# jerry102102102/RL_brain_trainer

Measured on AMD Instinct MI355X. Metric: env-steps/sec (whole node), Stage-5 Approach->Finisher PPO loops (rollout + update); value = the Approach loop, finisher.value = the Finisher loop, higher is better.
Workload: dtype f32

## Files before the change

include/kp1_ppo.h:

```cpp
#ifndef KP1_PPO_H
#define KP1_PPO_H

#include <stdint.h>

#include "kp1.h"

#ifdef __cplusplus
extern "C" {
#endif

int kp1_gae_scan(int32_t device, const float* rewards, const float* values, const uint8_t* dones, const float* last_values,
                 float gamma, float gae_lambda, float* advantages, float* returns, int32_t T, int32_t N, void* stream);

int kp1_gae_scan_replicas(int32_t device, const float* rewards, const float* values, const uint8_t* dones, const float* last_values,
                          const float* gamma_lambda, int32_t n_per_replica, float* advantages, float* returns, int32_t T, int32_t N, void* stream);

int kp1_bootstrap_truncated(int32_t device, float* rewards, const float* terminal_values, const uint8_t* dones, float gamma,
                            int64_t count, void* stream);

int kp1_adv_minibatch_sums(int32_t device, const float* advantages, const int64_t* idx, int64_t total, int64_t minibatch, double* out_sums,
                           void* stream);
int kp1_random_permutation(int32_t device, int64_t n, const uint32_t* keys, int64_t* out, void* stream);

int kp1_adv_minibatch_stats(int32_t device, const double* sums, int64_t n_minibatches, float* out_stats, void* stream);

#define KP1_CURRICULUM_MAX_WINDOW 1024
#define KP1_CURRICULUM_MAX_HISTORY 64
typedef struct kp1_curriculum_event {
  int64_t total_timesteps;
  int32_t from_stage, to_stage;
  double trigger_success_rate;
} kp1_curriculum_event;
typedef struct kp1_curriculum_state {
  int32_t stage_index;
  int32_t stage_episode_count;
  int32_t ring_len, ring_head;
  int32_t window_episodes, min_episodes_per_stage, max_stage_index, n_events;
  double success_rate_threshold;
  int64_t num_timesteps;
  int32_t ring[KP1_CURRICULUM_MAX_WINDOW];
  kp1_curriculum_event events[KP1_CURRICULUM_MAX_HISTORY];
} kp1_curriculum_state;

int kp1_curriculum_create(int32_t device, double success_rate_threshold, int32_t window_episodes, int32_t min_episodes_per_stage,
                          int32_t max_stage_index, int32_t initial_stage_index, kp1_curriculum_state** out_dev);
int kp1_curriculum_destroy(int32_t device, kp1_curriculum_state* st_dev);
int kp1_curriculum_observe(int32_t device, kp1_curriculum_state* st_dev, const uint8_t* dones, int32_t n, int32_t steps_per_call, void* stream);
int kp1_curriculum_observe_chunk(int32_t device, kp1_curriculum_state* st_dev, const uint8_t* dones, int32_t n_local, int32_t chunk_steps,
                                 int32_t world, void* stream);
int kp1_curriculum_read(int32_t device, const kp1_curriculum_state* st_dev, kp1_curriculum_state* out_host, void* stream);
int kp1_bind_stage_ptr(kp1_env* env, const int32_t* stage_dev);

#define KP1_CURRICULUM_MAX_REPLICAS 16
int kp1_curriculum_create_population(int32_t device, int32_t n_replicas, double success_rate_threshold, int32_t window_episodes,
                                     int32_t min_episodes_per_stage, int32_t max_stage_index, const int32_t* initial_stages,
                                     kp1_curriculum_state** out_dev);
int kp1_curriculum_observe_population(int32_t device, kp1_curriculum_state* states_dev, const uint8_t* dones, int32_t n_per_replica,
                                      int32_t n_replicas, int32_t steps_per_call, void* stream);
int kp1_curriculum_read_replica(int32_t device, const kp1_curriculum_state* states_dev, int32_t n_replicas, int32_t k,
                                kp1_curriculum_state* out_host, void* stream);
int kp1_bind_population_stages(kp1_env* env, const kp1_curriculum_state* states_dev, int32_t n_replicas);

#define KP1_DOCK_CURRICULUM_MAX_STAGES 16
#define KP1_DOCK_CURRICULUM_MAX_WINDOW 1024
#define KP1_DOCK_CURRICULUM_MAX_HISTORY 32
typedef struct kp1_dock_curriculum_stage {
  double action_delta_scale, dock_residual_action_limit, dock_delta_q_change_limit_scale;
  double close_bucket_probability, close_bucket_min_pos_error_m, close_bucket_max_pos_error_m, close_bucket_max_ori_error_rad,
         handoff_state_probability;
  double close_init_q_noise[KP1_NJ], init_q_noise[KP1_NJ];
  double success_rate_threshold;
  int32_t min_episodes;
  int32_t window_episodes;
  int32_t handoff_offset, handoff_count;
} kp1_dock_curriculum_stage;
typedef struct kp1_dock_curriculum_event {
  int64_t total_timesteps;
  int32_t from_stage, to_stage, stage_episode_count, reserved0;
  double trigger_success_rate;
} kp1_dock_curriculum_event;
typedef struct kp1_dock_curriculum_state {
  int32_t stage_index, stage_episode_count, ring_len, ring_head, window_episodes, n_stages, n_events, reserved0;
  int64_t num_timesteps;
  kp1_dock_curriculum_stage stages[KP1_DOCK_CURRICULUM_MAX_STAGES];
  kp1_dock_curriculum_event events[KP1_DOCK_CURRICULUM_MAX_HISTORY];
  uint8_t ring[KP1_DOCK_CURRICULUM_MAX_WINDOW];
} kp1_dock_curriculum_state;
int kp1_dock_curriculum_create(kp1_env* env, const kp1_dock_curriculum_stage* stages_host, int32_t n_stages, int32_t window_episodes,
                               kp1_dock_curriculum_state** out_dev);
int kp1_dock_curriculum_destroy(kp1_env* env, kp1_dock_curriculum_state* st_dev);
int kp1_dock_curriculum_observe(kp1_env* env, kp1_dock_curriculum_state* st_dev, const uint8_t* dones, int32_t n_local, int32_t chunk_steps, int32_t world,
                                void* stream);
int kp1_dock_curriculum_read(kp1_env* env, const kp1_dock_curriculum_state* st_dev, kp1_dock_curriculum_state* out_host, void* stream);
int kp1_dock_curriculum_create_population(kp1_env* env, const kp1_dock_curriculum_stage* stages_host, int32_t n_stages, int32_t window_episodes,
                                          int32_t n_replicas, kp1_dock_curriculum_state** out_dev);
int kp1_dock_curriculum_observe_population(kp1_env* env, kp1_dock_curriculum_state* states_dev, const uint8_t* dones, int32_t n_per_replica,
                                           int32_t n_replicas, void* stream);
int kp1_dock_curriculum_read_replica(kp1_env* env, const kp1_dock_curriculum_state* states_dev, int32_t n_replicas, int32_t k,
                                     kp1_dock_curriculum_state* out_host, void* stream);

#define KP1_MLP_IN 56
#define KP1_MLP_IN_PAD 64
#define KP1_MLP_IN_ROUTE 80
#define KP1_MLP_IN_ROUTE_PAD 128
#define KP1_MLP_ACT 7

typedef struct kp1_mlp kp1_mlp;

int kp1_mlp_create(int32_t device, int32_t hidden, int32_t max_batch, kp1_mlp** out);
int kp1_mlp_create_ex(int32_t device, int32_t hidden, int32_t obs_dim, int32_t max_batch, kp1_mlp** out);
#define KP1_MLP_MAX_REPLICAS 16
int kp1_mlp_create_population(int32_t device, int32_t hidden, int32_t obs_dim, int32_t max_batch, int32_t replicas, kp1_mlp** out);
int32_t kp1_mlp_replicas(const kp1_mlp* m);
typedef struct kp1_replica_hparams {
  float learning_rate, adam_eps, max_grad_norm, clip_range, ent_coef, vf_coef;
} kp1_replica_hparams;
int kp1_mlp_set_replica_hparams(kp1_mlp* m, const kp1_replica_hparams* host, int32_t n, void* stream);
int kp1_mlp_destroy(kp1_mlp* m);
int64_t kp1_mlp_num_params(int32_t hidden);
int64_t kp1_mlp_num_params_ex(int32_t hidden, int32_t obs_dim);
int kp1_mlp_pack_weights(kp1_mlp* m, const float* params, void* stream);

int kp1_mlp_forward(kp1_mlp* m, const float* obs, int32_t obs_stride, int32_t n, const float* noise, float* mean, float* value,
                    float* action, float* clipped_action, float* log_prob, void* stream);

int kp1_mlp_forward_env_step(kp1_mlp* m, kp1_env* env, const float* obs, int32_t obs_stride, const float* noise, float* value, float* action,
                             float* log_prob, float* next_obs, float* reward, uint8_t* done, float* terminal_obs, void* stream);

int kp1_eval_step(kp1_mlp* m, kp1_env* env, float* obs, float* reward, uint8_t* done, const kp1_eval_buffers* buffers, int32_t step,
                  const double* ready_thresholds , int32_t confirm_steps, void* stream);

int kp1_mlp_loss_grad(kp1_mlp* m, const float* obs, int32_t obs_stride, const int64_t* idx, int32_t n, const float* actions,
                      const float* old_log_prob, const float* advantages, const float* returns, float adv_mean, float adv_inv_std,
                      const float* adv_stats_dev, float clip_range, float ent_coef, float vf_coef, float inv_count, float* grad_out,
                      float* stats_out, int32_t grad_is_zero, void* stream);

#define KP1_MLP_OPT_FUSED 1
#define KP1_MLP_OPT_ACTOR_EXTRA_STEPS 2
#define KP1_MLP_OPT_STEP_COUNT 3
#define KP1_MLP_OPT_PROFILE 4
#define KP1_MLP_OPT_BF16X3_WGRAD 5
#define KP1_MLP_PROFILE_SLOTS 4
#define KP1_MLP_PROFILE_TILE 0
#define KP1_MLP_PROFILE_WGRAD 1
#define KP1_MLP_PROFILE_FINALIZE 2
#define KP1_MLP_PROFILE_ADAM 3
int kp1_mlp_set_option(kp1_mlp* m, int32_t option, int32_t value);
int kp1_mlp_profile_read(kp1_mlp* m, float* out_us , int32_t* out_launches );

int kp1_mlp_adam_step(kp1_mlp* m, float* params, float* grad, float* exp_avg, float* exp_avg_sq, float lr, float eps,
                      float max_grad_norm, int32_t step, int32_t flags, void* stream);

int kp1_mlp_anchor_loss_grad(kp1_mlp* m, const float* obs, int32_t obs_stride, const int64_t* idx, int32_t n, const float* teacher_actions,
                             float loss_weight, float* grad_out, float* loss_out, void* stream);

int kp1_mlp_anchor_adam_step(kp1_mlp* m, float* params, float* grad, float* exp_avg, float* exp_avg_sq, float lr, float eps,
                             float max_grad_norm, int32_t step, void* stream);

int kp1_mlp_placement_check(int32_t device, int32_t n_rows, int32_t* out, void* stream);
int kp1_mlp_time_kernels(kp1_mlp* m, const float* obs, int32_t obs_stride, int32_t n, int32_t iters, float* out_ms, double* out_flops,
                         void* stream);

int kp1_set_obs_stride(kp1_env* env, int32_t stride);

#ifdef __cplusplus
}
#endif
#endif
```

rl_brain_trainer_amd/csrc/kp1_mlp.hip:

```cpp
#include <hip/hip_runtime.h>
#include <hip/hip_ext.h>

#include <cmath>
#include <cstddef>
#include <cstdlib>
#include <cstring>
#include <vector>

#include "../../include/kp1_ppo.h"
#include "kp1_device.hpp"
#include "kp1_host.hpp"

using kp1::fail;
using namespace kp1;

typedef float f32x16 __attribute__((ext_vector_type(16)));
typedef float f32x4 __attribute__((ext_vector_type(4)));

namespace {

constexpr int ACT = KP1_MLP_ACT, HEADS = 8;
constexpr float LOG_SQRT_2PI = 0.9189385332046727f;

enum { EPI_BIAS_TANH = 0, EPI_DTANH = 1 };
// ... 1097 lines not shown
#pragma unroll
    for (int j = 0; j < WLOADS; ++j) *reinterpret_cast<f32x4*>(w3s + 4 * (threadIdx.x + 256 * j)) = wv[j];
#pragma unroll
    for (int j = 0; j < LOADS; ++j) {
      const int f = threadIdx.x + 256 * j, r = f / Q, c4 = f % Q;
      *reinterpret_cast<f32x4*>(h2s + r * hpitch + 4 * c4) = hv[j];
    }
  }
  __syncthreads();
  const int row_l = threadIdx.x >> 3, out = threadIdx.x & 7;
  const int row = blockIdx.x * HEAD_ROWS + row_l;
  const bool ok = row < a.n && out < ACT;
  float d = 0.f, l = 0.f;
  if (ok) {
    const int64_t src = a.idx ? a.idx[row] : (int64_t)row;
    const float mean = head_dot(h2s + row_l * hpitch, w3s + out * HP, HP) + a.b3[out];
    const float diff = mean - a.teacher[src * ACT + out];
    d = a.dcoef * diff;
    l = a.lcoef * diff * diff;
  }
  dout[row_l * 8 + out] = d;
  float dsum = d;
  dsum += __shfl_xor(dsum, 8);
  dsum += __shfl_xor(dsum, 16);
  dsum += __shfl_xor(dsum, 32);
  float lsum = l;
#pragma unroll
  for (int off = 1; off < 64; off <<= 1) lsum += __shfl_xor(lsum, off);
  const int wave_ = threadIdx.x >> 6;
  if ((threadIdx.x & 63) < 8) red[wave_ * 12 + out] = dsum;
  if ((threadIdx.x & 63) == 0) red[wave_ * 12 + 8] = lsum;
  __syncthreads();
  float* part = a.hpart + (int64_t)blockIdx.x * a.hpart_stride;
  if (threadIdx.x < 8) {
    const int slot = threadIdx.x < ACT ? threadIdx.x : 8;
    part[10 * HP + (threadIdx.x < ACT ? threadIdx.x : 15)] = ((red[slot] + red[12 + slot]) + red[24 + slot]) + red[36 + slot];
  }
  const int rows_here = min(HEAD_ROWS, a.n - blockIdx.x * HEAD_ROWS);
  for (int hh = threadIdx.x; hh < 2 * HP; hh += 256) {
    const int h = hh % HP;
    if (hh >= HP) {
      for (int r = 0; r < rows_here; ++r) a.dz2[a.strideH + (int64_t)(blockIdx.x * HEAD_ROWS + r) * HP + h] = 0.f;
      continue;
    }
    float wcol[ACT], gw[ACT];
#pragma unroll
    for (int o = 0; o < ACT; ++o) {
      wcol[o] = w3s[o * HP + h];
      gw[o] = 0.f;
    }
    float gb2 = 0.f;
    for (int r = 0; r < rows_here; ++r) {
      const float hp = h2s[r * hpitch + h];
      float dp = 0.f;
#pragma unroll
      for (int o = 0; o < ACT; ++o) {
        const float dd = dout[r * 8 + o];
        dp = fmaf(dd, wcol[o], dp);
        gw[o] = fmaf(dd, hp, gw[o]);
      }
      const float dz = dp * (1.f - hp * hp);
      a.dz2[(int64_t)(blockIdx.x * HEAD_ROWS + r) * HP + h] = dz;
      gb2 += dz;
    }
#pragma unroll
    for (int o = 0; o < ACT; ++o) part[o * HP + h] = gw[o];
    part[8 * HP + h] = gb2;
  }
}

__device__ __forceinline__ bool is_actor_element(const ParamLayout& L, int64_t i) {
  return (i >= L.p_w1 && i < L.v_w1) || (i >= L.a_w && i < L.c_w);
}

struct AnchorFinalizeArgs {
  FinalizeArgs f;
  float* loss_out;
};

template <bool POP = false>
__global__ void __launch_bounds__(256) anchor_finalize_kernel(const AnchorFinalizeArgs a_) {
  const FinalizeArgs a = POP ? finalize_args_replica(a_.f, blockIdx.y) : a_.f;
  const ParamLayout& L = a.L;
  __shared__ double sq[4];
  const int64_t i = (int64_t)(blockIdx.x * 256u + threadIdx.x);
  float gval = 0.f;
  if (i < L.total) {
    if (is_actor_element(L, i)) {
      const PartialSrc s = finalize_source(a, i);
      for (int c = 0; c < s.n; ++c) gval += s.p[(int64_t)c * s.stride];
    }
    a.grad[i] = gval;
  }
  if (blockIdx.x == 0 && threadIdx.x == 0) {
    float t = 0.f;
    for (int c = 0; c < a.h_n; ++c) t += a.hpart[(int64_t)c * a.h_stride + 10 * L.Hp + 15];
    a_.loss_out[POP ? blockIdx.y : 0u] = t;
  }
  double w = (double)gval * (double)gval;
  for (int off = 32; off > 0; off >>= 1) w += __shfl_xor(w, off);
  if ((threadIdx.x & 63) == 0) sq[threadIdx.x >> 6] = w;
  __syncthreads();
  if (threadIdx.x == 0) a.sumsq[blockIdx.x] = ((sq[0] + sq[1]) + sq[2]) + sq[3];
}

template <bool POP = false>
__global__ void __launch_bounds__(ADAM_BLOCK) anchor_adam_kernel(float* __restrict__ p, const float* __restrict__ g, float* __restrict__ m, float* __restrict__ v,
                                                          const double* __restrict__ partials, int n_partials, float lr, float eps, float max_norm,
                                                          const ParamLayout L, const Packed k_, const int* __restrict__ step_dev, int host_step,
                                                          unsigned r_partials, const float* __restrict__ hparams) {
  __shared__ float sh[3];
  const Packed k = POP ? packed_replica(k_, L, blockIdx.y) : k_;
  if constexpr (POP) {
    const unsigned o = blockIdx.y * (unsigned)L.total;
    p += o; g += o; m += o; v += o;
    partials += blockIdx.y * r_partials;
    if (hparams) {
      const float* e = hparams + blockIdx.y * (unsigned)HP_FIELDS;
      lr = e[HP_LR];
      eps = e[HP_EPS];
    }
  }
  const int64_t i = (int64_t)blockIdx.x * ADAM_BLOCK + threadIdx.x;
  const bool actor = i < L.total && is_actor_element(L, i);
  const int64_t il = actor ? i : L.p_w1;
  const float g_in = g[il], m_in = m[il], v_in = v[il], p_in = p[il];
  double s = 0.0;
  if (threadIdx.x < 64) {
    for (int q = threadIdx.x; q < n_partials; q += 64) s += partials[q];
    for (int off = 32; off > 0; off >>= 1) s += __shfl_xor(s, off);
  }
  if (threadIdx.x == 0) {
    const float norm = (float)sqrt(s);
    const int st = (host_step > 0 ? host_step : step_dev[0]) + step_dev[1] + 1;
    sh[0] = max_norm > 0.f ? fminf(max_norm / (norm + 1e-6f), 1.f) : 1.f;
    sh[1] = (float)((double)lr / (1.0 - pow(0.9, (double)st)));
    sh[2] = (float)sqrt(1.0 - pow(0.999, (double)st));
  }
  __syncthreads();
  if (actor) {
    const float gi = g_in * sh[0];
    const float mn = 0.9f * m_in + 0.1f * gi;
    const float vn = 0.999f * v_in + 0.001f * gi * gi;
    const float denom = sqrtf(vn) / sh[2] + eps;
    const float pn = p_in - sh[1] * (mn / denom);
    m[i] = mn; v[i] = vn; p[i] = pn;
    pack_one(i, pn, L, k);
  }
}

__global__ void anchor_count_kernel(int* __restrict__ actor_extra) { *actor_extra += 1; }

#include "kp1_env_step.inc"
#include "kp1_eval_step.inc"
#include "kp1_mlp_tile.inc"
#include "kp1_mlp_fused.inc"

}

struct kp1_mlp {
  int device = 0, H = 0, Hp = 0, max_batch = 0;
  int K = 1;
  ParamLayout L;
  Packed k{};
  float* h1 = nullptr;
  float* h2 = nullptr;
  float* dz2 = nullptr;
  float* dz1 = nullptr;
  float* xf = nullptr;
  int bf16x3 = 0;
  unsigned short* sp_h1 = nullptr; unsigned short* sp_dz2 = nullptr; unsigned short* sp_dz1 = nullptr; unsigned short* sp_xf = nullptr;
  double* partials = nullptr;
  double* anchor_partials = nullptr;
  float* slab = nullptr;
  float* slab1 = nullptr;
  float* bslab = nullptr;
  float* hpart = nullptr;
  int n_finalize_blocks = 0;
  int* step_dev = nullptr;
  float* hparams_dev = nullptr;
  bool hparams_on = false;
  int last_s2_n = 0, last_s1_n = 0;
  int fused = 1;
  const float* last_params = nullptr;
  bool slab_stale = false;
  std::vector<void*> allocs;
  int profile = 0;
  struct ProfPair { hipEvent_t a, b; };
  std::vector<ProfPair> prof[KP1_MLP_PROFILE_SLOTS];
  int prof_used[KP1_MLP_PROFILE_SLOTS] = {0, 0, 0, 0};
};

namespace {
struct ProfSlotInFlight { hipEvent_t a = nullptr, b = nullptr; bool attached = false; };
thread_local ProfSlotInFlight tl_prof;

struct ProfScope {
  kp1_mlp* m; int slot; hipStream_t stream; bool on;
  ProfScope(kp1_mlp* m_, int slot_, hipStream_t s_) : m(m_), slot(slot_), stream(s_), on(m_->profile != 0) {
    if (!on) return;
    auto& v = m->prof[slot];
    if (m->prof_used[slot] >= (int)v.size()) {
      kp1_mlp::ProfPair p{};
      if (hipEventCreate(&p.a) != hipSuccess || hipEventCreate(&p.b) != hipSuccess) { on = false; return; }
      v.push_back(p);
    }
    tl_prof.a = v[m->prof_used[slot]].a;
    tl_prof.b = v[m->prof_used[slot]].b;
    tl_prof.attached = false;
  }
  ~ProfScope() {
    if (!on) return;
    if (!tl_prof.attached) {
      (void)hipEventRecord(tl_prof.a, stream);
      (void)hipEventRecord(tl_prof.b, stream);
    }
    tl_prof = ProfSlotInFlight{};
    m->prof_used[slot] += 1;
  }
};

#define KP1_LAUNCH(kernel, grid, block, bytes, stream, ...)                                                        \
  do {                                                                                                             \
    if (tl_prof.a != nullptr && !tl_prof.attached) {                                                               \
      tl_prof.attached = true;                                                                                     \
      hipExtLaunchKernelGGL(kernel, grid, block, bytes, stream, tl_prof.a, tl_prof.b, 0, __VA_ARGS__);             \
    } else {                                                                                                       \
      hipLaunchKernelGGL(kernel, grid, block, bytes, stream, __VA_ARGS__);                                         \
    }                                                                                                              \
  } while (0)
}

namespace {

constexpr int N_PARTIALS = 128;
constexpr int ANCHOR_PARTIALS = 256;
constexpr int PARTIALS_STRIDE = 2 * N_PARTIALS + 2048;
constexpr int TN_SPLIT2 = 8, TN_SPLIT1 = 16;

int tn_chunk_rows(int n, int tiles) {
  int chunks = (256 + tiles - 1) / tiles;
  if (chunks > 64) chunks = 64;
  if (chunks < 1) chunks = 1;
  int rows = (n + chunks - 1) / chunks;
  rows = (rows + 63) / 64 * 64;
  return rows < 64 ? 64 : rows;
}

int mlp_check_device(const kp1_mlp* m) {
  HIP_TRY(hipSetDevice(m->device));
  return KP1_OK;
}

constexpr size_t TN_LDS_BYTES = sizeof(float) * 2 * 2 * 64 * (128 + 4);

template <int BN, int EPI, int K, bool POP = false>
int launch_nt_inst(const GemmNT& g, hipStream_t stream) {
  constexpr int NTH = BN == 256 ? 512 : 256;
  constexpr int BM = 64;
  constexpr int BKS = 32;
  size_t bytes = sizeof(float) * (BM * (size_t)(K + 4) + 2 * (size_t)BN * (BKS + 4));
  const size_t epi = sizeof(float) * (BM * (size_t)(BN + 4) + (size_t)(NTH / (BN / 4)) * BN);
  if (epi > bytes) bytes = epi;
  HIP_TRY(hipFuncSetAttribute((const void*)gemm_nt_kernel<BN, EPI, K, NTH, BM, BKS, POP>, hipFuncAttributeMaxDynamicSharedMemorySize, (int)bytes));
  hipLaunchKernelGGL((gemm_nt_kernel<BN, EPI, K, NTH, BM, BKS, POP>), dim3((g.M + BM - 1) / BM, g.N / BN, POP ? 2 * g.reps : 2), dim3(NTH), bytes, stream, g);
  return KP1_OK;
}

int nt_row_tiles(int n, int Hp) {
  (void)Hp;
  return (n + 63) / 64;
}

template <int EPI>
int launch_nt(const GemmNT& g, hipStream_t stream) {
  if (g.N % 128 != 0) return fail(KP1_ERR_INVALID, "gemm_nt needs N % 128 == 0");
  if (g.reps > 1) {
    if (g.N != 128) return fail(KP1_ERR_UNSUPPORTED, "population gemm_nt is instantiated for N = 128");
    if (g.K == 64) return launch_nt_inst<128, EPI, 64, true>(g, stream);
    if (g.K == 128) return launch_nt_inst<128, EPI, 128, true>(g, stream);
    return fail(KP1_ERR_UNSUPPORTED, "population gemm_nt is instantiated for K in {64, 128}");
  }
  const int row_tiles = (g.M + 63) / 64;
  const bool wide = (g.N % 256 == 0) && row_tiles * 2 >= 200;
  if (g.K == 64) return wide ? launch_nt_inst<256, EPI, 64>(g, stream) : launch_nt_inst<128, EPI, 64>(g, stream);
  if (g.K == 128) return wide ? launch_nt_inst<256, EPI, 128>(g, stream) : launch_nt_inst<128, EPI, 128>(g, stream);
  if (g.K == 256) return wide ? launch_nt_inst<256, EPI, 256>(g, stream) : launch_nt_inst<128, EPI, 256>(g, stream);
  return fail(KP1_ERR_UNSUPPORTED, "gemm_nt is instantiated for K in {64, 128, 256}");
}

int launch_tn(kp1_mlp* m, GemmTN t, int n_o_tiles, int slab_cols, float* slab, int* n_chunks_out, hipStream_t stream);

int launch_fused(const FusedArgs& fa_in, hipStream_t stream) {
  FusedArgs fa = fa_in;
  static const int stagger_us = [] { const char* e = std::getenv("KP1_FU_STAGGER_US"); return e ? std::atoi(e) : 11; }();
  static const int n_cus = [] {
    int dev = 0, n = 0;
    if (hipGetDevice(&dev) != hipSuccess || hipDeviceGetAttribute(&n, hipDeviceAttributeMultiprocessorCount, dev) != hipSuccess) n = 256;
    return n;
  }();
  const dim3 grid((fa.n + FU_BM - 1) / FU_BM, 1, 2);
  fa.n_cus = n_cus;
  fa.stagger_ticks = (int)(grid.x * grid.z) > n_cus ? stagger_us * 100 : 0;
  const size_t bytes = sizeof(float) * FU_LDS_FLOATS;
  if (fa.sp_h1 != nullptr) {
    if (fa.inp == 64) {
// ... 205 lines not shown
  }
  *out = m;
  return KP1_OK;
}
}

extern "C" {

int kp1_mlp_destroy(kp1_mlp* m) {
  if (!m) return KP1_OK;
  (void)hipSetDevice(m->device);
  (void)hipDeviceSynchronize();
  for (void* p : m->allocs) (void)hipFree(p);
  for (void* p : {(void*)m->sp_h1, (void*)m->sp_dz2, (void*)m->sp_dz1, (void*)m->sp_xf}) (void)hipFree(p);
  for (auto& v : m->prof)
    for (auto& pr : v) {
      (void)hipEventDestroy(pr.a);
      (void)hipEventDestroy(pr.b);
    }
  delete m;
  return KP1_OK;
}

int kp1_mlp_set_option(kp1_mlp* m, int32_t option, int32_t value) {
  if (!m) return fail(KP1_ERR_INVALID, "NULL argument");
  if (option == KP1_MLP_OPT_FUSED) {
    m->fused = value ? 1 : 0;
    if (!m->fused && m->slab_stale && m->last_params) {
      HIP_TRY(hipSetDevice(m->device));
      HIP_TRY(hipDeviceSynchronize());
      Packed k = m->k;
      k.formats = PACK_SLAB | PACK_FRAG;
      hipLaunchKernelGGL(pack_kernel<false>, dim3((unsigned)((m->L.total + 255) / 256)), dim3(256), 0, (hipStream_t)0, m->last_params, m->L, k);
      HIP_TRY(kp1::launch_status());
      HIP_TRY(hipDeviceSynchronize());
      m->slab_stale = false;
    }
    return KP1_OK;
  }
  if (option == KP1_MLP_OPT_BF16X3_WGRAD) {
    if (value && m->K > 1) return fail(KP1_ERR_UNSUPPORTED, "the bf16x3 weight-gradient experiment is not available on population handles");
    if (value && !(m->fused && m->Hp == FU_HP)) return fail(KP1_ERR_UNSUPPORTED, "the bf16x3 weight-gradient experiment needs the 2x256 tile kernels");
    if (value && !m->sp_h1) {
      HIP_TRY(hipSetDevice(m->device));
      const size_t act = (size_t)3 * 2 * m->max_batch * m->Hp * sizeof(unsigned short), xb = (size_t)3 * m->max_batch * m->L.INP * sizeof(unsigned short);
      for (unsigned short** p : {&m->sp_h1, &m->sp_dz2, &m->sp_dz1}) {
        HIP_TRY(hipMalloc((void**)p, act));
        HIP_TRY(hipMemset(*p, 0, act));
      }
      HIP_TRY(hipMalloc((void**)&m->sp_xf, xb));
      HIP_TRY(hipMemset(m->sp_xf, 0, xb));
    }
    m->bf16x3 = value ? 1 : 0;
    return KP1_OK;
  }
  if (option == KP1_MLP_OPT_PROFILE) {
    m->profile = value ? 1 : 0;
    for (int k = 0; k < KP1_MLP_PROFILE_SLOTS; ++k) m->prof_used[k] = 0;
    return KP1_OK;
  }
  if (option == KP1_MLP_OPT_STEP_COUNT) {
    if (value < 0) return fail(KP1_ERR_INVALID, "step count must be >= 0");
    HIP_TRY(hipSetDevice(m->device));
    HIP_TRY(hipMemcpy(m->step_dev, &value, sizeof(int), hipMemcpyHostToDevice));
    return KP1_OK;
  }
  if (option == KP1_MLP_OPT_ACTOR_EXTRA_STEPS) {
    if (value < 0) return fail(KP1_ERR_INVALID, "actor extra steps must be >= 0");
    HIP_TRY(hipSetDevice(m->device));
    HIP_TRY(hipMemcpy(m->step_dev + 1, &value, sizeof(int), hipMemcpyHostToDevice));
    return KP1_OK;
  }
  return fail(KP1_ERR_INVALID, "unknown kp1_mlp option");
}

int kp1_mlp_set_replica_hparams(kp1_mlp* m, const kp1_replica_hparams* host, int32_t n, void* stream) {
  static_assert(sizeof(kp1_replica_hparams) == sizeof(float) * HP_FIELDS, "kp1_replica_hparams is HP_FIELDS floats");
  static_assert(offsetof(kp1_replica_hparams, learning_rate) == sizeof(float) * HP_LR && offsetof(kp1_replica_hparams, adam_eps) == sizeof(float) * HP_EPS &&
                offsetof(kp1_replica_hparams, max_grad_norm) == sizeof(float) * HP_MAX_NORM && offsetof(kp1_replica_hparams, clip_range) == sizeof(float) * HP_CLIP &&
                offsetof(kp1_replica_hparams, ent_coef) == sizeof(float) * HP_ENT && offsetof(kp1_replica_hparams, vf_coef) == sizeof(float) * HP_VF,
                "kp1_replica_hparams field order");
  if (!m) return fail(KP1_ERR_INVALID, "NULL argument");
  if (n == 0) {
    m->hparams_on = false;
    return KP1_OK;
  }
  if (m->K == 1) return fail(KP1_ERR_UNSUPPORTED, "a K = 1 handle takes its hyper-parameters as scalar arguments, not a per-replica table");
  if (n != m->K || !host) return fail(KP1_ERR_INVALID, "kp1_mlp_set_replica_hparams needs one entry per replica (n = K)");
  for (int r = 0; r < n; ++r) {
    const kp1_replica_hparams& h = host[r];
    for (float v : {h.learning_rate, h.adam_eps, h.max_grad_norm, h.clip_range, h.ent_coef, h.vf_coef})
      if (!std::isfinite(v)) return fail(KP1_ERR_INVALID, "replica hyper-parameters must be finite");
  }
  int rc = mlp_check_device(m);
  if (rc != KP1_OK) return rc;
  HIP_TRY(hipMemcpyAsync(m->hparams_dev, host, sizeof(kp1_replica_hparams) * (size_t)n, hipMemcpyHostToDevice, (hipStream_t)stream));
  HIP_TRY(hipStreamSynchronize((hipStream_t)stream));
  m->hparams_on = true;
  return KP1_OK;
}

int kp1_mlp_pack_weights(kp1_mlp* m, const float* params, void* stream) {
  if (!m || !params) return fail(KP1_ERR_INVALID, "NULL argument");
  int rc = mlp_check_device(m);
  if (rc != KP1_OK) return rc;
  Packed k = m->k;
  k.formats = PACK_SLAB | PACK_FRAG;
  if (m->K > 1)
    hipLaunchKernelGGL(pack_kernel<true>, dim3((unsigned)((m->L.total + 255) / 256), m->K), dim3(256), 0, (hipStream_t)stream, params, m->L, k);
  else
    hipLaunchKernelGGL(pack_kernel<false>, dim3((unsigned)((m->L.total + 255) / 256)), dim3(256), 0, (hipStream_t)stream, params, m->L, k);
  HIP_TRY(kp1::launch_status());
  m->last_params = params;
  m->slab_stale = false;
  return KP1_OK;
}

int kp1_mlp_forward(kp1_mlp* m, const float* obs, int32_t obs_stride, int32_t n, const float* noise, float* mean, float* value, float* action,
                    float* clipped_action, float* log_prob, void* stream) {
  if (!m || !obs) return fail(KP1_ERR_INVALID, "NULL argument");
  if (n <= 0 || n > m->max_batch) return fail(KP1_ERR_INVALID, "n exceeds the workspace max_batch");
  const int IN = m->L.IN, INP = m->L.INP;
  if (obs_stride != IN && obs_stride != INP) return fail(KP1_ERR_INVALID, "obs_stride must be the observation width or its padded width (56 / 64, or 80 / 128)");
  int rc = mlp_check_device(m);
  if (rc != KP1_OK) return rc;
  if (m->fused && m->Hp == FU_HP) {
    FusedArgs fa{};
    fa.obs = obs; fa.obs_stride = obs_stride; fa.Kreal = obs_stride >= INP ? INP : IN; fa.inp = INP; fa.idx = nullptr; fa.n = n;
    fa.k = m->k;
    fa.noise = noise; fa.mean = mean; fa.value = value; fa.action = action; fa.clipped = clipped_action; fa.log_prob = log_prob;
    rc = launch_fused_infer(fa, (hipStream_t)stream);
    if (rc != KP1_OK) return rc;
    HIP_TRY(kp1::launch_status());
    return KP1_OK;
  }
  rc = launch_forward_layers(m, obs, obs_stride, nullptr, n, (hipStream_t)stream);
  if (rc != KP1_OK) return rc;
  HeadArgs a{};
  a.h2 = m->h2; a.strideH = (int64_t)m->max_batch * m->Hp; a.Hp = m->Hp; a.n = n; a.H = m->H;
  a.w3 = m->k.w3; a.b3 = m->k.b3; a.log_std = m->k.log_std;
  a.noise = noise; a.mean = mean; a.value = value; a.action = action; a.clipped = clipped_action; a.log_prob = log_prob;
  if (m->K > 1) {
    a.r_act = (unsigned)(2 * a.strideH);
    hipLaunchKernelGGL(head_infer_kernel<true>, dim3((n + HEAD_ROWS - 1) / HEAD_ROWS, m->K), dim3(256), sizeof(float) * HEADS * m->Hp, (hipStream_t)stream, a);
  } else {
    hipLaunchKernelGGL(head_infer_kernel<false>, dim3((n + HEAD_ROWS - 1) / HEAD_ROWS), dim3(256), sizeof(float) * HEADS * m->Hp, (hipStream_t)stream, a);
  }
  HIP_TRY(kp1::launch_status());
  return KP1_OK;
}

int kp1_mlp_forward_env_step(kp1_mlp* m, kp1_env* env, const float* obs, int32_t obs_stride, const float* noise, float* value, float* action,
                             float* log_prob, float* next_obs, float* reward, uint8_t* done, float* terminal_obs, void* stream) {
  if (!m || !env || !obs || !action || !next_obs || !reward || !done) return fail(KP1_ERR_INVALID, "NULL argument to kp1_mlp_forward_env_step");
  if (m->K > 1) return fail(KP1_ERR_UNSUPPORTED, "kp1_mlp_forward_env_step is not available on population handles");
  if (!(m->fused && m->Hp == FU_HP) || m->L.INP != 64)
    return fail(KP1_ERR_UNSUPPORTED, "kp1_mlp_forward_env_step needs the 2x256 tile kernels and the 56-float observation (padded to 64)");
  if (obs_stride != m->L.IN && obs_stride != m->L.INP) return fail(KP1_ERR_INVALID, "obs_stride must be 56 or 64");
  int rc = mlp_check_device(m);
  if (rc != KP1_OK) return rc;
  FusedArgs fa{};
  int mode = 0, device = 0;
  int64_t n_envs = 0;
  rc = kp1::env_step_args_f32(env, &fa.env, sizeof fa.env, nullptr, next_obs, reward, done, terminal_obs, 1, &mode, &n_envs, &device);
  if (rc != KP1_OK) return rc;
  if (device != m->device) return fail(KP1_ERR_INVALID, "the env handle and the MLP workspace live on different devices");
  if (n_envs > m->max_batch) return fail(KP1_ERR_INVALID, "more envs than the workspace max_batch");
  fa.obs = obs; fa.obs_stride = obs_stride; fa.Kreal = obs_stride >= m->L.INP ? m->L.INP : m->L.IN; fa.inp = m->L.INP; fa.idx = nullptr; fa.n = (int)n_envs;
  fa.k = m->k;
  fa.noise = noise; fa.value = value; fa.action = action; fa.log_prob = log_prob;
  rc = launch_fused_infer_env(fa, mode, (hipStream_t)stream);
  if (rc != KP1_OK) return rc;
  HIP_TRY(kp1::launch_status());
  return KP1_OK;
}

int kp1_eval_step(kp1_mlp* m, kp1_env* env, float* obs, float* reward, uint8_t* done, const kp1_eval_buffers* b, int32_t step,
                  const double* ready_thresholds, int32_t confirm_steps, void* stream) {
  if (!m || !env || !obs || !reward || !done || !b) return fail(KP1_ERR_INVALID, "NULL argument to kp1_eval_step");
  if (!b->metrics || !b->counters || !b->flags || !b->state || !b->n_alive) return fail(KP1_ERR_INVALID, "kp1_eval_step: NULL buffer");
  if (b->hand_metrics && (!b->hand_step || !b->hand_success || !b->hand_state)) return fail(KP1_ERR_INVALID, "kp1_eval_step: incomplete handoff buffers");
  if (step < 1) return fail(KP1_ERR_INVALID, "kp1_eval_step accounts env steps 1, 2, ...: step 0 (the initialisation after a reset) is kp1_eval_accumulate's");
  if (m->Hp != ES_HP) return fail(KP1_ERR_UNSUPPORTED, "kp1_eval_step covers the layer-wise widths (hidden 64 / 128); a 2x256 policy is evaluated through kp1_mlp_forward");
  if (m->L.INP != ES_INP) return fail(KP1_ERR_UNSUPPORTED, "kp1_eval_step needs the 56-float observation (padded to 64)");
  EvalStepArgs a{};
  int mode = 0, device = 0;
  int64_t n_envs = 0;
  int rc = kp1::env_step_args_f32(env, &a.env, sizeof a.env, nullptr, obs, reward, done, nullptr, 0, &mode, &n_envs, &device);
  if (rc != KP1_OK) return rc;
  if (a.env.stage_ptr) return fail(KP1_ERR_UNSUPPORTED, "kp1_eval_step: the env handle is bound to a curriculum tracker (an evaluation handle has none)");
  if (device != m->device) return fail(KP1_ERR_INVALID, "the env handle and the MLP workspace live on different devices");
  if (mode != KP1_MODE_APPROACH && mode != KP1_MODE_DOCK) return fail(KP1_ERR_UNSUPPORTED, "kp1_eval_step steps the approach or the dock mode");
  if (n_envs <= 0 || n_envs % m->K != 0) return fail(KP1_ERR_INVALID, "kp1_eval_step: the env count must be a multiple of the handle's replica count");
  rc = mlp_check_device(m);
  if (rc != KP1_OK) return rc;
  const int Hp = m->Hp, INP = m->L.INP;
  a.b = *b;
  a.w1 = m->k.w1p; a.b1 = m->k.b1; a.w2 = m->k.w2; a.b2 = m->k.b2; a.w3 = m->k.w3; a.b3 = m->k.b3;
  a.r_w1 = (unsigned)(2 * Hp * INP); a.r_w2 = (unsigned)(2 * Hp * Hp); a.r_b = (unsigned)(2 * Hp); a.r_w3 = (unsigned)(HEADS * Hp); a.r_b3 = (unsigned)HEADS;
  a.n = (int)(n_envs / m->K);
  a.Kreal = a.env.obs_stride >= INP ? INP : m->L.IN;
  a.step = step; a.confirm = confirm_steps;
  a.track_ready = ready_thresholds != nullptr;
  if (ready_thresholds) { a.thr_pos = ready_thresholds[0]; a.thr_ori = ready_thresholds[1]; a.thr_act = ready_thresholds[2]; a.thr_dq = ready_thresholds[3]; }
  hipStream_t st = (hipStream_t)stream;
  HIP_TRY(hipMemsetAsync(b->n_alive, 0, sizeof(int32_t), st));
  const dim3 grid((unsigned)((a.n + ES_BM - 1) / ES_BM), (unsigned)m->K);
  const bool pop = m->K > 1, dock = mode == KP1_MODE_DOCK;
  if (pop && dock) hipLaunchKernelGGL((eval_step_kernel<KP1_MODE_DOCK, true>), grid, dim3(ES_NTH), 0, st, a);
  else if (pop) hipLaunchKernelGGL((eval_step_kernel<KP1_MODE_APPROACH, true>), grid, dim3(ES_NTH), 0, st, a);
  else if (dock) hipLaunchKernelGGL((eval_step_kernel<KP1_MODE_DOCK, false>), grid, dim3(ES_NTH), 0, st, a);
  else hipLaunchKernelGGL((eval_step_kernel<KP1_MODE_APPROACH, false>), grid, dim3(ES_NTH), 0, st, a);
  HIP_TRY(kp1::launch_status());
  return KP1_OK;
}

int kp1_mlp_loss_grad(kp1_mlp* m, const float* obs, int32_t obs_stride, const int64_t* idx, int32_t n, const float* actions,
                      const float* old_log_prob, const float* advantages, const float* returns, float adv_mean, float adv_inv_std,
                      const float* adv_stats_dev, float clip_range, float ent_coef, float vf_coef, float inv_count, float* grad_out,
                      float* stats_out, int32_t grad_is_zero, void* stream_) {
  if (!m || !obs || !actions || !old_log_prob || !advantages || !returns || !grad_out) return fail(KP1_ERR_INVALID, "NULL argument");
  if (n <= 0 || n > m->max_batch) return fail(KP1_ERR_INVALID, "n exceeds the workspace max_batch");
  const int IN = m->L.IN, INP = m->L.INP;
  if (obs_stride != IN && obs_stride != INP) return fail(KP1_ERR_INVALID, "obs_stride must be the observation width or its padded width (56 / 64, or 80 / 128)");
  int rc = mlp_check_device(m);
  if (rc != KP1_OK) return rc;
  hipStream_t stream = (hipStream_t)stream_;
  const int Hp = m->Hp, H = m->H;
  const int64_t act_stride = (int64_t)m->max_batch * Hp;
  const ParamLayout& L = m->L;
  (void)grad_is_zero;
  const bool fused = m->fused && Hp == FU_HP;
  const bool pop = m->K > 1;
  if (pop && !idx) return fail(KP1_ERR_INVALID, "population handles gather their rows through idx [K][n]");
  const int64_t hpart_rep = (int64_t)(m->max_batch / 32) * (10 * Hp + 32);
  int adv_mode = 0;
  if (adv_stats_dev) adv_mode = 2;
  else if (adv_inv_std > 0.f) adv_mode = 3;
  else if (adv_inv_std == 0.f) adv_mode = 1;
  if (adv_mode == 1) {
    if (pop)
      hipLaunchKernelGGL(adv_partials_kernel<true>, dim3(N_PARTIALS, m->K), dim3(256), 0, stream, advantages, idx, n, m->partials, (unsigned)PARTIALS_STRIDE);
    else
      hipLaunchKernelGGL(adv_partials_kernel<false>, dim3(N_PARTIALS), dim3(256), 0, stream, advantages, idx, n, m->partials, 0u);
  }
  const int hpart_stride = 10 * Hp + 32;
  if (fused) {
    FusedArgs fa{};
    fa.obs = obs; fa.obs_stride = obs_stride; fa.Kreal = obs_stride >= INP ? INP : IN; fa.inp = INP; fa.idx = idx; fa.n = n;
    fa.k = m->k;
    fa.actions = actions; fa.old_logp = old_log_prob; fa.adv = advantages; fa.ret = returns;
    fa.adv_partials = m->partials; fa.n_adv_partials = N_PARTIALS; fa.adv_stats = adv_stats_dev; fa.adv_mean = adv_mean; fa.adv_inv_std = adv_inv_std;
    fa.adv_mode = adv_mode;
    fa.clip_range = clip_range; fa.vf_coef = vf_coef; fa.inv_count = inv_count;
    fa.h1 = m->h1; fa.dz2 = m->dz2; fa.dz1 = m->dz1; fa.act_stride = act_stride; fa.xf = m->xf;
    fa.bslab = m->bslab; fa.hpart = m->hpart; fa.hpart_stride = hpart_stride;
    if (m->bf16x3) {
      fa.sp_h1 = m->sp_h1; fa.sp_dz2 = m->sp_dz2; fa.sp_dz1 = m->sp_dz1; fa.sp_xf = m->sp_xf;
      fa.sp_plane = (int64_t)2 * m->max_batch * Hp; fa.sp_plane_x = (int64_t)m->max_batch * INP;
    }
    {
      ProfScope ps(m, KP1_MLP_PROFILE_TILE, stream);
      rc = launch_fused(fa, stream);
    }
    if (rc != KP1_OK) return rc;
  } else {
    rc = launch_forward_layers(m, obs, obs_stride, idx, n, stream);
    if (rc != KP1_OK) return rc;
    HeadArgs a{};
    a.h2 = m->h2; a.strideH = act_stride; a.Hp = Hp; a.n = n; a.H = H;
    a.w3 = m->k.w3; a.b3 = m->k.b3; a.log_std = m->k.log_std;
    a.idx = idx; a.actions = actions; a.old_logp = old_log_prob; a.adv = advantages; a.ret = returns;
    a.adv_partials = m->partials; a.n_adv_partials = N_PARTIALS; a.adv_stats = adv_stats_dev; a.adv_mean = adv_mean; a.adv_inv_std = adv_inv_std;
    a.adv_mode = adv_mode;
    a.clip_range = clip_range; a.ent_coef = ent_coef; a.vf_coef = vf_coef; a.inv_count = inv_count;
    a.dz2 = m->dz2;
    a.hpart = m->hpart; a.hpart_stride = hpart_stride;
    a.r_act = (unsigned)(2 * act_stride); a.r_hpart = (unsigned)hpart_rep; a.r_partials = (unsigned)PARTIALS_STRIDE;
    a.hparams = pop && m->hparams_on ? m->hparams_dev : nullptr;
    {
      const dim3 hgrid((n + HEAD_ROWS - 1) / HEAD_ROWS, m->K);
      const size_t hbytes = sizeof(float) * (HEADS * Hp + HEAD_ROWS * 8 + 84 + 2 * HEAD_ROWS * (Hp + 4));
      if (pop) {
        HIP_TRY(hipFuncSetAttribute((const void*)head_train_kernel<128, true>, hipFuncAttributeMaxDynamicSharedMemorySize, (int)hbytes));
        hipLaunchKernelGGL((head_train_kernel<128, true>), hgrid, dim3(256), hbytes, stream, a);
      } else if (Hp == 256) {
        HIP_TRY(hipFuncSetAttribute((const void*)head_train_kernel<256>, hipFuncAttributeMaxDynamicSharedMemorySize, (int)hbytes));
        hipLaunchKernelGGL(head_train_kernel<256>, hgrid, dim3(256), hbytes, stream, a);
      } else {
        HIP_TRY(hipFuncSetAttribute((const void*)head_train_kernel<128>, hipFuncAttributeMaxDynamicSharedMemorySize, (int)hbytes));
        hipLaunchKernelGGL(head_train_kernel<128>, hgrid, dim3(256), hbytes, stream, a);
      }
    }
    GemmNT g{};
    g.A = m->dz2; g.lda = Hp; g.strideA = act_stride; g.gather = nullptr;
    g.W = m->k.w2t; g.strideW = (int64_t)Hp * Hp;
    g.bias = nullptr; g.strideBias = 0;
    g.C = m->dz1; g.ldc = Hp; g.strideC = act_stride;
    g.aux = m->h1; g.strideAux = act_stride;
    g.colsum = m->bslab; g.strideColsum = Hp;
    g.M = n; g.N = Hp; g.K = Hp; g.Kreal = Hp;
    g.reps = m->K;
    g.r_A = g.r_C = g.r_aux = (unsigned)(2 * act_stride); g.r_W = (unsigned)(2 * Hp * Hp);
    g.r_colsum = (unsigned)((m->max_batch / 32) * 2 * Hp);
    rc = launch_nt<EPI_DTANH>(g, stream);
    if (rc != KP1_OK) return rc;
  }

  int s2_n = 0, s1_n = 0;
  if (fused) {
    TnFragArgs t{};
    t.inp = INP;
    t.dz2 = m->dz2; t.h1 = m->h1; t.dz1 = m->dz1; t.act_stride = act_stride; t.xf = m->xf;
    t.slab2 = m->slab; t.s2_net = (int64_t)Hp * Hp; t.s2_chunk = 2 * t.s2_net;
    t.slab1 = m->slab1; t.s1_net = (int64_t)Hp * INP; t.s1_chunk = 2 * t.s1_net;
    t.groups = (n + FU_BM - 1) / FU_BM * (FU_BM / 8);
    auto up8 = [](int v) { return (v + 7) / 8 * 8; };
    t.cg2 = up8((t.groups + TN_SPLIT2 - 1) / TN_SPLIT2);
    t.cg1 = up8((t.groups + TN_SPLIT1 - 1) / TN_SPLIT1);
    t.n_chunks2 = (t.groups + t.cg2 - 1) / t.cg2;
    t.n_chunks1 = (t.groups + t.cg1 - 1) / t.cg1;
    if (m->bf16x3) {
      TnBf16Args b{};
// ... 398 lines not shown
```

rl_brain_trainer_amd/csrc/kp1_mlp_tile.inc:

```

struct FusedArgs {
  const float* obs; int64_t obs_stride; int Kreal;
  int inp;
  const int64_t* idx; int n;
  Packed k;
  const float* actions; const float* old_logp; const float* adv; const float* ret;
  const double* adv_partials; int n_adv_partials; const float* adv_stats; float adv_mean, adv_inv_std; int adv_mode;
  float clip_range, vf_coef, inv_count;
  float* h1; float* dz2; float* dz1; int64_t act_stride;
  float* xf;
  float* bslab;
  float* hpart; int hpart_stride;
  const float* noise; float* mean; float* value; float* action; float* clipped; float* log_prob;
  int net_base;
  int stagger_ticks, n_cus;
  StepArgs<float> env;
  unsigned short* sp_h1; unsigned short* sp_dz2; unsigned short* sp_dz1; unsigned short* sp_xf; int64_t sp_plane, sp_plane_x;
};

typedef __bf16 bf16x8 __attribute__((ext_vector_type(8)));
struct Split3 { bf16x8 hi, mid, lo; };
__device__ __forceinline__ Split3 split3(const float* v) {
  Split3 o;
#pragma unroll
  for (int j = 0; j < 8; ++j) {
    const __bf16 h = (__bf16)v[j];
    const float r1 = v[j] - (float)h;
    const __bf16 m = (__bf16)r1;
    const float r2 = r1 - (float)m;
    o.hi[j] = h;
    o.mid[j] = m;
    o.lo[j] = (__bf16)r2;
  }
  return o;
}
__device__ __forceinline__ void store_split3(unsigned short* __restrict__ base, int64_t plane, int64_t fi, int ncb, int cb, int lane, const Split3& s) {
  const int64_t at = ((fi * ncb + cb) * 64 + lane) * 8;
  *reinterpret_cast<bf16x8*>(base + at) = s.hi;
  *reinterpret_cast<bf16x8*>(base + plane + at) = s.mid;
  *reinterpret_cast<bf16x8*>(base + 2 * plane + at) = s.lo;
}

__host__ __device__ inline int64_t frag8_at(int64_t b, int64_t col, int64_t C) {
  return ((b >> 3) * (C >> 5) + (col >> 5)) * 256 + ((col & 31) + 32 * ((b & 7) >> 2)) * 4 + (b & 3);
}

__device__ __forceinline__ f32x4 fu_wload(const char* __restrict__ base, unsigned off) {
  const __amdgpu_buffer_rsrc_t r = __builtin_amdgcn_make_buffer_rsrc(const_cast<char*>(base), 0, 0x7fffffff, 0x00020000);
  return __builtin_bit_cast(f32x4, __builtin_amdgcn_raw_buffer_load_b128(r, (int)off, 0, AUX_SC1));
}
constexpr int FU_HP = 256, FU_BKS = 32, FU_AP = FU_HP + 4;
constexpr int FU_STAGE = FU_HP * FU_BKS;
constexpr int FU_BM = 32, FU_NW = 4, FU_CB = 2, FU_NTH = 64 * FU_NW;
constexpr int FU_SCRATCH = 4 * FU_BM * 8 + FU_BM * 8 + FU_NW * 24 + 64;
constexpr int FU_LDS_FLOATS = 2 * FU_BM * FU_AP + HEADS * FU_HP + FU_SCRATCH;
static_assert(FU_LDS_FLOATS * 4 * 2 <= 160 * 1024, "the two training tiles of one CU must fit its LDS");

template <bool TRAIN, int K1S, int ENV = 0, bool SPLIT = false>
__global__ void __launch_bounds__(FU_NTH, ENV ? 1 : 2) mlp_tile_kernel(const FusedArgs a) {
  static_assert(!(TRAIN && ENV), "the env step rides on the inference tile only");
  static_assert(TRAIN || !SPLIT, "split planes are written by the training tile");
  constexpr int NW = FU_NW, CB = FU_CB, BM = FU_BM, NTH = FU_NTH, CW = 32 * CB;
  constexpr int INP = K1S * FU_BKS, FU_XP = INP + 4, GS_L2 = K1S, GS_BW = K1S + 8, GS_END = K1S + 16;
  constexpr int KG = FU_BKS / 8, NB = CB * KG;
  constexpr int L1_REAL_GROUPS = K1S == 2 ? (KP1_MLP_IN + 7) / 8 : (KP1_MLP_IN_ROUTE + 7) / 8;
  extern __shared__ float lds[];
  float* bufA = lds;
  float* bufB = bufA + BM * FU_AP;
  float* w3s = bufB + BM * FU_AP;
  float* dotred = w3s + HEADS * FU_HP;
  float* dout = dotred + 4 * BM * 8;
  float* wsum = dout + BM * 8;
  float* misc = wsum + NW * 24;

  const int z = (int)blockIdx.z + a.net_base;
  const int m0 = blockIdx.x * BM, slot = blockIdx.x;
  const int tid = threadIdx.x, lane = tid & 63, wave = __builtin_amdgcn_readfirstlane(tid >> 6);
  const unsigned lane_off = (unsigned)lane * 16u;
  const char* __restrict__ W1F = reinterpret_cast<const char*>(a.k.w1f + (int64_t)z * K1S * FU_STAGE + wave * NB * 64 * 4);
  const char* __restrict__ W2F = reinterpret_cast<const char*>(a.k.w2f + (int64_t)z * 8 * FU_STAGE + wave * NB * 64 * 4);
  const char* __restrict__ W2TF = reinterpret_cast<const char*>(a.k.w2tf + (int64_t)z * 8 * FU_STAGE + wave * NB * 64 * 4);

  f32x4 bf[3][NB];
#define FU_BLOAD(gs)                                                                                    \
  if ((gs) < GS_END) {                                                                                  \
    const char* p_ = (gs) < GS_L2 ? W1F + (gs) * (FU_STAGE * 4) : ((gs) < GS_BW ? W2F + ((gs) - GS_L2) * (FU_STAGE * 4) : W2TF + ((gs) - GS_BW) * (FU_STAGE * 4)); \
    _Pragma("unroll") for (int q = 0; q < NB; ++q) bf[(gs) % 3][q] = fu_wload(p_, q * 1024 + lane_off); \
  }
  f32x16 acc[CB];
#define FU_INIT_ACC(bias)                                                                               \
  _Pragma("unroll") for (int c = 0; c < CB; ++c)                                                        \
    _Pragma("unroll") for (int e = 0; e < 16; ++e) acc[c][e] = (bias)[c];
#ifdef KP1_TR_HEADS
#define KP1_TR_G2(slot)
#define KP1_TR_HD(slot) KP1_TR(slot)
#else
#define KP1_TR_G2(slot) KP1_TR(slot)
#define KP1_TR_HD(slot)
#endif
#ifdef KP1_FU_NOMFMA
#define FU_MFMA(acc_, a_, b_) acc_[0] += (a_) * (b_);
#else
#define FU_MFMA(acc_, a_, b_) acc_ = __builtin_amdgcn_mfma_f32_32x32x2f32(a_, b_, acc_, 0, 0, 0);
#endif
#ifdef KP1_FU_NOTANH
#define FU_TANH(x) (x)
#else
#define FU_TANH(x) kp_tanh(x)
#endif
#define FU_GEMM(abuf, ap, KT, GS0)                                                                      \
  {                                                                                                     \
    const float* as = (abuf) + (lane & 31) * (ap) + 4 * (lane >> 5);                                     \
    _Pragma("unroll") for (int s = 0; s < (KT); ++s) {                                                  \
      FU_BLOAD((GS0) + s + 2)                                                                           \
      __builtin_amdgcn_sched_barrier(0);                                                                \
      f32x4 av[KG];                                                                                     \
      _Pragma("unroll") for (int kg = 0; kg < KG; ++kg)                                                 \
        av[kg] = *reinterpret_cast<const f32x4*>(as + s * FU_BKS + kg * 8);                              \
      _Pragma("unroll") for (int kg = 0; kg < KG; ++kg)                                                 \
        if (!((GS0) == 0 && s * KG + kg >= L1_REAL_GROUPS))    \
        _Pragma("unroll") for (int i = 0; i < 4; ++i)                                                   \
          _Pragma("unroll") for (int c = 0; c < CB; ++c)                                                \
            FU_MFMA(acc[c], av[kg][i], bf[((GS0) + s) % 3][c * KG + kg][i])                              \
      __builtin_amdgcn_sched_barrier(0);                                                                \
      if ((GS0) == GS_L2) { KP1_TR_G2(7 + s) }                                                          \
    }                                                                                                   \
  }
#define FU_ROW(e) (((e) & 3) + 8 * ((e) >> 2) + 4 * (lane >> 5))
#define FU_COL(c) (wave * CW + (c) * 32 + (lane & 31))
#ifdef KP1_FU_NOSTORE
#define FU_STORE_ACC(dst)
#else
#define FU_STORE_ACC(dst)                                                                               \
  _Pragma("unroll") for (int c = 0; c < CB; ++c)                                                        \
    _Pragma("unroll") for (int g = 0; g < 4; ++g) {                                                     \
      const f32x4 v_ = {acc[c][4 * g], acc[c][4 * g + 1], acc[c][4 * g + 2], acc[c][4 * g + 3]};        \
      *reinterpret_cast<f32x4*>((dst) + ((int64_t)((m0 >> 3) + g) * (FU_HP / 32) + wave * CB + c) * 256 + lane * 4) = v_; \
    }
#endif
#define FU_STORE_ACC_SPLIT(dst, plane)                                                                  \
  if constexpr (SPLIT) {                                                                               \
    _Pragma("unroll") for (int c = 0; c < CB; ++c)                                                      \
      _Pragma("unroll") for (int f = 0; f < 2; ++f) {                                                   \
        float v8_[8];                                                                                   \
        _Pragma("unroll") for (int j = 0; j < 8; ++j) v8_[j] = acc[c][8 * f + j];                       \
        store_split3((dst) + (int64_t)z * ((plane) / 2), (plane), (int64_t)(m0 >> 4) + f, FU_HP / 32, wave * CB + c, lane, split3(v8_)); \
      }                                                                                                 \
  }
#define FU_STORE_FRAG_SPLIT(tile, pitch, dst, plane, zoff, C)                                           \
  if constexpr (SPLIT) {                                                                               \
    _Pragma("unroll") for (int q = wave; q < (BM / 16) * ((C) / 32); q += NW) {                         \
      const int f_ = q / ((C) / 32), cb_ = q % ((C) / 32);                                              \
      const float* t_ = (tile) + (16 * f_ + 4 * (lane >> 5)) * (pitch) + 32 * cb_ + (lane & 31);        \
      float v8_[8];                                                                                     \
      _Pragma("unroll") for (int j = 0; j < 8; ++j) v8_[j] = t_[(8 * (j >> 2) + (j & 3)) * (pitch)];    \
      store_split3((dst) + (zoff), (plane), (int64_t)(m0 >> 4) + f_, (C) / 32, cb_, lane, split3(v8_));  \
    }                                                                                                   \
  }
#ifdef KP1_FU_NOSTORE
#define FU_STORE_FRAG(tile, pitch, dst, C)
#else
#define FU_STORE_FRAG(tile, pitch, dst, C)                                                              \
  _Pragma("unroll") for (int q = wave; q < (BM / 8) * ((C) / 32); q += NW) {                            \
    const int g_ = q / ((C) / 32), cb_ = q % ((C) / 32);                                                \
    const float* t_ = (tile) + (8 * g_ + 4 * (lane >> 5)) * (pitch) + 32 * cb_ + (lane & 31);           \
    f32x4 v_;                                                                                           \
    _Pragma("unroll") for (int i = 0; i < 4; ++i) v_[i] = t_[i * (pitch)];                              \
    *reinterpret_cast<f32x4*>((dst) + ((int64_t)((m0 >> 3) + g_) * ((C) / 32) + cb_) * 256 + lane * 4) = v_; \
  }
#endif

  KP1_TR(0)
  if (TRAIN) { KP1_CLK(0, 0) }
  if (TRAIN && a.stagger_ticks > 0) {
    const int linear = blockIdx.x + gridDim.x * blockIdx.z;
    if (linear >= a.n_cus && linear < 2 * a.n_cus) {
      const unsigned long long t0_ = wall_clock64();
      while (wall_clock64() - t0_ < (unsigned long long)a.stagger_ticks) __builtin_amdgcn_s_sleep(16);
    }
  }
  FU_BLOAD(0)
  FU_BLOAD(1)
  __builtin_amdgcn_sched_barrier(0);
  {
    constexpr int XQ = INP / 4, X_LOADS = BM * XQ / NTH;
    constexpr int W3_LOADS = HEADS * FU_HP / 4 / NTH;
    static_assert(X_LOADS >= 1 && X_LOADS * NTH == BM * XQ && W3_LOADS >= 1 && W3_LOADS * NTH == HEADS * FU_HP / 4, "prologue loads must tile the workgroup");
    int64_t xrow[X_LOADS];
    f32x4 xv[X_LOADS], w3v[W3_LOADS];
#pragma unroll
    for (int j = 0; j < X_LOADS; ++j) {
      const int m = min(m0 + (tid + NTH * j) / XQ, a.n - 1);
      xrow[j] = a.idx ? a.idx[m] : (int64_t)m;
    }
#pragma unroll
    for (int j = 0; j < X_LOADS; ++j) {
      const int k = 4 * ((tid + NTH * j) % XQ);
      xv[j] = *reinterpret_cast<const f32x4*>(a.obs + xrow[j] * a.obs_stride + (k < a.Kreal ? k : 0));
    }
#pragma unroll
    for (int j = 0; j < W3_LOADS; ++j) w3v[j] = *reinterpret_cast<const f32x4*>(a.k.w3 + 4 * (tid + NTH * j));
#pragma unroll
    for (int j = 0; j < X_LOADS; ++j) {
      const int f = tid + NTH * j, row = f / XQ, k = 4 * (f % XQ);
      const float keep = (m0 + row < a.n && k < a.Kreal) ? 1.f : 0.f;
      *reinterpret_cast<f32x4*>(bufB + row * FU_XP + k) = xv[j] * keep;
    }
#pragma unroll
    for (int j = 0; j < W3_LOADS; ++j) *reinterpret_cast<f32x4*>(w3s + 4 * (tid + NTH * j)) = w3v[j];
  }
  if (TRAIN && z == 0 && wave == 0) {
    float mean = 0.f, inv_std = 1.f;
    if (a.adv_mode == 1) {
      double ps = 0.0, pss = 0.0;
      for (int k = lane; k < a.n_adv_partials; k += 64) {
        ps += a.adv_partials[2 * k];
        pss += a.adv_partials[2 * k + 1];
      }
      for (int off = 32; off > 0; off >>= 1) {
        ps += __shfl_xor(ps, off);
        pss += __shfl_xor(pss, off);
      }
      const double mu = ps / a.n;
      const double var = a.n > 1 ? fmax((pss - a.n * mu * mu) / (a.n - 1), 0.0) : 0.0;
      mean = (float)mu;
      inv_std = (float)(1.0 / (sqrt(var) + 1e-8));
    } else if (a.adv_mode == 2) {
      mean = a.adv_stats[0];
      inv_std = a.adv_stats[1];
    } else if (a.adv_mode == 3) {
      mean = a.adv_mean;
      inv_std = a.adv_inv_std;
    }
    if (lane == 0) {
      misc[0] = mean;
      misc[1] = inv_std;
    }
  }
  float bias1[CB], bias2[CB];
#pragma unroll
  for (int c = 0; c < CB; ++c) {
    bias1[c] = a.k.b1[z * FU_HP + FU_COL(c)];
    bias2[c] = a.k.b2[z * FU_HP + FU_COL(c)];
  }
  const int l_row = tid >> 3, l_out = tid & 7;
  const bool l_ok = m0 + l_row < a.n;
  const int64_t l_src = a.idx ? a.idx[min(m0 + l_row, a.n - 1)] : (int64_t)min(m0 + l_row, a.n - 1);
  __syncthreads();
  KP1_TR(1)
  constexpr bool fp32_out = !SPLIT;
  if (TRAIN && z == 0 && fp32_out) { FU_STORE_FRAG(bufB, FU_XP, a.xf, INP) }
  if (TRAIN && z == 0) { FU_STORE_FRAG_SPLIT(bufB, FU_XP, a.sp_xf, a.sp_plane_x, (int64_t)0, INP) }

  FU_INIT_ACC(bias1)
  FU_GEMM(bufB, FU_XP, K1S, 0)
#pragma unroll
  for (int c = 0; c < CB; ++c)
#pragma unroll
    for (int e = 0; e < 16; ++e) {
      acc[c][e] = FU_TANH(acc[c][e]);
      bufA[FU_ROW(e) * FU_AP + FU_COL(c)] = acc[c][e];
    }
  if (TRAIN && fp32_out) { FU_STORE_ACC(a.h1 + z * a.act_stride) }
  if (TRAIN) { FU_STORE_ACC_SPLIT(a.sp_h1, a.sp_plane) }
  __syncthreads();
  KP1_TR(2)
  float l_act = 0.f, l_old = 0.f, l_adv = 0.f, l_ret = 0.f, l_b3 = a.k.b3[l_out], l_ls = a.k.log_std[l_out < ACT ? l_out : 0];
  if (TRAIN) {
    if (z == 0) {
      if (l_out < ACT) l_act = a.actions[l_src * ACT + l_out];
      l_old = a.old_logp[l_src];
      l_adv = a.adv[l_src];
    } else {
      l_ret = a.ret[l_src];
    }
  } else if (z == 0 && a.noise && l_ok && l_out < ACT) {
    l_act = a.noise[l_src * ACT + l_out];
  }

  FU_INIT_ACC(bias2)
  FU_GEMM(bufA, FU_AP, 8, GS_L2)
#pragma unroll
  for (int c = 0; c < CB; ++c)
#pragma unroll
    for (int e = 0; e < 16; ++e) bufB[FU_ROW(e) * FU_AP + FU_COL(c)] = FU_TANH(acc[c][e]);
  __syncthreads();
  KP1_TR(3)

  {
    const int row = lane & 31, kq = wave, part = kq * 2 + (lane >> 5);
    const float* hrow = bufB + row * FU_AP + part * 32;
    f32x4 hv[8];
#pragma unroll
    for (int q = 0; q < 8; ++q) hv[q] = *reinterpret_cast<const f32x4*>(hrow + 4 * q);
    auto dot = [&](int o) {
      const float* w = w3s + o * FU_HP + part * 32;
      float s = 0.f;
#pragma unroll
      for (int q = 0; q < 8; ++q) {
        const f32x4 wv = *reinterpret_cast<const f32x4*>(w + 4 * q);
        s = fmaf(hv[q].x, wv.x, s);
        s = fmaf(hv[q].y, wv.y, s);
        s = fmaf(hv[q].z, wv.z, s);
        s = fmaf(hv[q].w, wv.w, s);
      }
      s += __shfl_xor(s, 32);
      if (lane < 32) dotred[(kq * BM + row) * 8 + o] = s;
    };
    if (z == 0) {
#pragma unroll
      for (int o = 0; o < ACT; ++o) dot(o);
    } else {
      dot(7);
    }
  }
  __syncthreads();
  KP1_TR_HD(7)
  if (!TRAIN) {
    const bool mine = z == 0 ? l_out < ACT : l_out == 7;
    float v = 0.f;
    if (mine) {
#pragma unroll
      for (int p = 0; p < 4; ++p) v += dotred[(p * BM + l_row) * 8 + l_out];
      v += l_b3;
    }
    float lp = 0.f;
    if (z == 0) {
      float act = v;
      if (l_ok && l_out < ACT) {
        if (a.mean) a.mean[l_src * ACT + l_out] = v;
        if (a.noise) {
          act = fmaf(expf(l_ls), l_act, v);
          lp = -0.5f * l_act * l_act - l_ls - LOG_SQRT_2PI;
        }
        if (a.action) a.action[l_src * ACT + l_out] = act;
        if (a.clipped) a.clipped[l_src * ACT + l_out] = fminf(fmaxf(act, -1.f), 1.f);
      }
      lp += __shfl_xor(lp, 1);
      lp += __shfl_xor(lp, 2);
      lp += __shfl_xor(lp, 4);
      if (l_ok && l_out == 0 && a.log_prob) a.log_prob[l_src] = lp;
      if constexpr (ENV != 0) {
        dout[l_row * 8 + l_out] = (l_ok && l_out < ACT) ? act : 0.f;
        __syncthreads();
        if (wave == 0) {
          const bool live = lane < BM && m0 + lane < a.n;
          float o[KP1_OBS_DIM];
          if (live) step_env_lane<float, ENV == 1 ? KP1_MODE_APPROACH : KP1_MODE_DOCK, false>(a.env, (int64_t)(m0 + lane), dout + lane * 8, o);
          store_obs_tile(a.env.obs, (int64_t)m0, min(BM, a.n - m0), o, live, a.env.obs_stride, bufA);
        }
      }
    } else if (l_ok && l_out == 7 && a.value) {
      a.value[l_src] = v;
    }
    return;
  }
  {
    const int row_l = l_row, out = l_out;
    const bool ok = l_ok;
    const bool mine = z == 0 ? out < ACT : out == 7;
    float v = 0.f;
    if (mine) {
#pragma unroll
      for (int p = 0; p < 4; ++p) v += dotred[(p * BM + row_l) * 8 + out];
      v += l_b3;
    }
    float zs = 0.f, inv_sd = 1.f, lp = 0.f;
    if (z == 0 && ok && out < ACT) {
      inv_sd = expf(-l_ls);
      zs = (l_act - v) * inv_sd;
      lp = -0.5f * zs * zs - l_ls - LOG_SQRT_2PI;
    }
    lp += __shfl_xor(lp, 1);
    lp += __shfl_xor(lp, 2);
    lp += __shfl_xor(lp, 4);
    float g_logp = 0.f, d = 0.f, pl = 0.f, vl = 0.f, kl = 0.f;
    if (ok && z == 0) {
      const float A = (l_adv - misc[0]) * misc[1];
      const float lr_ = lp - l_old;
      const float ratio = expf(lr_);
      const float rc = fminf(fmaxf(ratio, 1.f - a.clip_range), 1.f + a.clip_range);
      const float s1 = ratio * A, s2 = rc * A;
      const bool inside = ratio >= 1.f - a.clip_range && ratio <= 1.f + a.clip_range;
      g_logp = (inside || s1 < s2) ? -A * ratio * a.inv_count : 0.f;
      if (out < ACT) {
        d = g_logp * zs * inv_sd;
      } else {
        pl = -fminf(s1, s2);
        kl = (ratio - 1.f) - lr_;
      }
    } else if (ok && out == 7) {
      d = a.vf_coef * 2.f * (v - l_ret) * a.inv_count;
      vl = (l_ret - v) * (l_ret - v);
    }
    dout[row_l * 8 + out] = (ok && mine) ? d : 0.f;
    float gls = (z == 0 && ok && out < ACT) ? g_logp * (zs * zs - 1.f) : 0.f;
    float dsum = (ok && mine) ? d : 0.f;
    float l0 = pl, l1 = vl, l2 = kl;
#pragma unroll
    for (int off = 8; off < 64; off <<= 1) {
      gls += __shfl_xor(gls, off);
      dsum += __shfl_xor(dsum, off);
      l0 += __shfl_xor(l0, off);
      l1 += __shfl_xor(l1, off);
      l2 += __shfl_xor(l2, off);
    }
    if (lane < 8) {
      wsum[wave * 24 + out] = dsum;
      wsum[wave * 24 + 8 + out] = gls;
      if (out == 7) {
        wsum[wave * 24 + 16] = l0;
        wsum[wave * 24 + 17] = l1;
        wsum[wave * 24 + 18] = l2;
      }
    }
  }
  KP1_TR_HD(8)
  __syncthreads();
  KP1_TR_HD(9)
  if (tid < 18) {
    const int k = tid;
    const int w = k < 8 ? k : (k < 15 ? 8 + (k - 8) : 16 + (k - 15));
    const float v = ((wsum[w] + wsum[24 + w]) + wsum[48 + w]) + wsum[72 + w];
    const bool pi_slot = (k < 7) || (k >= 8 && k < 15) || k == 15 || k == 17;
    if (pi_slot == (z == 0)) a.hpart[(int64_t)slot * a.hpart_stride + 10 * FU_HP + k] = v;
  }
  {
    constexpr int DZ_COLS = FU_HP / NW, DZ_CG = DZ_COLS / 4, DZ_RG = 64 / DZ_CG, DZ_ROWS = 32 / DZ_RG;
    const int cg = lane % DZ_CG, rg = lane / DZ_CG, col = wave * DZ_COLS + 4 * cg;
    float* part = a.hpart + (int64_t)slot * a.hpart_stride;
    f32x4 gw[ACT], gb2 = {0.f, 0.f, 0.f, 0.f}, w3c[ACT];
#pragma unroll
    for (int o = 0; o < ACT; ++o) {
      gw[o] = f32x4{0.f, 0.f, 0.f, 0.f};
      w3c[o] = f32x4{0.f, 0.f, 0.f, 0.f};
    }
    if (z == 0) {
#pragma unroll
      for (int o = 0; o < ACT; ++o) w3c[o] = *reinterpret_cast<const f32x4*>(w3s + o * FU_HP + col);
    } else {
      w3c[0] = *reinterpret_cast<const f32x4*>(w3s + 7 * FU_HP + col);
    }
#pragma unroll
    for (int j = 0; j < DZ_ROWS; ++j) {
      const int row = rg * DZ_ROWS + j;
      const f32x4 h = *reinterpret_cast<const f32x4*>(bufB + row * FU_AP + col);
      f32x4 dp = {0.f, 0.f, 0.f, 0.f};
      if (z == 0) {
#pragma unroll
        for (int o = 0; o < ACT; ++o) {
          const float dd = dout[row * 8 + o];
          dp += dd * w3c[o];
          gw[o] += dd * h;
        }
      } else {
        const float dd = dout[row * 8 + 7];
        dp = dd * w3c[0];
        gw[0] += dd * h;
      }
      const f32x4 dz = dp * (1.f - h * h);
      gb2 += dz;
      *reinterpret_cast<f32x4*>(bufB + row * FU_AP + col) = dz;
    }
    auto fold = [&](f32x4 v) {
#pragma unroll
      for (int i = 0; i < 4; ++i) {
#pragma unroll
        for (int off = DZ_CG; off < 64; off <<= 1) v[i] += __shfl_xor(v[i], off);
      }
      return v;
    };
    gb2 = fold(gb2);
    if (z == 0) {
#pragma unroll
      for (int o = 0; o < ACT; ++o) {
        const f32x4 t = fold(gw[o]);
        if (rg == 0) *reinterpret_cast<f32x4*>(part + o * FU_HP + col) = t;
      }
      if (rg == 0) *reinterpret_cast<f32x4*>(part + 8 * FU_HP + col) = gb2;
    } else {
      const f32x4 t = fold(gw[0]);
      if (rg == 0) {
        *reinterpret_cast<f32x4*>(part + 7 * FU_HP + col) = t;
        *reinterpret_cast<f32x4*>(part + 9 * FU_HP + col) = gb2;
      }
    }
  }
  KP1_TR_HD(10)
  __syncthreads();
  KP1_TR(4)
  if (fp32_out) { FU_STORE_FRAG(bufB, FU_AP, a.dz2 + z * a.act_stride, FU_HP) }
  if (TRAIN) { FU_STORE_FRAG_SPLIT(bufB, FU_AP, a.sp_dz2, a.sp_plane, (int64_t)z * (a.sp_plane / 2), FU_HP) }

  {
    float zero[CB];
#pragma unroll
    for (int c = 0; c < CB; ++c) zero[c] = 0.f;
    FU_INIT_ACC(zero)
  }
  FU_GEMM(bufB, FU_AP, 8, GS_BW)
  {
    float* __restrict__ bs = a.bslab + ((int64_t)slot * 2 + z) * FU_HP;
#pragma unroll
// ... 31 lines not shown
```

rl_brain_trainer_amd/csrc/kp1_ppo.hip:

```cpp
#include <hip/hip_runtime.h>

#include <cstring>
#include <vector>

#include "../../include/kp1_ppo.h"
#include "kp1_host.hpp"

using kp1::fail;

namespace {

__global__ void __launch_bounds__(256) gae_scan_kernel(const float* __restrict__ rewards, const float* __restrict__ values,
                                                       const uint8_t* __restrict__ dones, const float* __restrict__ last_values,
                                                       float gamma, float lam, float* __restrict__ adv, float* __restrict__ ret, int T, int N) {
  const int i = blockIdx.x * blockDim.x + threadIdx.x;
  if (i >= N) return;
  float next_value = last_values[i];
  float last_gae = 0.0f;
  for (int t = T - 1; t >= 0; --t) {
    const int64_t k = (int64_t)t * N + i;
    const float nonterm = (dones[k] & (KP1_DONE_TERMINATED | KP1_DONE_TRUNCATED)) ? 0.0f : 1.0f;
    const float v = values[k];
    const float delta = rewards[k] + gamma * next_value * nonterm - v;
    last_gae = delta + gamma * lam * nonterm * last_gae;
    adv[k] = last_gae;
    ret[k] = last_gae + v;
    next_value = v;
  }
}

__global__ void __launch_bounds__(256) gae_scan_replicas_kernel(const float* __restrict__ rewards, const float* __restrict__ values,
                                                                const uint8_t* __restrict__ dones, const float* __restrict__ last_values,
                                                                const float* __restrict__ gamma_lambda, int n_per_replica, float* __restrict__ adv,
                                                                float* __restrict__ ret, int T, int N) {
  const int i = blockIdx.x * blockDim.x + threadIdx.x;
  if (i >= N) return;
  const int r = i / n_per_replica;
  const float gamma = gamma_lambda[2 * r], lam = gamma_lambda[2 * r + 1];
  float next_value = last_values[i];
  float last_gae = 0.0f;
  for (int t = T - 1; t >= 0; --t) {
    const int64_t k = (int64_t)t * N + i;
    const float nonterm = (dones[k] & (KP1_DONE_TERMINATED | KP1_DONE_TRUNCATED)) ? 0.0f : 1.0f;
    const float v = values[k];
    const float delta = rewards[k] + gamma * next_value * nonterm - v;
    last_gae = delta + gamma * lam * nonterm * last_gae;
    adv[k] = last_gae;
    ret[k] = last_gae + v;
    next_value = v;
  }
}

__global__ void __launch_bounds__(256) bootstrap_kernel(float* __restrict__ rewards, const float* __restrict__ tv,
                                                        const uint8_t* __restrict__ dones, float gamma, int64_t count) {
  const int64_t k = (int64_t)blockIdx.x * blockDim.x + threadIdx.x;
  if (k >= count) return;
  const uint8_t d = dones[k];
  if ((d & KP1_DONE_TRUNCATED) && !(d & KP1_DONE_TERMINATED)) rewards[k] += gamma * tv[k];
}

struct TrackerCtx {
  int stage, count, len, head, window, min_episodes, max_stage, n_events, sum;
  double threshold;
  long long timesteps;
  bool ring_dirty;
};

__device__ __forceinline__ void tracker_load(const kp1_curriculum_state* __restrict__ st, int* __restrict__ ring, TrackerCtx& c) {
  const int lane = threadIdx.x;
  c.stage = st->stage_index; c.count = st->stage_episode_count; c.len = st->ring_len; c.head = st->ring_head;
  c.window = st->window_episodes; c.min_episodes = st->min_episodes_per_stage; c.max_stage = st->max_stage_index; c.n_events = st->n_events;
  c.threshold = st->success_rate_threshold; c.timesteps = st->num_timesteps;
  c.ring_dirty = false;
  int part = 0;
  for (int k = lane; k < c.window; k += 64) {
    const int v = st->ring[k];
    ring[k] = v;
    const int age = k >= c.head ? k - c.head : k - c.head + c.window;
    if (age < c.len) part += v;
  }
  for (int off = 32; off > 0; off >>= 1) part += __shfl_xor(part, off);
  c.sum = part;
  __syncthreads();
}

__device__ __forceinline__ void tracker_store(kp1_curriculum_state* __restrict__ st, const int* __restrict__ ring, const TrackerCtx& c) {
  const int lane = threadIdx.x;
  __syncthreads();
  if (c.ring_dirty)
    for (int k = lane; k < c.window; k += 64) st->ring[k] = ring[k];
  if (lane == 0) {
    st->stage_index = c.stage; st->stage_episode_count = c.count; st->ring_len = c.len; st->ring_head = c.head;
    st->n_events = c.n_events; st->num_timesteps = c.timesteps;
  }
}

constexpr int TRK_BLOCK = 64 * 64, TRK_PARALLEL_MIN = 192;
struct TrackerScratch { uint8_t* sbit; uint16_t* pfx; };

__device__ __forceinline__ void tracker_append_run(int* __restrict__ ring, TrackerCtx& c, const uint8_t* __restrict__ sbit, int pos, int R) {
  const int lane = threadIdx.x, W = c.window;
  const int j0 = R > W ? R - W : 0;
  __syncthreads();
  for (int j = j0 + lane; j < R; j += 64) ring[(c.head + c.len + j) % W] = sbit[pos + j];
  __syncthreads();
  const int over = c.len + R - W;
  c.head = over > 0 ? (c.head + over) % W : c.head;
  c.len = c.len + R < W ? c.len + R : W;
  c.count += R;
  int part = 0;
  for (int k = lane; k < W; k += 64) {
    const int age = k >= c.head ? k - c.head : k - c.head + W;
    if (age < c.len) part += ring[k];
  }
  for (int off = 32; off > 0; off >>= 1) part += __shfl_xor(part, off);
  c.sum = part;
}

__device__ __forceinline__ void tracker_block_parallel(kp1_curriculum_state* __restrict__ st, int* __restrict__ ring, TrackerCtx& c, const TrackerScratch& ws,
                                                       unsigned long long dmask, unsigned long long smask, int E) {
  const int lane = threadIdx.x, W = c.window;
  int mine = __popcll(dmask), off = mine;
  for (int d = 1; d < 64; d <<= 1) {
    const int up = __shfl_up(off, d);
    if (lane >= d) off += up;
  }
  off -= mine;
  __syncthreads();
  for (unsigned long long m = dmask; m; m &= m - 1) {
    const int b = __ffsll((long long)m) - 1;
    ws.sbit[off++] = (uint8_t)((smask >> b) & 1ull);
  }
  __syncthreads();
  int pos = 0;
  while (pos < E) {
    const int R = E - pos;
    if (c.stage >= c.max_stage) {
      tracker_append_run(ring, c, ws.sbit, pos, R);
      break;
    }
    const int L = c.len, T = L + R;
    const int seg = (T + 63) / 64, j_lo = lane * seg < T ? lane * seg : T, j_hi = j_lo + seg < T ? j_lo + seg : T;
    auto y = [&](int j) -> int { return j < L ? ring[(c.head + j) % W] : (int)ws.sbit[pos + (j - L)]; };
    int tot = 0;
    for (int j = j_lo; j < j_hi; ++j) tot += y(j);
    int run = tot;
    for (int d = 1; d < 64; d <<= 1) {
      const int up = __shfl_up(run, d);
      if (lane >= d) run += up;
    }
    run -= tot;
    __syncthreads();
    if (lane == 0) ws.pfx[0] = 0;
    for (int j = j_lo; j < j_hi; ++j) {
      run += y(j);
      ws.pfx[j + 1] = (uint16_t)run;
    }
    __syncthreads();
    int best = R;
    for (int r = lane; r < R; r += 64) {
      const int filled = L + r + 1;
      if (filled < W || c.count + r + 1 < c.min_episodes) continue;
      const int wsum = (int)ws.pfx[filled] - (int)ws.pfx[filled - W];
      if ((double)wsum / (double)W >= c.threshold) {
        best = r;
        break;
      }
    }
    for (int d = 32; d > 0; d >>= 1) {
      const int o = __shfl_xor(best, d);
      best = o < best ? o : best;
    }
    if (best >= R) {
      tracker_append_run(ring, c, ws.sbit, pos, R);
      break;
    }
    const int filled = L + best + 1;
    const double rate = (double)((int)ws.pfx[filled] - (int)ws.pfx[filled - W]) / (double)W;
    if (lane == 0 && c.n_events < KP1_CURRICULUM_MAX_HISTORY) {
      kp1_curriculum_event& ev = st->events[c.n_events];
      ev.total_timesteps = c.timesteps;
      ev.from_stage = c.stage;
      ev.to_stage = c.stage + 1;
      ev.trigger_success_rate = rate;
    }
    c.n_events += 1;
    c.stage += 1;
    c.count = 0;
    c.len = 0;
    c.head = 0;
    c.sum = 0;
    pos += best + 1;
  }
}

__device__ __forceinline__ void curriculum_scan(kp1_curriculum_state* __restrict__ st, int* __restrict__ ring, TrackerCtx& c, const TrackerScratch& ws,
                                                const uint8_t* __restrict__ dones, int n, int steps_per_call) {
  const int lane = threadIdx.x;
  c.timesteps += steps_per_call;
  for (int base = 0; base < n; base += 64 * 64) {
    const int first = base + lane * 64;
    unsigned long long dmask = 0ull, smask = 0ull;
    if (first + 64 <= n && (reinterpret_cast<uintptr_t>(dones + first) & 15) == 0) {
      const uint4* p = reinterpret_cast<const uint4*>(dones + first);
      uint4 w[4];
#pragma unroll
      for (int q = 0; q < 4; ++q) w[q] = p[q];
#pragma unroll
      for (int q = 0; q < 4; ++q) {
        const unsigned int words[4] = {w[q].x, w[q].y, w[q].z, w[q].w};
#pragma unroll
        for (int k = 0; k < 4; ++k)
#pragma unroll
          for (int b = 0; b < 4; ++b) {
            const unsigned int d = (words[k] >> (8 * b)) & 0xffu;
            const int bit = q * 16 + k * 4 + b;
            if (d & (KP1_DONE_TERMINATED | KP1_DONE_TRUNCATED)) {
              dmask |= 1ull << bit;
              if (d & KP1_DONE_SUCCESS) smask |= 1ull << bit;
            }
          }
      }
    } else {
      for (int b = 0; b < 64 && first + b < n; ++b) {
        const uint8_t d = dones[first + b];
        if (d & (KP1_DONE_TERMINATED | KP1_DONE_TRUNCATED)) {
          dmask |= 1ull << b;
          if (d & KP1_DONE_SUCCESS) smask |= 1ull << b;
        }
      }
    }
    unsigned long long busy = __ballot(dmask != 0ull);
    if (busy == 0ull) continue;
    c.ring_dirty = true;
    {
      int ended = __popcll(dmask);
      for (int off = 32; off > 0; off >>= 1) ended += __shfl_xor(ended, off);
      if (ended >= TRK_PARALLEL_MIN) {
        tracker_block_parallel(st, ring, c, ws, dmask, smask, ended);
        continue;
      }
    }
    int stage = c.stage, count = c.count, len = c.len, head = c.head, sum = c.sum, n_events = c.n_events;
    const int window = c.window;
    while (busy) {
      const int src = __ffsll((long long)busy) - 1;
      busy &= busy - 1;
      unsigned long long m = __shfl(dmask, src);
      const unsigned long long sm = __shfl(smask, src);
      if (lane != 0) continue;
      while (m) {
        const int b = __ffsll((long long)m) - 1;
        m &= m - 1;
        const int success = (int)((sm >> b) & 1ull);
        count += 1;
        if (len < window) {
          ring[head + len < window ? head + len : head + len - window] = success;
          len += 1;
          sum += success;
        } else {
          sum += success - ring[head];
          ring[head] = success;
          head = head + 1 < window ? head + 1 : 0;
        }
        if (stage >= c.max_stage) continue;
        if (count < c.min_episodes) continue;
        if (len < window) continue;
        const double rate = (double)sum / (double)len;
        if (rate >= c.threshold) {
          if (n_events < KP1_CURRICULUM_MAX_HISTORY) {
            kp1_curriculum_event& ev = st->events[n_events];
            ev.total_timesteps = c.timesteps;
            ev.from_stage = stage;
            ev.to_stage = stage + 1;
            ev.trigger_success_rate = rate;
          }
          n_events += 1;
          stage += 1;
          count = 0;
          len = 0;
          head = 0;
          sum = 0;
        }
      }
    }
    c.stage = __shfl(stage, 0); c.count = __shfl(count, 0); c.len = __shfl(len, 0); c.head = __shfl(head, 0);
    c.sum = __shfl(sum, 0); c.n_events = __shfl(n_events, 0);
  }
}

__global__ void __launch_bounds__(64) curriculum_kernel(kp1_curriculum_state* __restrict__ st, const uint8_t* __restrict__ dones, int n,
                                                        int steps_per_call) {
  __shared__ int ring[KP1_CURRICULUM_MAX_WINDOW];
  __shared__ uint8_t sbit[TRK_BLOCK];
  __shared__ uint16_t pfx[TRK_BLOCK + KP1_CURRICULUM_MAX_WINDOW + 1];
  const TrackerScratch ws = {sbit, pfx};
  {
    const int lane = threadIdx.x;
    bool any = false;
    for (int base = 0; base < n; base += 64 * 64) {
      const int first = base + lane * 64;
      if (first + 64 <= n && (reinterpret_cast<uintptr_t>(dones + first) & 15) == 0) {
        const uint4* p = reinterpret_cast<const uint4*>(dones + first);
        unsigned int acc = 0u;
#pragma unroll
        for (int q = 0; q < 4; ++q) {
          const uint4 w = p[q];
          acc |= w.x | w.y | w.z | w.w;
        }
        any |= (acc & (0x01010101u * (unsigned)(KP1_DONE_TERMINATED | KP1_DONE_TRUNCATED))) != 0u;
      } else {
        for (int b = 0; b < 64 && first + b < n; ++b) any |= (dones[first + b] & (KP1_DONE_TERMINATED | KP1_DONE_TRUNCATED)) != 0;
      }
    }
    if (__ballot(any) == 0ull) {
      if (lane == 0) atomicAdd(reinterpret_cast<unsigned long long*>(&st->num_timesteps), (unsigned long long)(long long)steps_per_call);
      return;
    }
  }
  TrackerCtx c;
  tracker_load(st, ring, c);
  curriculum_scan(st, ring, c, ws, dones, n, steps_per_call);
  tracker_store(st, ring, c);
}

__global__ void __launch_bounds__(64) curriculum_chunk_kernel(kp1_curriculum_state* __restrict__ st, const uint8_t* __restrict__ dones, int n_local,
                                                              int chunk_steps, int world, int steps_per_env_step) {
  __shared__ int ring[KP1_CURRICULUM_MAX_WINDOW];
  __shared__ uint8_t sbit[TRK_BLOCK];
  __shared__ uint16_t pfx[TRK_BLOCK + KP1_CURRICULUM_MAX_WINDOW + 1];
  const TrackerScratch ws = {sbit, pfx};
  TrackerCtx c;
  tracker_load(st, ring, c);
  for (int t = 0; t < chunk_steps; ++t)
    for (int r = 0; r < world; ++r)
      curriculum_scan(st, ring, c, ws, dones + ((int64_t)r * chunk_steps + t) * n_local, n_local, r == 0 ? steps_per_env_step : 0);
  tracker_store(st, ring, c);
}

__global__ void __launch_bounds__(64) curriculum_population_kernel(kp1_curriculum_state* __restrict__ states, const uint8_t* __restrict__ dones_all,
                                                                   int n, int steps_per_call) {
  __shared__ int ring[KP1_CURRICULUM_MAX_WINDOW];
  __shared__ uint8_t sbit[TRK_BLOCK];
  __shared__ uint16_t pfx[TRK_BLOCK + KP1_CURRICULUM_MAX_WINDOW + 1];
  const TrackerScratch ws = {sbit, pfx};
  kp1_curriculum_state* __restrict__ st = states + blockIdx.x;
  const uint8_t* __restrict__ dones = dones_all + (int64_t)blockIdx.x * n;
  {
    const int lane = threadIdx.x;
    bool any = false;
    for (int base = 0; base < n; base += 64 * 64) {
      const int first = base + lane * 64;
      if (first + 64 <= n && (reinterpret_cast<uintptr_t>(dones + first) & 15) == 0) {
        const uint4* p = reinterpret_cast<const uint4*>(dones + first);
        unsigned int acc = 0u;
#pragma unroll
        for (int q = 0; q < 4; ++q) {
          const uint4 w = p[q];
          acc |= w.x | w.y | w.z | w.w;
        }
        any |= (acc & (0x01010101u * (unsigned)(KP1_DONE_TERMINATED | KP1_DONE_TRUNCATED))) != 0u;
      } else {
        for (int b = 0; b < 64 && first + b < n; ++b) any |= (dones[first + b] & (KP1_DONE_TERMINATED | KP1_DONE_TRUNCATED)) != 0;
      }
    }
    if (__ballot(any) == 0ull) {
      if (lane == 0) atomicAdd(reinterpret_cast<unsigned long long*>(&st->num_timesteps), (unsigned long long)(long long)steps_per_call);
      return;
    }
  }
  TrackerCtx c;
  tracker_load(st, ring, c);
  curriculum_scan(st, ring, c, ws, dones, n, steps_per_call);
  tracker_store(st, ring, c);
}

int check_device(int device) {
  int count = 0;
  if (hipGetDeviceCount(&count) != hipSuccess || count <= 0) return fail(KP1_ERR_NO_DEVICE, "no HIP device: this library has no CPU path");
  if (device < 0 || device >= count) return fail(KP1_ERR_INVALID, "device index out of range");
  HIP_TRY(hipSetDevice(device));
  return KP1_OK;
}

}

extern "C" {

int kp1_gae_scan(int32_t device, const float* rewards, const float* values, const uint8_t* dones, const float* last_values, float gamma,
                 float gae_lambda, float* advantages, float* returns, int32_t T, int32_t N, void* stream) {
  if (!rewards || !values || !dones || !last_values || !advantages || !returns || T <= 0 || N <= 0) return fail(KP1_ERR_INVALID, "bad argument to kp1_gae_scan");
  int rc = check_device(device);
  if (rc != KP1_OK) return rc;
  const int block = N <= 16384 ? 64 : 256;
  hipLaunchKernelGGL(gae_scan_kernel, dim3((N + block - 1) / block), dim3(block), 0, (hipStream_t)stream, rewards, values, dones, last_values,
                     gamma, gae_lambda, advantages, returns, T, N);
  HIP_TRY(kp1::launch_status());
  return KP1_OK;
}

int kp1_gae_scan_replicas(int32_t device, const float* rewards, const float* values, const uint8_t* dones, const float* last_values,
                          const float* gamma_lambda, int32_t n_per_replica, float* advantages, float* returns, int32_t T, int32_t N, void* stream) {
  if (!rewards || !values || !dones || !last_values || !gamma_lambda || !advantages || !returns || T <= 0 || N <= 0)
    return fail(KP1_ERR_INVALID, "bad argument to kp1_gae_scan_replicas");
  if (n_per_replica <= 0 || N % n_per_replica != 0) return fail(KP1_ERR_INVALID, "kp1_gae_scan_replicas: N must be a multiple of n_per_replica");
  int rc = check_device(device);
  if (rc != KP1_OK) return rc;
  const int block = N <= 16384 ? 64 : 256;
  hipLaunchKernelGGL(gae_scan_replicas_kernel, dim3((N + block - 1) / block), dim3(block), 0, (hipStream_t)stream, rewards, values, dones,
                     last_values, gamma_lambda, n_per_replica, advantages, returns, T, N);
  HIP_TRY(kp1::launch_status());
  return KP1_OK;
}

}

namespace {
__global__ void __launch_bounds__(256) adv_minibatch_sums_kernel(const float* __restrict__ adv, const int64_t* __restrict__ idx, int64_t total, int64_t mb,
                                                                 double* __restrict__ out) {
  __shared__ double s1[256], s2[256];
  const int64_t begin = (int64_t)blockIdx.x * mb, end = begin + mb < total ? begin + mb : total;
  double a = 0.0, b = 0.0;
  for (int64_t i = begin + threadIdx.x; i < end; i += 256) {
    const double v = (double)adv[idx ? idx[i] : i];
    a += v;
    b += v * v;
  }
  s1[threadIdx.x] = a;
  s2[threadIdx.x] = b;
  __syncthreads();
  for (int k = 128; k > 0; k >>= 1) {
    if (threadIdx.x < k) {
      s1[threadIdx.x] += s1[threadIdx.x + k];
      s2[threadIdx.x] += s2[threadIdx.x + k];
    }
    __syncthreads();
  }
  if (threadIdx.x == 0) {
    out[3 * blockIdx.x] = s1[0];
    out[3 * blockIdx.x + 1] = s2[0];
    out[3 * blockIdx.x + 2] = (double)(end - begin);
  }
}
struct PermKeys { uint32_t mul[4], add[4]; };
__global__ void __launch_bounds__(256) permutation_kernel(int64_t* __restrict__ out, int64_t n, int bits, const PermKeys k) {
  const int64_t i = (int64_t)blockIdx.x * 256 + threadIdx.x;
  if (i >= n) return;
  const uint32_t mask = bits >= 32 ? 0xffffffffu : ((1u << bits) - 1u);
  const int sh = bits > 1 ? bits / 2 : 1;
  uint32_t x = (uint32_t)i;
  do {
#pragma unroll
    for (int r = 0; r < 4; ++r) {
      x = (x * k.mul[r] + k.add[r]) & mask;
      x ^= x >> sh;
    }
  } while ((int64_t)x >= n);
  out[i] = (int64_t)x;
}

__global__ void __launch_bounds__(64) adv_minibatch_stats_kernel(const double* __restrict__ sums, int64_t n_mb, float* __restrict__ out) {
#pragma clang fp contract(off)
  const int64_t b = (int64_t)blockIdx.x * 64 + threadIdx.x;
  if (b >= n_mb) return;
  const double s0 = sums[3 * b], s1 = sums[3 * b + 1], cnt = sums[3 * b + 2];
  const double mean = s0 / cnt;
  const double dof = cnt - 1.0 < 1.0 ? 1.0 : cnt - 1.0;
  double var = (s1 - cnt * mean * mean) / dof;
  var = var < 0.0 ? 0.0 : var;
  out[2 * b] = (float)mean;
  out[2 * b + 1] = (float)(1.0 / (sqrt(var) + 1e-8));
}
}

extern "C" {

int kp1_random_permutation(int32_t device, int64_t n, const uint32_t* keys, int64_t* out, void* stream) {
  if (!keys || !out || n <= 0 || n > ((int64_t)1 << 31)) return fail(KP1_ERR_INVALID, "bad argument to kp1_random_permutation");
  int rc = check_device(device);
  if (rc != KP1_OK) return rc;
  int bits = 1;
  while (((int64_t)1 << bits) < n) ++bits;
  PermKeys k;
  for (int r = 0; r < 4; ++r) {
    k.mul[r] = keys[r] | 1u;
    k.add[r] = keys[4 + r];
  }
  hipLaunchKernelGGL(permutation_kernel, dim3((unsigned)((n + 255) / 256)), dim3(256), 0, (hipStream_t)stream, out, n, bits, k);
  HIP_TRY(kp1::launch_status());
  return KP1_OK;
}

int kp1_adv_minibatch_stats(int32_t device, const double* sums, int64_t n_minibatches, float* out_stats, void* stream) {
  if (!sums || !out_stats || n_minibatches <= 0) return fail(KP1_ERR_INVALID, "bad argument to kp1_adv_minibatch_stats");
  int rc = check_device(device);
  if (rc != KP1_OK) return rc;
  hipLaunchKernelGGL(adv_minibatch_stats_kernel, dim3((unsigned)((n_minibatches + 63) / 64)), dim3(64), 0, (hipStream_t)stream, sums, n_minibatches,
                     out_stats);
  HIP_TRY(kp1::launch_status());
  return KP1_OK;
}

int kp1_adv_minibatch_sums(int32_t device, const float* advantages, const int64_t* idx, int64_t total, int64_t minibatch, double* out_sums,
                           void* stream) {
  if (!advantages || !out_sums || total <= 0 || minibatch <= 0) return fail(KP1_ERR_INVALID, "bad argument to kp1_adv_minibatch_sums");
  int rc = check_device(device);
  if (rc != KP1_OK) return rc;
  const int64_t n_mb = (total + minibatch - 1) / minibatch;
  hipLaunchKernelGGL(adv_minibatch_sums_kernel, dim3((unsigned)n_mb), dim3(256), 0, (hipStream_t)stream, advantages, idx, total, minibatch, out_sums);
  HIP_TRY(kp1::launch_status());
  return KP1_OK;
}

int kp1_bootstrap_truncated(int32_t device, float* rewards, const float* terminal_values, const uint8_t* dones, float gamma, int64_t count,
                            void* stream) {
  if (!rewards || !terminal_values || !dones || count <= 0) return fail(KP1_ERR_INVALID, "bad argument to kp1_bootstrap_truncated");
  int rc = check_device(device);
  if (rc != KP1_OK) return rc;
  hipLaunchKernelGGL(bootstrap_kernel, dim3((unsigned)((count + 255) / 256)), dim3(256), 0, (hipStream_t)stream, rewards, terminal_values, dones,
                     gamma, count);
  HIP_TRY(kp1::launch_status());
  return KP1_OK;
}

int kp1_curriculum_create(int32_t device, double success_rate_threshold, int32_t window_episodes, int32_t min_episodes_per_stage,
                          int32_t max_stage_index, int32_t initial_stage_index, kp1_curriculum_state** out_dev) {
  return kp1_curriculum_create_population(device, 1, success_rate_threshold, window_episodes, min_episodes_per_stage, max_stage_index,
                                          &initial_stage_index, out_dev);
}
int kp1_curriculum_create_population(int32_t device, int32_t n_replicas, double success_rate_threshold, int32_t window_episodes,
                                     int32_t min_episodes_per_stage, int32_t max_stage_index, const int32_t* initial_stages,
                                     kp1_curriculum_state** out_dev) {
  if (!out_dev || !initial_stages) return fail(KP1_ERR_INVALID, "NULL argument");
  if (n_replicas < 1 || n_replicas > KP1_CURRICULUM_MAX_REPLICAS) return fail(KP1_ERR_INVALID, "n_replicas must be in [1, KP1_CURRICULUM_MAX_REPLICAS]");
  int rc = check_device(device);
  if (rc != KP1_OK) return rc;
  std::vector<kp1_curriculum_state> h((size_t)n_replicas);
  for (int k = 0; k < n_replicas; ++k) {
    kp1_curriculum_state& s = h[(size_t)k];
    std::memset(&s, 0, sizeof s);
    s.success_rate_threshold = success_rate_threshold;
    s.window_episodes = window_episodes < 1 ? 1 : window_episodes;
    if (s.window_episodes > KP1_CURRICULUM_MAX_WINDOW) return fail(KP1_ERR_INVALID, "window_episodes exceeds KP1_CURRICULUM_MAX_WINDOW");
    s.min_episodes_per_stage = min_episodes_per_stage < 1 ? 1 : min_episodes_per_stage;
    s.max_stage_index = max_stage_index < 0 ? 0 : max_stage_index;
    int init = initial_stages[k] < s.max_stage_index ? initial_stages[k] : s.max_stage_index;
    s.stage_index = init < 0 ? 0 : init;
  }
  kp1_curriculum_state* d = nullptr;
  HIP_TRY(hipMalloc((void**)&d, sizeof(kp1_curriculum_state) * h.size()));
  HIP_TRY(hipMemcpy(d, h.data(), sizeof(kp1_curriculum_state) * h.size(), hipMemcpyHostToDevice));
  *out_dev = d;
  return KP1_OK;
}
int kp1_curriculum_destroy(int32_t device, kp1_curriculum_state* st_dev) {
  int rc = check_device(device);
  if (rc != KP1_OK) return rc;
  HIP_TRY(hipFree(st_dev));
  return KP1_OK;
}
int kp1_curriculum_observe(int32_t device, kp1_curriculum_state* st_dev, const uint8_t* dones, int32_t n, int32_t steps_per_call, void* stream) {
  if (!st_dev || !dones || n <= 0) return fail(KP1_ERR_INVALID, "bad argument to kp1_curriculum_observe");
  int rc = check_device(device);
  if (rc != KP1_OK) return rc;
  hipLaunchKernelGGL(curriculum_kernel, dim3(1), dim3(64), 0, (hipStream_t)stream, st_dev, dones, n, steps_per_call);
  HIP_TRY(kp1::launch_status());
  return KP1_OK;
}
int kp1_curriculum_observe_chunk(int32_t device, kp1_curriculum_state* st_dev, const uint8_t* dones, int32_t n_local, int32_t chunk_steps,
                                 int32_t world, void* stream) {
  if (!st_dev || !dones || n_local <= 0 || chunk_steps <= 0 || world <= 0) return fail(KP1_ERR_INVALID, "bad argument to kp1_curriculum_observe_chunk");
  int rc = check_device(device);
  if (rc != KP1_OK) return rc;
  hipLaunchKernelGGL(curriculum_chunk_kernel, dim3(1), dim3(64), 0, (hipStream_t)stream, st_dev, dones, n_local, chunk_steps, world, n_local * world);
  HIP_TRY(kp1::launch_status());
  return KP1_OK;
}
int kp1_curriculum_observe_population(int32_t device, kp1_curriculum_state* states_dev, const uint8_t* dones, int32_t n_per_replica,
                                      int32_t n_replicas, int32_t steps_per_call, void* stream) {
  if (!states_dev || !dones || n_per_replica <= 0 || n_replicas < 1 || n_replicas > KP1_CURRICULUM_MAX_REPLICAS)
    return fail(KP1_ERR_INVALID, "bad argument to kp1_curriculum_observe_population");
  int rc = check_device(device);
  if (rc != KP1_OK) return rc;
  hipLaunchKernelGGL(curriculum_population_kernel, dim3((unsigned)n_replicas), dim3(64), 0, (hipStream_t)stream, states_dev, dones, n_per_replica,
                     steps_per_call);
  HIP_TRY(kp1::launch_status());
  return KP1_OK;
}
int kp1_curriculum_read_replica(int32_t device, const kp1_curriculum_state* states_dev, int32_t n_replicas, int32_t k, kp1_curriculum_state* out_host,
                                void* stream) {
  if (!states_dev || !out_host) return fail(KP1_ERR_INVALID, "NULL argument");
  if (k < 0 || k >= n_replicas) return fail(KP1_ERR_INVALID, "replica index out of range");
  return kp1_curriculum_read(device, states_dev + k, out_host, stream);
}
int kp1_curriculum_read(int32_t device, const kp1_curriculum_state* st_dev, kp1_curriculum_state* out_host, void* stream) {
  if (!st_dev || !out_host) return fail(KP1_ERR_INVALID, "NULL argument");
  int rc = check_device(device);
  if (rc != KP1_OK) return rc;
  HIP_TRY(hipMemcpyAsync(out_host, st_dev, sizeof *out_host, hipMemcpyDeviceToHost, (hipStream_t)stream));
  HIP_TRY(hipStreamSynchronize((hipStream_t)stream));
  return KP1_OK;
}

}
```

rl_brain_trainer_amd/mlp.py:

```python
from __future__ import annotations

import ctypes as C

import torch

from . import native

OBS_DIM, OBS_PAD, ACT_DIM = 56, 64, 7


def _p(t: torch.Tensor | None):
    return C.c_void_p(t.data_ptr()) if t is not None else None


class MlpKernels:
    def __init__(self, hidden: int, device: torch.device, max_batch: int = 8192, obs_dim: int = OBS_DIM, replicas: int = 1) -> None:
        self.L = native.load()
        L = self.L
        vp, i32, f32 = C.c_void_p, C.c_int32, C.c_float
        L.kp1_mlp_create_ex.argtypes = [i32, i32, i32, i32, C.POINTER(vp)]
        L.kp1_mlp_create_population.argtypes = [i32, i32, i32, i32, i32, C.POINTER(vp)]
        L.kp1_mlp_replicas.argtypes = [vp]
        L.kp1_mlp_replicas.restype = i32
        L.kp1_mlp_destroy.argtypes = [vp]
        L.kp1_mlp_num_params_ex.argtypes = [i32, i32]
        L.kp1_mlp_num_params_ex.restype = C.c_int64
        L.kp1_mlp_pack_weights.argtypes = [vp, vp, vp]
        L.kp1_mlp_forward.argtypes = [vp, vp, i32, i32, vp, vp, vp, vp, vp, vp, vp]
        L.kp1_mlp_forward_env_step.argtypes = [vp, vp, vp, i32, vp, vp, vp, vp, vp, vp, vp, vp, vp]
        L.kp1_mlp_loss_grad.argtypes = [vp, vp, i32, vp, i32, vp, vp, vp, vp, f32, f32, vp, f32, f32, f32, f32, vp, vp, i32, vp]
        L.kp1_mlp_adam_step.argtypes = [vp, vp, vp, vp, vp, f32, f32, f32, i32, i32, vp]
        L.kp1_mlp_time_kernels.argtypes = [vp, vp, i32, i32, i32, vp, vp, vp]
        L.kp1_mlp_placement_check.argtypes = [i32, i32, vp, vp]
        L.kp1_mlp_set_option.argtypes = [vp, i32, i32]
        L.kp1_mlp_profile_read.argtypes = [vp, vp, vp]
        L.kp1_mlp_set_replica_hparams.argtypes = [vp, vp, i32, vp]
        self.hidden = hidden
        self.device = device
        self.max_batch = int(max_batch)
        self._h = vp()
        self.obs_dim = int(obs_dim)
        self.obs_pad = 64 if self.obs_dim <= 64 else 128
        if replicas == 1:
            native.check(L.kp1_mlp_create_ex(device.index or 0, hidden, self.obs_dim, self.max_batch, C.byref(self._h)))
        else:
            native.check(L.kp1_mlp_create_population(device.index or 0, hidden, self.obs_dim, self.max_batch, int(replicas), C.byref(self._h)))
        self.replicas = int(L.kp1_mlp_replicas(self._h))
        self.num_params = int(L.kp1_mlp_num_params_ex(hidden, self.obs_dim))

    def close(self) -> None:
        if self._h.value:
            self.L.kp1_mlp_destroy(self._h)
            self._h = C.c_void_p()

    OPT_FUSED = 1

    def set_fused(self, on: bool) -> None:
        native.check(self.L.kp1_mlp_set_option(self._h, self.OPT_FUSED, int(bool(on))))

    OPT_ACTOR_EXTRA_STEPS = 2

    def set_actor_extra_steps(self, steps: int) -> None:
        native.check(self.L.kp1_mlp_set_option(self._h, self.OPT_ACTOR_EXTRA_STEPS, int(steps)))

    OPT_STEP_COUNT = 3

    def set_step_count(self, steps: int) -> None:
        native.check(self.L.kp1_mlp_set_option(self._h, self.OPT_STEP_COUNT, int(steps)))

    OPT_BF16X3_WGRAD = 5

    def set_bf16x3_wgrad(self, on: bool) -> None:
        native.check(self.L.kp1_mlp_set_option(self._h, self.OPT_BF16X3_WGRAD, int(bool(on))))

    OPT_PROFILE = 4
    PROFILE_SLOTS = ("mlp_train_tile", "gemm_tn_split", "grad_finalize", "adam")

    def set_profile(self, on: bool) -> None:
        native.check(self.L.kp1_mlp_set_option(self._h, self.OPT_PROFILE, int(bool(on))))

    def profile_read(self) -> dict[str, dict[str, float]]:
        us = (C.c_float * 4)()
        cnt = (C.c_int32 * 4)()
        native.check(self.L.kp1_mlp_profile_read(self._h, C.cast(us, C.c_void_p), C.cast(cnt, C.c_void_p)))
        return {name: {"us": float(us[i]), "launches": int(cnt[i])} for i, name in enumerate(self.PROFILE_SLOTS)}

    HPARAM_FIELDS = ("learning_rate", "adam_eps", "max_grad_norm", "clip_range", "ent_coef", "vf_coef")

    def set_replica_hparams(self, rows: list[dict[str, float]] | None) -> None:
        if rows is None:
            native.check(self.L.kp1_mlp_set_replica_hparams(self._h, None, 0, self._stream()))
            return
        table = (C.c_float * (len(rows) * len(self.HPARAM_FIELDS)))(*[float(r[f]) for r in rows for f in self.HPARAM_FIELDS])
        native.check(self.L.kp1_mlp_set_replica_hparams(self._h, C.cast(table, C.c_void_p), len(rows), self._stream()))

    def _stream(self):
        return C.c_void_p(torch.cuda.current_stream(self.device).cuda_stream)

    def pack(self, flat_params: torch.Tensor) -> None:
        assert flat_params.numel() == self.replicas * self.num_params and flat_params.dtype == torch.float32 and flat_params.is_contiguous()
        native.check(self.L.kp1_mlp_pack_weights(self._h, _p(flat_params), self._stream()))

    def forward(self, obs: torch.Tensor, *, noise=None, mean=None, value=None, action=None, clipped=None, log_prob=None) -> None:
        assert obs.shape[0] % self.replicas == 0
        n, stride = obs.shape[0] // self.replicas, obs.shape[1]
        assert obs.is_contiguous() and obs.dtype == torch.float32
        native.check(self.L.kp1_mlp_forward(self._h, _p(obs), stride, n, _p(noise), _p(mean), _p(value), _p(action), _p(clipped), _p(log_prob), self._stream()))

    def forward_env_step(self, env, obs: torch.Tensor, *, noise, value, action, log_prob, next_obs, reward, done, terminal_obs) -> None:
        assert obs.is_contiguous() and obs.dtype == torch.float32 and obs.shape[0] == env.n_envs
        native.check(self.L.kp1_mlp_forward_env_step(self._h, env._handle, _p(obs), obs.shape[1], _p(noise), _p(value), _p(action), _p(log_prob),
                                                     _p(next_obs), _p(reward), _p(done), _p(terminal_obs), self._stream()))

    def mean_value(self, obs: torch.Tensor) -> tuple[torch.Tensor, torch.Tensor]:
        n = obs.shape[0]
        mean = torch.empty((n, ACT_DIM), dtype=torch.float32, device=obs.device)
        value = torch.empty(n, dtype=torch.float32, device=obs.device)
        for s in range(0, n, self.max_batch):
            e = min(s + self.max_batch, n)
            self.forward(obs[s:e], mean=mean[s:e], value=value[s:e])
        return mean, value

    def loss_grad(self, obs: torch.Tensor, idx: torch.Tensor | None, n: int, actions, old_logp, adv, ret, *, clip_range: float, ent_coef: float,
                  vf_coef: float, inv_count: float, grad_out: torch.Tensor, stats_out: torch.Tensor | None, adv_stats: torch.Tensor | None = None,
                  normalize: bool = True, grad_is_zero: bool = False) -> None:
        assert obs.is_contiguous() and grad_out.numel() == self.replicas * self.num_params
        assert self.replicas == 1 or (idx is not None and idx.numel() == self.replicas * n)
        inv_std = 0.0 if normalize else -1.0
        native.check(self.L.kp1_mlp_loss_grad(self._h, _p(obs), obs.shape[-1], _p(idx), n, _p(actions), _p(old_logp), _p(adv), _p(ret), 0.0, inv_std,
                                              _p(adv_stats), clip_range, ent_coef, vf_coef, inv_count, _p(grad_out), _p(stats_out), int(grad_is_zero), self._stream()))

    def adam_step(self, params, grad, exp_avg, exp_avg_sq, *, lr: float, eps: float, max_grad_norm: float, step: int,
                  fused_norm: bool = False) -> None:
        native.check(self.L.kp1_mlp_adam_step(self._h, _p(params), _p(grad), _p(exp_avg), _p(exp_avg_sq), lr, eps, max_grad_norm, step,
                                              2 if fused_norm else 0, self._stream()))

    def anchor_loss_grad(self, obs: torch.Tensor, idx: torch.Tensor | None, n: int, teacher_actions: torch.Tensor, *, loss_weight: float,
                         grad_out: torch.Tensor, loss_out: torch.Tensor) -> None:
        assert obs.is_contiguous() and obs.dtype == torch.float32 and teacher_actions.is_contiguous() and teacher_actions.dtype == torch.float32
        assert teacher_actions.shape == (obs.shape[0], ACT_DIM) and grad_out.numel() == self.replicas * self.num_params
        assert loss_out.numel() == self.replicas and loss_out.dtype == torch.float32
        assert idx is None or (idx.dtype == torch.int64 and idx.is_contiguous() and idx.numel() == self.replicas * n)
        native.check(self.L.kp1_mlp_anchor_loss_grad(self._h, _p(obs), obs.shape[-1], _p(idx), n, _p(teacher_actions), loss_weight, _p(grad_out),
                                                     _p(loss_out), self._stream()))

    def anchor_adam_step(self, params, grad, exp_avg, exp_avg_sq, *, lr: float, eps: float, max_grad_norm: float, step: int) -> None:
        native.check(self.L.kp1_mlp_anchor_adam_step(self._h, _p(params), _p(grad), _p(exp_avg), _p(exp_avg_sq), lr, eps, max_grad_norm, step,
                                                     self._stream()))

    def placement_check(self, n_rows: int) -> dict[str, int | float]:
        out = (C.c_int32 * 8)()
        native.check(self.L.kp1_mlp_placement_check(self.device.index or 0, int(n_rows), C.cast(out, C.c_void_p), self._stream()))
        wgs, pairs, same, rr, cus, used, arrived, xcds = (int(v) for v in out)
        return {"workgroups": wgs, "compute_units": cus, "compute_units_used": used, "second_tile_on_same_cu": same, "second_tile_pairs": pairs,
                "on_xcd_of_block_index_mod_8": rr, "xcds_among_first_8_blocks": xcds, "all_resident": arrived == wgs}

    def time_kernels(self, obs: torch.Tensor, n: int, iters: int = 20) -> dict[str, dict[str, float]]:
        ms = (C.c_float * 6)()
        fl = (C.c_double * 6)()
        native.check(self.L.kp1_mlp_time_kernels(self._h, _p(obs), obs.shape[-1], n, iters, C.cast(ms, C.c_void_p), C.cast(fl, C.c_void_p), self._stream()))
        names = ("gemm_nt_fwd_l2", "gemm_nt_bwd_dz1", "gemm_tn_dw2", "gemm_nt_fwd_l1", "mlp_train_tile", "gemm_tn_split")
        return {nm: {"ms": float(ms[i]), "flops": float(fl[i]), "tflops": float(fl[i]) / (float(ms[i]) * 1e-3) / 1e12}
                for i, nm in enumerate(names) if ms[i] > 0}
```

rl_brain_trainer_amd/native.py:

```python
from __future__ import annotations

import ctypes as C
import re
from pathlib import Path

from . import config as kcfg

PKG_DIR = Path(__file__).resolve().parent
LIB_PATH = PKG_DIR / "libkp1.so"

KP1_OK = 0
REAL_F32, REAL_F64 = 0, 1
DONE_TERMINATED, DONE_TRUNCATED, DONE_SUCCESS, DONE_INVALID = 1, 2, 4, 8
FLAG_PRE_NEAR_HIT, FLAG_NEAR_HIT, FLAG_SUCCESS = 1, 2, 4


class EvalBuffers(C.Structure):
    _fields_ = [(n, C.c_void_p) for n in ("metrics", "counters", "flags", "state", "hand_metrics", "hand_step", "hand_success", "hand_state", "n_alive")]


class RouteChainView(C.Structure):
    _fields_ = [("records", C.c_void_p), ("n_records", C.c_void_p), ("n_alive", C.c_void_p), ("n_rows", C.c_int32), ("max_len", C.c_int32)]


class Kp1Error(RuntimeError):
    pass


_lib: C.CDLL | None = None


def declared_symbols() -> list[str]:
    names: list[str] = []
    for header in sorted((kcfg.repo_root() / "include").glob("*.h")):
        text = re.sub(r"/\*.*?\*/", "", header.read_text(), flags=re.S)
        names += re.findall(r"\b(kp1_[a-z0-9_]+)\s*\(", text)
    seen, out = set(), []
    for n in names:
        if n not in seen and not n.endswith("_t"):
            seen.add(n)
            out.append(n)
    return out


def load() -> C.CDLL:
    global _lib
    if _lib is not None:
        return _lib
    if not LIB_PATH.exists():
        raise Kp1Error(
            f"{LIB_PATH} is missing: the HIP extension has not been built. There is no CPU fallback; "
            "build it with `python -c 'import __graft_entry__ as g; g.build()'`."
        )
    L = C.CDLL(str(LIB_PATH))
    vp, i32, u64, i64 = C.c_void_p, C.c_int32, C.c_uint64, C.c_int64
    L.kp1_last_error.restype = C.c_char_p
    L.kp1_abi_version.restype = C.c_int
    L.kp1_config_size.restype = u64
    L.kp1_config_default.argtypes = [C.POINTER(kcfg.Kp1Config)]
    L.kp1_create.argtypes = [C.POINTER(kcfg.Kp1Config), i32, i32, i32, u64, u64, vp, C.POINTER(vp)]
    L.kp1_destroy.argtypes = [vp]
    L.kp1_set_stream.argtypes = [vp, vp]
    L.kp1_num_envs.argtypes = [vp]
    L.kp1_set_stage.argtypes = [vp, i32]
    L.kp1_get_stage.argtypes = [vp, C.POINTER(i32)]
    L.kp1_set_mode.argtypes = [vp, i32]
    L.kp1_update_config.argtypes = [vp, C.POINTER(kcfg.Kp1Config)]
    L.kp1_set_handoff_states.argtypes = [vp, vp, i32]
    L.kp1_seed.argtypes = [vp, u64, u64]
    L.kp1_reset.argtypes = [vp, vp, C.POINTER(kcfg.ResetOpts), vp]
    L.kp1_step.argtypes = [vp, vp, vp, vp, vp, vp, i32]
    L.kp1_observe.argtypes = [vp, vp]
    L.kp1_get_info.argtypes = [vp, C.POINTER(kcfg.InfoView)]
    L.kp1_eval_accumulate.argtypes = [vp, C.POINTER(EvalBuffers), vp, vp, vp, i32, vp, i32, vp]
    L.kp1_eval_step.argtypes = [vp, vp, vp, vp, vp, C.POINTER(EvalBuffers), i32, vp, i32, vp]
    L.kp1_get_reward_components.argtypes = [vp, C.POINTER(vp), C.POINTER(i32)]
    L.kp1_enable_reward_components.argtypes = [vp, i32]
    L.kp1_component_name.argtypes = [i32, i32]
    L.kp1_component_name.restype = C.c_char_p
    L.kp1_num_components.argtypes = [i32]
    L.kp1_get_state.argtypes = [vp] + [vp] * 5
    L.kp1_set_state.argtypes = [vp] + [vp] * 5 + [i32]
    L.kp1_rng_get.argtypes = [vp, vp]
    L.kp1_rng_set.argtypes = [vp, vp]
    L.kp1_state_snapshot.argtypes = [vp]
    L.kp1_state_restore.argtypes = [vp]
    L.kp1_fk_pose6.argtypes = [i32, i32, vp, vp, i64, vp]
    L.kp1_pose_error.argtypes = [i32, i32, vp, vp, vp, vp, vp, i64, vp]
    L.kp1_joint_utils.argtypes = [i32, i32, C.POINTER(kcfg.Kp1Config), vp, vp, vp, vp, vp, vp, i64, vp]
    L.kp1_rng_seed_state.argtypes = [u64, C.POINTER(kcfg.RngState)]
    f32 = C.c_float
    L.kp1_gae_scan.argtypes = [i32, vp, vp, vp, vp, f32, f32, vp, vp, i32, i32, vp]
    L.kp1_gae_scan_replicas.argtypes = [i32, vp, vp, vp, vp, vp, i32, vp, vp, i32, i32, vp]
    L.kp1_bootstrap_truncated.argtypes = [i32, vp, vp, vp, f32, i64, vp]
    L.kp1_adv_minibatch_sums.argtypes = [i32, vp, vp, i64, i64, vp, vp]
    L.kp1_adv_minibatch_stats.argtypes = [i32, vp, i64, vp, vp]
    L.kp1_random_permutation.argtypes = [i32, i64, vp, vp, vp]
    L.kp1_curriculum_create.argtypes = [i32, C.c_double, i32, i32, i32, i32, C.POINTER(vp)]
    L.kp1_curriculum_destroy.argtypes = [i32, vp]
    L.kp1_curriculum_observe.argtypes = [i32, vp, vp, i32, i32, vp]
    L.kp1_curriculum_observe_chunk.argtypes = [i32, vp, vp, i32, i32, i32, vp]
    L.kp1_curriculum_read.argtypes = [i32, vp, vp, vp]
    L.kp1_bind_stage_ptr.argtypes = [vp, vp]
    L.kp1_curriculum_create_population.argtypes = [i32, i32, C.c_double, i32, i32, i32, vp, C.POINTER(vp)]
    L.kp1_curriculum_observe_population.argtypes = [i32, vp, vp, i32, i32, i32, vp]
    L.kp1_curriculum_read_replica.argtypes = [i32, vp, i32, i32, vp, vp]
    L.kp1_bind_population_stages.argtypes = [vp, vp, i32]
    L.kp1_seed_blocks.argtypes = [vp, vp, i32, i32]
    L.kp1_set_obs_stride.argtypes = [vp, i32]
    L.kp1_route_chain_create.argtypes = [vp, vp, vp, i32, i32, C.POINTER(vp)]
    L.kp1_route_chain_destroy.argtypes = [vp, vp]
    L.kp1_route_chain_begin.argtypes = [vp, vp, vp]
    L.kp1_route_chain_step.argtypes = [vp, vp, vp, vp, vp, vp, vp]
    L.kp1_route_chain_get_view.argtypes = [vp, C.POINTER(RouteChainView)]
    L.kp1_mlp_anchor_loss_grad.argtypes = [vp, vp, i32, vp, i32, vp, f32, vp, vp, vp]
    L.kp1_mlp_anchor_adam_step.argtypes = [vp, vp, vp, vp, vp, f32, f32, f32, i32, vp]
    if L.kp1_config_size() != C.sizeof(kcfg.Kp1Config):
        raise Kp1Error(f"kp1_config layout mismatch: library {L.kp1_config_size()} vs binding {C.sizeof(kcfg.Kp1Config)}")
    _lib = L
    return L


def check(rc: int) -> None:
    if rc != KP1_OK:
        msg = load().kp1_last_error().decode(errors="replace")
        if rc == -1:
            raise ValueError(msg)
        raise Kp1Error(f"kp1 error {rc}: {msg}")


def component_names(mode: int) -> list[str]:
    L = load()
    return [L.kp1_component_name(mode, i).decode() for i in range(L.kp1_num_components(mode))]
```

rl_brain_trainer_amd/ppo.py:

```python
from __future__ import annotations

import ctypes as C
import math
import os
import time
from dataclasses import dataclass, field
from typing import Any

import numpy as np
import torch

from . import config as kcfg
from . import native
from .curriculum import PointCurriculum
from .vec_env import ArmKinematicVecEnv

OBS_DIM = kcfg.OBS_DIM
ACT_DIM = kcfg.NJ


@dataclass
class PPOConfig:

    learning_rate: float = 3e-4
# ... 284 lines not shown
            mine = torch.full((16,), self.rank + 1, dtype=torch.uint8, device=device)
            gathered = torch.zeros((self.world_size, 16), dtype=torch.uint8, device=device)
            self.dist.all_reduce(buf.clone())
            self.dist.all_gather_into_tensor(gathered.clone().view(-1), mine)
            torch.cuda.synchronize(device)

            def _hung() -> None:
                print("[kp1] a captured RCCL all-reduce did not complete within 120 s: re-run with KP1_DIST_GRAPHS=0", file=sys.stderr, flush=True)
                os._exit(3)

            dog = threading.Timer(120.0, _hung)
            dog.daemon = True
            dog.start()
            g, good = None, True
            try:
                g = torch.cuda.CUDAGraph()
                with torch.cuda.graph(g, capture_error_mode="thread_local"):
                    self.dist.all_reduce(buf)
                    self.dist.all_gather_into_tensor(gathered.view(-1), mine)
            except Exception as exc:
                print(f"[kp1] rank {self.rank}: RCCL inside hipGraph capture not available ({type(exc).__name__}: {exc}); eager collectives", file=sys.stderr)
                good = False
            captured = torch.tensor([1.0 if good else 0.0], device=device)
            self.dist.all_reduce(captured, op=self.dist.ReduceOp.MIN)
            good = bool(captured.item() > 0.5)
            if good:
                buf.fill_(float(self.rank + 1))
                gathered.zero_()
                g.replay()
                torch.cuda.synchronize(device)
                want = torch.arange(1, self.world_size + 1, dtype=torch.uint8, device=device)[:, None].expand(-1, 16)
                good = bool(torch.all(buf == expect).item()) and bool(torch.equal(gathered, want))
            dog.cancel()
            verdict.fill_(1.0 if good else 0.0)
        self.dist.all_reduce(verdict, op=self.dist.ReduceOp.MIN)
        return bool(verdict.item() > 0.5)


def _bind_policy(policy: ActorCritic, flat: torch.Tensor) -> None:
    flat.copy_(policy.flat)
    policy.flat = flat
    off = 0
    for name, shape in policy.spec:
        n = math.prod(shape)
        policy.views[name] = flat[off:off + n].view(shape)
        off += n


def load_adam_state(opt: dict[str, Any], spec, adam_m: torch.Tensor, adam_v: torch.Tensor) -> tuple[int, int]:
    steps, off = [], 0
    for i, (name, shape) in enumerate(spec):
        n = math.prod(shape)
        st = opt["state"].get(i)
        if st is None or tuple(st["exp_avg"].shape) != tuple(shape):
            raise ValueError(f"optimizer state of parameter {i} ({name}) does not match the policy")
        adam_m[off:off + n].copy_(st["exp_avg"].to(adam_m.device, torch.float32).reshape(-1))
        adam_v[off:off + n].copy_(st["exp_avg_sq"].to(adam_v.device, torch.float32).reshape(-1))
        steps.append((name, int(float(st["step"]))))
        off += n
    actor = [s_ for n_, s_ in steps if n_.startswith(("mlp_extractor.policy_net", "action_net"))]
    rest = [s_ for n_, s_ in steps if not n_.startswith(("mlp_extractor.policy_net", "action_net"))]
    if len(set(actor)) != 1 or len(set(rest)) != 1 or actor[0] < rest[0]:
        raise ValueError(f"unsupported per-tensor Adam step pattern {steps}")
    return rest[0], actor[0] - rest[0]


def restore_saved_hyperparameters(cfg: "PPOConfig", data: dict[str, Any]) -> dict[str, Any]:
    taken = {}
    for key, cast in (("gamma", float), ("gae_lambda", float), ("ent_coef", float), ("vf_coef", float), ("max_grad_norm", float),
                      ("n_epochs", int), ("normalize_advantage", bool)):
        v = data.get(key)
        if isinstance(v, (int, float, bool)) and not (isinstance(v, bool) and cast is not bool):
            setattr(cfg, key, cast(v))
            taken[key] = cast(v)
    clip = data.get("clip_range")
    if isinstance(clip, dict) and isinstance(clip.get("value"), (int, float)):
        cfg.clip_range = float(clip["value"])
        taken["clip_range"] = cfg.clip_range
    return taken


class PPO:

    def __init__(self, env: ArmKinematicVecEnv, cfg: PPOConfig, *, curriculum: PointCurriculum | None = None,
                 dist: Dist | None = None, backend: str = "hip", use_graphs: bool = True) -> None:
        if backend != "hip":
            raise ValueError("backend must be 'hip': the HIP kernels are the only training path")
        if getattr(env, "is_population", False):
            raise TypeError("PPO trains one seed; a population env (K replicas in one handle) is trained by population.ApproachPopulationPPO")
        if env.dtype != torch.float32:
            raise ValueError("PPO drives the production f32 env")
        self.env = env
        self.curriculum = curriculum
        self._setup(cfg, [cfg.seed], [env], [curriculum], dist or Dist(), use_graphs, min_batch=8192, stacked=False)
        self.policy = self.policies[0]
        T, N, dev = cfg.n_steps, self.n_envs, self.device
        self.done_chunk = 1
        if self.dist.enabled:
            self.done_chunk = math.gcd(T, max(int(os.environ.get("KP1_DONE_EXCHANGE_STEPS", "16")), 1))
            self._done_gather = torch.zeros((self.dist.world_size, self.done_chunk, N), dtype=torch.uint8, device=dev)
            self._record_stage = None
            if curriculum is not None and getattr(curriculum, "needs_episode_records", False):
                self._record_stage = torch.zeros((self.done_chunk, N), dtype=torch.uint8, device=dev)
        self._fused_env_step = bool(type(env) is ArmKinematicVecEnv and env.dtype == torch.float32 and cfg.hidden == 256
                                    and self.obs_dim <= 64 and not getattr(env, "_reward_components_on", False)
                                    and os.environ.get("KP1_FUSED_ROLLOUT", "1") != "0")

    def _setup(self, cfg: PPOConfig, seeds: list[int], envs: list[Any], curricula: list[Any], dist: Dist, use_graphs: bool, *,
               min_batch: int, stacked: bool) -> None:
        self.cfg = cfg
        self.dist = dist
        self.backend = "hip"
        self.L = native.load()
        self.K = K = len(seeds)
        self.envs, self.curricula = envs, curricula
        self.device = dev = envs[0].device
        self.n_envs = N = envs[0].n_envs
        self.obs_dim = int(getattr(envs[0], "obs_dim", OBS_DIM))
        self.obs_w = 64 if self.obs_dim <= 64 else 128
        for env, cur in zip(envs, curricula):
            if cur is not None:
                cur.attach(env)
            env.set_obs_stride(self.obs_w)
        self.policies = [ActorCritic(cfg.hidden, dev, seed=s, obs_dim=self.obs_dim) for s in seeds]
        self.flat = self.policies[0].flat
        if stacked:
            self.flat = torch.zeros((K, self.policies[0].numel), dtype=torch.float32, device=dev)
            for k, pol in enumerate(self.policies):
                _bind_policy(pol, self.flat[k])
        self.dist.broadcast(self.flat)
        self.adam_m = torch.zeros_like(self.flat)
        self.adam_v = torch.zeros_like(self.flat)
        self.grad = torch.zeros_like(self.flat)
        self.stats_dev = torch.zeros((K, 4), dtype=torch.float32, device=dev)
        self.adam_t = 0
        self.n_train_calls = 0
        self.actor_extra_steps = 0
        self.num_timesteps = 0
        T, KN = cfg.n_steps, K * N
        self.obs_buf = torch.zeros((T + 1, KN, self.obs_w), dtype=torch.float32, device=dev)
        self.term_obs_buf = torch.zeros((T, KN, self.obs_w), dtype=torch.float32, device=dev)
        self.act_buf = torch.zeros((T, KN, ACT_DIM), dtype=torch.float32, device=dev)
        self.clip_act = torch.zeros((KN, ACT_DIM), dtype=torch.float32, device=dev)
        self.logp_buf = torch.zeros((T, KN), dtype=torch.float32, device=dev)
        self.val_buf = torch.zeros((T, KN), dtype=torch.float32, device=dev)
        self.rew_buf = torch.zeros((T, KN), dtype=torch.float32, device=dev)
        self.done_buf = torch.zeros((T, KN), dtype=torch.uint8, device=dev)
        self.adv_buf = torch.zeros((T, KN), dtype=torch.float32, device=dev)
        self.ret_buf = torch.zeros((T, KN), dtype=torch.float32, device=dev)
        self.noise_all = torch.zeros((T, KN, ACT_DIM), dtype=torch.float32, device=dev)
        self.perm = torch.zeros((K, T * N), dtype=torch.int64, device=dev)
        self.gens = [torch.Generator(device=dev).manual_seed(int(s) + 7919 * self.dist.rank) for s in seeds]
        self._perm_rngs = [np.random.Generator(np.random.PCG64(np.random.SeedSequence([int(s), self.dist.rank, 0x6B7031]))) for s in seeds]
        self._needs_reset = True
        self._last_stats_dev: tuple[torch.Tensor, int] | None = None
        self._last_stats_host: list[dict[str, float]] = [{} for _ in range(K)]
        from . import mlp as _mlp

        local_bs = max(cfg.batch_size // self.dist.world_size, 1)
        self._mlp = _mlp.MlpKernels(cfg.hidden, dev, max_batch=max(N, local_bs, min_batch), obs_dim=self.obs_dim, replicas=K)
        self._mlp.pack(self.flat)
        if os.environ.get("KP1_BF16X3_WGRAD", "0") == "1" and cfg.hidden == 256:
            self._mlp.set_bf16x3_wgrad(True)
        self.use_graphs = bool(use_graphs)
        self.dist.use_stream_collectives(dev)
        self.graph_mode = self.dist.graph_mode(dev) if self.use_graphs else "none"
        self._first_replay_checked = {"rollout": not (self.dist.enabled and self.graph_mode == "captured"),
                                      "epoch": not (self.dist.enabled and self.graph_mode == "captured")}
        self._rollout_graph = None
        self._epoch_graph = None
        self._epoch_policy = os.environ.get("KP1_DP_EPOCH", "auto")
        self._epoch_auto = None
        self.epoch_form = "one graph" if self.graph_mode == "captured" else ("eager launches" if self.graph_mode == "none" or self._epoch_policy == "eager" else "graph segments")
        self._rollout_graph_key = None
        self._epoch_graph_key = None
        self._epoch_warm = False
        self._kernels_warm = False
        self.step_callback = None

    def _sl(self, k: int) -> slice:
        return slice(k * self.n_envs, (k + 1) * self.n_envs)

    PERM_CIPHER_MIN = 1 << 17

    def _draw_perm(self, k: int) -> None:
        out = self.perm[k]
        total = out.numel()
        if total < self.PERM_CIPHER_MIN:
            torch.randperm(total, device=self.device, generator=self.gens[k], out=out)
            return
        keys = self._perm_rngs[k].integers(0, 1 << 32, size=8, dtype=np.uint64).astype(np.uint32)
        native.check(self.L.kp1_random_permutation(self.device.index or 0, total, keys.ctypes.data_as(C.c_void_p), C.c_void_p(out.data_ptr()),
                                                   C.c_void_p(torch.cuda.current_stream(self.device).cuda_stream)))

    def _draw_noise(self) -> None:
        self.noise_all.normal_(generator=self.gens[0])

    def invalidate_graphs(self) -> None:
        self._rollout_graph = None
        self._epoch_graph = None

    def _epoch_key(self) -> tuple:
        c = self.cfg
        return (c.learning_rate, c.clip_range, c.ent_coef, c.vf_coef, c.max_grad_norm, c.adam_eps, c.batch_size, c.n_steps, c.normalize_advantage,
                self.dist.world_size)

    def _curriculum_observe(self, t: int) -> None:
        if self.curriculum is None:
            return
        if not self.dist.enabled:
            self.curriculum.observe(self.done_buf[t], self.n_envs)
            return
        c = self.done_chunk
        if self._record_stage is not None:
            self.curriculum.record(self.done_buf[t], self._record_stage[t % c])
        if (t + 1) % c == 0:
            src = self.done_buf[t + 1 - c:t + 1] if self._record_stage is None else self._record_stage
            self.dist.all_gather_into(self._done_gather, src)
            self.curriculum.observe_chunk(self._done_gather, self.n_envs, c, self.dist.world_size)

    def load_checkpoint(self, path: str, *, restore_optimizer: bool = True, restore_timesteps: bool = False,
                        restore_hyperparameters: bool = False) -> dict[str, Any]:
        from . import checkpoint

        self.policy.load_state_dict(checkpoint.load_policy_state_dict(path))
        restored: dict[str, Any] = {"policy": True, "optimizer": False}
        opt = checkpoint.load_optimizer_state_dict(path) if restore_optimizer else None
        if opt and opt.get("state"):
            self.adam_t, self.actor_extra_steps = load_adam_state(opt, self.policy.spec, self.adam_m, self.adam_v)
            restored.update({"optimizer": True, "adam_steps": self.adam_t, "actor_extra_steps": self.actor_extra_steps})
        self._mlp.pack(self.policy.flat)
        self._mlp.set_step_count(self.adam_t)
        self._mlp.set_actor_extra_steps(self.actor_extra_steps)
        if restore_timesteps or restore_hyperparameters:
            data = checkpoint.load_data(path)
            if restore_timesteps:
                self.num_timesteps = int(data.get("num_timesteps", 0))
                restored["num_timesteps"] = self.num_timesteps
                saved_epochs = data.get("n_epochs")
                if isinstance(data.get("_n_updates"), int) and isinstance(saved_epochs, int) and saved_epochs > 0:
                    self.n_train_calls = int(data["_n_updates"]) // saved_epochs
            if restore_hyperparameters:
                if self._epoch_graph is not None or self.adam_t != restored.get("adam_steps", self.adam_t):
                    raise RuntimeError("restore_hyperparameters must happen before the first update")
                restored["hyperparameters"] = restore_saved_hyperparameters(self.cfg, data)
        return restored

    def _forward(self, obs: torch.Tensor) -> tuple[torch.Tensor, torch.Tensor]:
        return self._mlp.mean_value(obs.contiguous())

    def predict(self, obs: torch.Tensor, deterministic: bool = True) -> torch.Tensor:
        with torch.no_grad():
            mean, _ = self._forward(obs)
            if not deterministic:
                mean = mean + torch.exp(self.policy.views["log_std"]) * torch.randn(mean.shape, device=mean.device, generator=self.gens[0])
            return mean.clamp(-1.0, 1.0)

    def predict_unclipped(self, obs: torch.Tensor) -> torch.Tensor:
        with torch.no_grad():
            return self._forward(obs)[0]

    def _bootstrap_truncated(self, dense: bool = False) -> None:
        cfg, env = self.cfg, self.env
        T, N = cfg.n_steps, self.n_envs
        stream = torch.cuda.current_stream(self.device).cuda_stream
        dev = self.device.index or 0
        if not dense:
            max_steps = max(int(env.config.c.termination.max_episode_steps), 1)
            cap = min(N * (T // max_steps + 1), T * N)
            trunc = (self.done_buf.view(-1) & 3) == 2
            idx = torch.nonzero_static(trunc, size=cap, fill_value=0).view(-1)
            valid = torch.arange(cap, device=self.device) < trunc.sum()
            sel = self.term_obs_buf.view(T * N, self.obs_w).index_select(0, idx)
            tv = torch.empty(cap, dtype=torch.float32, device=self.device)
            for s0 in range(0, cap, self._mlp.max_batch):
                e0 = min(s0 + self._mlp.max_batch, cap)
                self._mlp.forward(sel[s0:e0], value=tv[s0:e0])
            self.rew_buf.view(-1).index_add_(0, idx, torch.where(valid, cfg.gamma * tv, torch.zeros_like(tv)))
        else:
            _, tv = self._forward(self.term_obs_buf.view(T * N, self.obs_w))
            tv = tv.contiguous()
            native.check(self.L.kp1_bootstrap_truncated(dev, C.c_void_p(self.rew_buf.data_ptr()), C.c_void_p(tv.data_ptr()),
                                                        C.c_void_p(self.done_buf.data_ptr()), cfg.gamma, T * N, C.c_void_p(stream)))

    @torch.no_grad()
    def collect_rollouts(self) -> None:
        cfg = self.cfg
        T, N = cfg.n_steps, self.n_envs
        if self._needs_reset:
            self._reset_envs()
            self._needs_reset = False
        else:
            self.obs_buf[0].copy_(self.obs_buf[T])
        world = self.dist.world_size
        graph_rollout = self.use_graphs and self.step_callback is None
        self._draw_noise()
        if graph_rollout:
            key = (tuple(getattr(env, "launch_args_version", 0) for env in self.envs), tuple(cur is not None for cur in self.curricula),
                   cfg.gamma, cfg.gae_lambda)
            if self._rollout_graph is None or self._rollout_graph_key != key:
                self._capture_rollout()
                self._rollout_graph_key = key
            self._replay_checked("rollout", self._rollout_graph)
        for t in range(0 if not graph_rollout else T, T):
            self._rollout_step_hip(t)
            if self.step_callback is not None:
                self.step_callback(self.done_buf[t])
        if not graph_rollout:
            self._kernels_warm = True
        self.num_timesteps += T * N * world
        if not graph_rollout:
            self._post_rollout()

    def _post_rollout(self) -> None:
        cfg = self.cfg
        T, KN = cfg.n_steps, self.K * self.n_envs
        self._bootstrap_truncated()
        stream = torch.cuda.current_stream(self.device).cuda_stream
        dev = self.device.index or 0
        last_v = torch.empty(KN, dtype=torch.float32, device=self.device)
        self._mlp.forward(self.obs_buf[T], value=last_v)
        native.check(self.L.kp1_gae_scan(dev, C.c_void_p(self.rew_buf.data_ptr()), C.c_void_p(self.val_buf.data_ptr()),
                                         C.c_void_p(self.done_buf.data_ptr()), C.c_void_p(last_v.data_ptr()), cfg.gamma, cfg.gae_lambda,
                                         C.c_void_p(self.adv_buf.data_ptr()), C.c_void_p(self.ret_buf.data_ptr()), T, KN, C.c_void_p(stream)))

    def _rollout_step_hip(self, t: int) -> None:
        self._policy_env_step(t)
        self._curriculum_observe(t)

    def _policy_env_step(self, t: int) -> None:
        if self._fused_env_step:
            self._mlp.forward_env_step(self.env, self.obs_buf[t], noise=self.noise_all[t], value=self.val_buf[t], action=self.act_buf[t],
                                       log_prob=self.logp_buf[t], next_obs=self.obs_buf[t + 1], reward=self.rew_buf[t], done=self.done_buf[t],
                                       terminal_obs=self.term_obs_buf[t])
        else:
            self._mlp.forward(self.obs_buf[t], noise=self.noise_all[t], value=self.val_buf[t], action=self.act_buf[t],
                              clipped=self.clip_act, log_prob=self.logp_buf[t])
            self.env.step_into(self.clip_act, self.obs_buf[t + 1], self.rew_buf[t], self.done_buf[t], self.term_obs_buf[t], True)

    def _capture_rollout(self) -> None:
        T = self.cfg.n_steps
        if not self._kernels_warm:
            side = torch.cuda.Stream(device=self.device)
            side.wait_stream(torch.cuda.current_stream(self.device))
            with torch.cuda.stream(side):
                for env in self.envs:
                    env.use_current_stream()
                    if hasattr(env, "snapshot"):
                        env.snapshot()
                self._policy_env_step(0)
                self._warm_curricula()
                self._post_rollout()
                fresh = []
                for k, env in enumerate(self.envs):
                    env.use_current_stream()
                    if hasattr(env, "snapshot"):
                        env.restore()
                    else:
                        fresh.append(k)
                if fresh:
                    self._reset_envs(fresh)
            torch.cuda.current_stream(self.device).wait_stream(side)
            self._kernels_warm = True
        torch.cuda.synchronize(self.device)

        def body() -> None:
            for t in range(T):
                self._rollout_step_hip(t)
            self._post_rollout()

        self._rollout_graph = self._capture(body, on_begin=self._envs_use_current_stream)
        self._envs_use_current_stream()

    def _reset_envs(self, which: list[int] | None = None) -> None:
        for k in range(len(self.envs)) if which is None else which:
            self.obs_buf[0, self._sl(k)].copy_(self.envs[k].reset())

    def _warm_curricula(self) -> None:
        for k, cur in enumerate(self.curricula):
            if cur is not None:
                cur.observe(self.done_buf[0, self._sl(k)].zero_(), 0)

    def _envs_use_current_stream(self) -> None:
        for env in self.envs:
            env.use_current_stream()

    def _capture(self, body, on_begin=None):
        if self.dist.enabled and self.graph_mode == "segmented":
            seg = GraphSegments(self.device, on_begin=on_begin)
            self.dist._segments = seg
            try:
                seg.begin()
                body()
                seg.finish()
            except BaseException:
                seg.abort()
                raise
            finally:
                self.dist._segments = None
            return seg
        g = torch.cuda.CUDAGraph()
        with torch.cuda.graph(g, capture_error_mode="thread_local" if self.dist.enabled else "global"):
            if on_begin is not None:
                on_begin()
            body()
        return g

    def _replay_checked(self, what: str, graph) -> None:
        if self._first_replay_checked[what]:
            graph.replay()
            return
        dog = self.dist.watchdog(300.0, f"the first replay of the {what} graph with captured RCCL collectives")
        graph.replay()
        torch.cuda.synchronize(self.device)
        ok = self.dist.ranks_agree(self.policy.flat)
        dog.cancel()
        self._first_replay_checked[what] = True
        if not ok:
            raise RuntimeError(f"ranks diverged after the first replay of the {what} graph with captured RCCL collectives; re-run with KP1_DIST_GRAPHS=0")

    def train(self) -> None:
        cfg = self.cfg
        total = cfg.n_steps * self.n_envs
        local_bs = max(cfg.batch_size // self.dist.world_size, 1)
        n_mb = (total + local_bs - 1) // local_bs
        self.n_train_calls += 1
        self.stats_dev.zero_()
        for _epoch in range(cfg.n_epochs):
            for k in range(self.K):
                self._draw_perm(k)
            if not self.use_graphs:
                self._mlp.set_step_count(self.adam_t)
                self._epoch_body()
            elif self._epoch_graph is None and not self._epoch_warm:
                self._epoch_warm = True
                self._epoch_body()
            elif self._epoch_graph is None or self._epoch_graph_key != self._epoch_key():
                self._epoch_graph = None
                torch.cuda.synchronize(self.device)
                self._epoch_graph = self._capture(self._epoch_body)
                self._epoch_graph_key = self._epoch_key()
                self._epoch_auto = {"phase": 0} if (self.graph_mode == "segmented" and self._epoch_policy == "auto") else None
                self._replay_checked("epoch", self._epoch_graph)
            else:
                if self.graph_mode == "segmented" and self._segmented_epoch_eager():
                    self._epoch_body()
                else:
                    self._replay_checked("epoch", self._epoch_graph)
                self._segmented_epoch_timed()
            self.adam_t += n_mb
        self._last_stats_dev = (self.stats_dev.clone(), n_mb * cfg.n_epochs)

    def _epoch_body(self) -> None:
        cfg = self.cfg
        T = cfg.n_steps
        total = T * self.n_envs
        local_bs = max(cfg.batch_size // self.dist.world_size, 1)
        obs = self.obs_buf[:T].view(total, self.obs_w)
        act, old_logp = self.act_buf.view(total, ACT_DIM), self.logp_buf.view(total)
        adv, ret = self.adv_buf.view(total), self.ret_buf.view(total)
        perm = self.perm[0]
        mb_stats = self._epoch_adv_stats(adv, perm, total, local_bs)
        for i, start in enumerate(range(0, total, local_bs)):
            self._hip_minibatch_step(obs, perm[start:start + local_bs], act, old_logp, adv, ret, device_step=True,
                                     adv_stats=None if mb_stats is None else mb_stats[i])

    def _segmented_epoch_eager(self) -> bool:
        if self._epoch_policy != "auto":
            return self._epoch_policy == "eager"
        a = self._epoch_auto
        if a is None:
            return False
        if a["phase"] in (0, 1):
            a["ev"] = (torch.cuda.Event(enable_timing=True), torch.cuda.Event(enable_timing=True))
            a["ev"][0].record()
            return a["phase"] == 1
        return bool(a["eager"])

    def _segmented_epoch_timed(self) -> None:
        a = self._epoch_auto
        if a is None or self._epoch_policy != "auto" or a["phase"] > 1:
            return
        a["ev"][1].record()
        a["t_graph" if a["phase"] == 0 else "t_eager"] = a["ev"]
        a["phase"] += 1
        if a["phase"] == 2:
            torch.cuda.synchronize(self.device)
            t = torch.tensor([a["t_graph"][0].elapsed_time(a["t_graph"][1]), a["t_eager"][0].elapsed_time(a["t_eager"][1])], dtype=torch.float64, device=self.device)
            if self.dist.enabled:
                self.dist.dist.all_reduce(t, op=self.dist.dist.ReduceOp.MAX)
            a["ms"] = [float(x) for x in t.tolist()]
            a["eager"] = a["ms"][1] < a["ms"][0]
            self.epoch_form = "eager launches" if a["eager"] else "graph segments"

    @property
    def last_stats(self) -> dict[str, float]:
        return self._stats_rows()[0]

    def _stats_rows(self) -> list[dict[str, float]]:
        if self._last_stats_dev is not None:
            stats, n_updates = self._last_stats_dev
            rows = (stats / max(n_updates, 1)).tolist()
            self._last_stats_host = [dict(zip(("policy_loss", "value_loss", "entropy", "approx_kl"), r), n_updates=n_updates) for r in rows]
            self._last_stats_dev = None
        return self._last_stats_host

    def _epoch_adv_stats(self, adv, perm, total: int, local_bs: int):
        if not self.cfg.normalize_advantage:
            return None
        n_mb = (total + local_bs - 1) // local_bs
        sums = torch.empty((n_mb, 3), dtype=torch.float64, device=self.device)
        stream = torch.cuda.current_stream(self.device).cuda_stream
        native.check(self.L.kp1_adv_minibatch_sums(self.device.index or 0, C.c_void_p(adv.data_ptr()), C.c_void_p(perm.data_ptr()), total, local_bs,
                                                   C.c_void_p(sums.data_ptr()), C.c_void_p(stream)))
        self.dist.all_reduce_sum(sums)
        out = torch.empty((n_mb, 2), dtype=torch.float32, device=self.device)
        native.check(self.L.kp1_adv_minibatch_stats(self.device.index or 0, C.c_void_p(sums.data_ptr()), n_mb, C.c_void_p(out.data_ptr()),
                                                    C.c_void_p(stream)))
        return out

    def _hip_minibatch_step(self, obs, idx, act, old_logp, adv, ret, device_step: bool = False, adv_stats=None) -> None:
        cfg = self.cfg
        n = int(idx.numel())
        world = self.dist.world_size
        if adv_stats is None and cfg.normalize_advantage and self.dist.enabled:
            mean, inv_std = global_advantage_stats(adv[idx], self.dist)
            adv_stats = torch.stack([mean, inv_std]).float()
        self._mlp.loss_grad(obs, idx, n, act, old_logp, adv, ret, clip_range=cfg.clip_range, ent_coef=cfg.ent_coef / world, vf_coef=cfg.vf_coef,
                            inv_count=1.0 / (n * world), grad_out=self.grad, stats_out=self.stats_dev, adv_stats=adv_stats,
                            normalize=cfg.normalize_advantage)
        self.dist.all_reduce_sum(self.grad)
        if not device_step:
            self.adam_t += 1
        self._mlp.adam_step(self.policy.flat, self.grad, self.adam_m, self.adam_v, lr=cfg.learning_rate, eps=cfg.adam_eps,
                            max_grad_norm=cfg.max_grad_norm, step=0 if device_step else self.adam_t, fused_norm=not self.dist.enabled)

    def learn(self, total_timesteps: int | None = None, log_every: int = 0) -> "PPO":
        total = int(total_timesteps if total_timesteps is not None else self.cfg.total_timesteps)
        start_steps = self.num_timesteps
        it = 0
        t0 = time.time()
        while self.num_timesteps - start_steps < total:
            self.collect_rollouts()
            self.train()
            it += 1
            if log_every and it % log_every == 0 and self.dist.rank == 0:
                dt = time.time() - t0
                stages = [cur.read().stage_index if cur is not None else -1 for cur in self.curricula]
                stats = self._stats_rows()
                print(f"[ppo] it={it} steps={self.num_timesteps} fps={(self.num_timesteps - start_steps) / dt:,.0f} "
                      f"stage={stages[0] if self.K == 1 else stages} rew={self.rew_buf.mean().item():.4f} {stats[0] if self.K == 1 else stats}",
                      flush=True)
        return self


class InferencePolicy:

    def __init__(self, state_dict: dict[str, torch.Tensor], device: torch.device | int = 0, max_batch: int = 8192) -> None:
        self.device = torch.device("cuda", device) if isinstance(device, int) else torch.device(device)
        hidden, obs_dim = (int(v) for v in state_dict["mlp_extractor.policy_net.0.weight"].shape)
        self.obs_dim = obs_dim
        self.policy = ActorCritic(hidden, self.device, obs_dim=obs_dim)
        self.policy.load_state_dict(state_dict)
        from . import mlp as _mlp

        self._mlp = _mlp.MlpKernels(hidden, self.device, max_batch=max_batch, obs_dim=obs_dim)
        self._mlp.pack(self.policy.flat)

    @classmethod
    def load(cls, path: str, device: torch.device | int = 0, max_batch: int = 8192) -> "InferencePolicy":
        from . import checkpoint

        return cls(checkpoint.load_policy_state_dict(path), device=device, max_batch=max_batch)

    @torch.no_grad()
    def predict(self, obs: torch.Tensor, deterministic: bool = True) -> torch.Tensor:
        if not deterministic:
            raise NotImplementedError("evaluators use deterministic=True")
        mean, _ = self._mlp.mean_value(obs.contiguous())
        return mean.clamp(-1.0, 1.0)

    __call__ = predict


def ppo_loss_and_grad_torch(flat: torch.Tensor, spec, obs, act, old_logp, adv, ret, *, clip_range: float, ent_coef: float, vf_coef: float,
                            world_size: int = 1) -> torch.Tensor:
    flat = flat.detach().clone().requires_grad_(True)
    P, off = {}, 0
    for name, shape in spec:
        n = math.prod(shape)
        P[name] = flat[off:off + n].view(shape)
        off += n
    mean, value = mlp_forward(P, obs)
    logp = gaussian_log_prob(act, mean, P["log_std"])
    ratio = torch.exp(logp - old_logp)
    denom = float(obs.shape[0] * world_size)
    pl = -torch.min(adv * ratio, adv * torch.clamp(ratio, 1 - clip_range, 1 + clip_range)).sum() / denom
    vl = ((ret - value) ** 2).sum() / denom
    ent = (0.5 + LOG_SQRT_2PI + P["log_std"]).sum()
    loss = pl + vf_coef * vl - ent_coef * ent / world_size
    (grad,) = torch.autograd.grad(loss, flat)
    return grad


def global_advantage_stats(adv: torch.Tensor, dist: "Dist") -> tuple[torch.Tensor, torch.Tensor]:
# ... 23 lines not shown
```

Measured before the change: 11.37 million.

## Fuse curriculum tracking into env-step kernel and capture whole update in one graph

Moves curriculum success tracking into the fused rollout tile kernel, where the last-finishing block uses a ticket counter to update the tracker state. It also adds device-side compaction and scatter for truncated-episode bootstrap, and a single fused epoch-prepare kernel that builds the permutation and advantage stats. The whole multi-epoch PPO update is captured in one graph. Together these aim to remove per-step curriculum launches, torch index ops and per-epoch host round trips, at the cost of added kernel complexity, more LDS use and ticket synchronisation.

After: 11.41 million, median of 6. No clear change (+0.3%).

```diff
diff --git a/include/kp1_ppo.h b/include/kp1_ppo.h
--- a/include/kp1_ppo.h
+++ b/include/kp1_ppo.h
@@ -18,11 +18,18 @@
 int kp1_bootstrap_truncated(int32_t device, float* rewards, const float* terminal_values, const uint8_t* dones, float gamma,
                             int64_t count, void* stream);
 
+int kp1_truncated_compact(int32_t device, const uint8_t* dones, int64_t count, int64_t* out_idx, int32_t cap, int32_t* out_count, void* stream);
+int kp1_bootstrap_scatter(int32_t device, float* rewards, const int64_t* idx, const float* values, const int32_t* count_dev, float gamma, int32_t cap,
+                          void* stream);
+
 int kp1_adv_minibatch_sums(int32_t device, const float* advantages, const int64_t* idx, int64_t total, int64_t minibatch, double* out_sums,
                            void* stream);
 int kp1_random_permutation(int32_t device, int64_t n, const uint32_t* keys, int64_t* out, void* stream);
 
 int kp1_adv_minibatch_stats(int32_t device, const double* sums, int64_t n_minibatches, float* out_stats, void* stream);
+
+int kp1_epoch_prepare(int32_t device, const float* advantages, int64_t total, int64_t minibatch, const uint32_t* keys_dev, int32_t epoch,
+                      int64_t* out_perm, double* out_sums, float* out_stats, uint32_t* ticket, void* stream);
 
 #define KP1_CURRICULUM_MAX_WINDOW 1024
 #define KP1_CURRICULUM_MAX_HISTORY 64
@@ -127,6 +134,11 @@
 int kp1_mlp_forward_env_step(kp1_mlp* m, kp1_env* env, const float* obs, int32_t obs_stride, const float* noise, float* value, float* action,
                              float* log_prob, float* next_obs, float* reward, uint8_t* done, float* terminal_obs, void* stream);
 
+int kp1_mlp_forward_env_step_tracked(kp1_mlp* m, kp1_env* env, const float* obs, int32_t obs_stride, const float* noise, float* value,
+                                     float* action, float* log_prob, float* next_obs, float* reward, uint8_t* done, float* terminal_obs,
+                                     kp1_curriculum_state* tracker, uint32_t* ticket, int32_t steps_per_call, void* stream);
+int kp1_ticket_clear(int32_t device, uint32_t* tickets, int64_t count, void* stream);
+
 int kp1_eval_step(kp1_mlp* m, kp1_env* env, float* obs, float* reward, uint8_t* done, const kp1_eval_buffers* buffers, int32_t step,
                   const double* ready_thresholds , int32_t confirm_steps, void* stream);
 
diff --git a/rl_brain_trainer_amd/csrc/kp1_curriculum.inc b/rl_brain_trainer_amd/csrc/kp1_curriculum.inc
--- /dev/null
+++ b/rl_brain_trainer_amd/csrc/kp1_curriculum.inc
@@ -0,0 +1,265 @@
+#ifndef KP1_TRACKER_SYNC
+#error "define KP1_TRACKER_SYNC() before including kp1_curriculum.inc"
+#endif
+
+struct TrackerCtx {
+  int stage, count, len, head, window, min_episodes, max_stage, n_events, sum;
+  double threshold;
+  long long timesteps;
+  bool ring_dirty;
+};
+
+__device__ __forceinline__ void tracker_load(const kp1_curriculum_state* __restrict__ st, int* __restrict__ ring, TrackerCtx& c) {
+  const int lane = threadIdx.x;
+  c.stage = st->stage_index; c.count = st->stage_episode_count; c.len = st->ring_len; c.head = st->ring_head;
+  c.window = st->window_episodes; c.min_episodes = st->min_episodes_per_stage; c.max_stage = st->max_stage_index; c.n_events = st->n_events;
+  c.threshold = st->success_rate_threshold; c.timesteps = st->num_timesteps;
+  c.ring_dirty = false;
+  int part = 0;
+  for (int k = lane; k < c.window; k += 64) {
+    const int v = st->ring[k];
+    ring[k] = v;
+    const int age = k >= c.head ? k - c.head : k - c.head + c.window;
+    if (age < c.len) part += v;
+  }
+  for (int off = 32; off > 0; off >>= 1) part += __shfl_xor(part, off);
+  c.sum = part;
+  KP1_TRACKER_SYNC();
+}
+
+__device__ __forceinline__ void tracker_store(kp1_curriculum_state* __restrict__ st, const int* __restrict__ ring, const TrackerCtx& c) {
+  const int lane = threadIdx.x;
+  KP1_TRACKER_SYNC();
+  if (c.ring_dirty)
+    for (int k = lane; k < c.window; k += 64) st->ring[k] = ring[k];
+  if (lane == 0) {
+    st->stage_index = c.stage; st->stage_episode_count = c.count; st->ring_len = c.len; st->ring_head = c.head;
+    st->n_events = c.n_events; st->num_timesteps = c.timesteps;
+  }
+}
+
+constexpr int TRK_BLOCK = 64 * 64, TRK_PARALLEL_MIN = 192;
+struct TrackerScratch { uint8_t* sbit; uint16_t* pfx; };
+
+__device__ __forceinline__ void tracker_append_run(int* __restrict__ ring, TrackerCtx& c, const uint8_t* __restrict__ sbit, int pos, int R) {
+  const int lane = threadIdx.x, W = c.window;
+  const int j0 = R > W ? R - W : 0;
+  KP1_TRACKER_SYNC();
+  for (int j = j0 + lane; j < R; j += 64) ring[(c.head + c.len + j) % W] = sbit[pos + j];
+  KP1_TRACKER_SYNC();
+  const int over = c.len + R - W;
+  c.head = over > 0 ? (c.head + over) % W : c.head;
+  c.len = c.len + R < W ? c.len + R : W;
+  c.count += R;
+  int part = 0;
+  for (int k = lane; k < W; k += 64) {
+    const int age = k >= c.head ? k - c.head : k - c.head + W;
+    if (age < c.len) part += ring[k];
+  }
+  for (int off = 32; off > 0; off >>= 1) part += __shfl_xor(part, off);
+  c.sum = part;
+}
+
+__device__ __forceinline__ void tracker_block_parallel(kp1_curriculum_state* __restrict__ st, int* __restrict__ ring, TrackerCtx& c, const TrackerScratch& ws,
+                                                       unsigned long long dmask, unsigned long long smask, int E) {
+  const int lane = threadIdx.x, W = c.window;
+  int mine = __popcll(dmask), off = mine;
+  for (int d = 1; d < 64; d <<= 1) {
+    const int up = __shfl_up(off, d);
+    if (lane >= d) off += up;
+  }
+  off -= mine;
+  KP1_TRACKER_SYNC();
+  for (unsigned long long m = dmask; m; m &= m - 1) {
+    const int b = __ffsll((long long)m) - 1;
+    ws.sbit[off++] = (uint8_t)((smask >> b) & 1ull);
+  }
+  KP1_TRACKER_SYNC();
+  int pos = 0;
+  while (pos < E) {
+    const int R = E - pos;
+    if (c.stage >= c.max_stage) {
+      tracker_append_run(ring, c, ws.sbit, pos, R);
+      break;
+    }
+    const int L = c.len, T = L + R;
+    const int seg = (T + 63) / 64, j_lo = lane * seg < T ? lane * seg : T, j_hi = j_lo + seg < T ? j_lo + seg : T;
+    auto y = [&](int j) -> int { return j < L ? ring[(c.head + j) % W] : (int)ws.sbit[pos + (j - L)]; };
+    int tot = 0;
+    for (int j = j_lo; j < j_hi; ++j) tot += y(j);
+    int run = tot;
+    for (int d = 1; d < 64; d <<= 1) {
+      const int up = __shfl_up(run, d);
+      if (lane >= d) run += up;
+    }
+    run -= tot;
+    KP1_TRACKER_SYNC();
+    if (lane == 0) ws.pfx[0] = 0;
+    for (int j = j_lo; j < j_hi; ++j) {
+      run += y(j);
+      ws.pfx[j + 1] = (uint16_t)run;
+    }
+    KP1_TRACKER_SYNC();
+    int best = R;
+    for (int r = lane; r < R; r += 64) {
+      const int filled = L + r + 1;
+      if (filled < W || c.count + r + 1 < c.min_episodes) continue;
+      const int wsum = (int)ws.pfx[filled] - (int)ws.pfx[filled - W];
+      if ((double)wsum / (double)W >= c.threshold) {
+        best = r;
+        break;
+      }
+    }
+    for (int d = 32; d > 0; d >>= 1) {
+      const int o = __shfl_xor(best, d);
+      best = o < best ? o : best;
+    }
+    if (best >= R) {
+      tracker_append_run(ring, c, ws.sbit, pos, R);
+      break;
+    }
+    const int filled = L + best + 1;
+    const double rate = (double)((int)ws.pfx[filled] - (int)ws.pfx[filled - W]) / (double)W;
+    if (lane == 0 && c.n_events < KP1_CURRICULUM_MAX_HISTORY) {
+      kp1_curriculum_event& ev = st->events[c.n_events];
+      ev.total_timesteps = c.timesteps;
+      ev.from_stage = c.stage;
+      ev.to_stage = c.stage + 1;
+      ev.trigger_success_rate = rate;
+    }
+    c.n_events += 1;
+    c.stage += 1;
+    c.count = 0;
+    c.len = 0;
+    c.head = 0;
+    c.sum = 0;
+    pos += best + 1;
+  }
+}
+
+__device__ __forceinline__ void curriculum_scan(kp1_curriculum_state* __restrict__ st, int* __restrict__ ring, TrackerCtx& c, const TrackerScratch& ws,
+                                                const uint8_t* __restrict__ dones, int n, int steps_per_call) {
+  const int lane = threadIdx.x;
+  c.timesteps += steps_per_call;
+  for (int base = 0; base < n; base += 64 * 64) {
+    const int first = base + lane * 64;
+    unsigned long long dmask = 0ull, smask = 0ull;
+    if (first + 64 <= n && (reinterpret_cast<uintptr_t>(dones + first) & 15) == 0) {
+      const uint4* p = reinterpret_cast<const uint4*>(dones + first);
+      uint4 w[4];
+#pragma unroll
+      for (int q = 0; q < 4; ++q) w[q] = p[q];
+#pragma unroll
+      for (int q = 0; q < 4; ++q) {
+        const unsigned int words[4] = {w[q].x, w[q].y, w[q].z, w[q].w};
+#pragma unroll
+        for (int k = 0; k < 4; ++k)
+#pragma unroll
+          for (int b = 0; b < 4; ++b) {
+            const unsigned int d = (words[k] >> (8 * b)) & 0xffu;
+            const int bit = q * 16 + k * 4 + b;
+            if (d & (KP1_DONE_TERMINATED | KP1_DONE_TRUNCATED)) {
+              dmask |= 1ull << bit;
+              if (d & KP1_DONE_SUCCESS) smask |= 1ull << bit;
+            }
+          }
+      }
+    } else {
+      for (int b = 0; b < 64 && first + b < n; ++b) {
+        const uint8_t d = dones[first + b];
+        if (d & (KP1_DONE_TERMINATED | KP1_DONE_TRUNCATED)) {
+          dmask |= 1ull << b;
+          if (d & KP1_DONE_SUCCESS) smask |= 1ull << b;
+        }
+      }
+    }
+    unsigned long long busy = __ballot(dmask != 0ull);
+    if (busy == 0ull) continue;
+    c.ring_dirty = true;
+    {
+      int ended = __popcll(dmask);
+      for (int off = 32; off > 0; off >>= 1) ended += __shfl_xor(ended, off);
+      if (ended >= TRK_PARALLEL_MIN) {
+        tracker_block_parallel(st, ring, c, ws, dmask, smask, ended);
+        continue;
+      }
+    }
+    int stage = c.stage, count = c.count, len = c.len, head = c.head, sum = c.sum, n_events = c.n_events;
+    const int window = c.window;
+    while (busy) {
+      const int src = __ffsll((long long)busy) - 1;
+      busy &= busy - 1;
+      unsigned long long m = __shfl(dmask, src);
+      const unsigned long long sm = __shfl(smask, src);
+      if (lane != 0) continue;
+      while (m) {
+        const int b = __ffsll((long long)m) - 1;
+        m &= m - 1;
+        const int success = (int)((sm >> b) & 1ull);
+        count += 1;
+        if (len < window) {
+          ring[head + len < window ? head + len : head + len - window] = success;
+          len += 1;
+          sum += success;
+        } else {
+          sum += success - ring[head];
+          ring[head] = success;
+          head = head + 1 < window ? head + 1 : 0;
+        }
+        if (stage >= c.max_stage) continue;
+        if (count < c.min_episodes) continue;
+        if (len < window) continue;
+        const double rate = (double)sum / (double)len;
+        if (rate >= c.threshold) {
+          if (n_events < KP1_CURRICULUM_MAX_HISTORY) {
+            kp1_curriculum_event& ev = st->events[n_events];
+            ev.total_timesteps = c.timesteps;
+            ev.from_stage = stage;
+            ev.to_stage = stage + 1;
+            ev.trigger_success_rate = rate;
+          }
+          n_events += 1;
+          stage += 1;
+          count = 0;
+          len = 0;
+          head = 0;
+          sum = 0;
+        }
+      }
+    }
+    c.stage = __shfl(stage, 0); c.count = __shfl(count, 0); c.len = __shfl(len, 0); c.head = __shfl(head, 0);
+    c.sum = __shfl(sum, 0); c.n_events = __shfl(n_events, 0);
+  }
+}
+
+__device__ __forceinline__ bool tracker_idle_step(kp1_curriculum_state* __restrict__ st, const uint8_t* __restrict__ dones, int n, int steps_per_call) {
+  const int lane = threadIdx.x;
+  bool any = false;
+  for (int base = 0; base < n; base += 64 * 64) {
+    const int first = base + lane * 64;
+    if (first + 64 <= n && (reinterpret_cast<uintptr_t>(dones + first) & 15) == 0) {
+      const uint4* p = reinterpret_cast<const uint4*>(dones + first);
+      unsigned int acc = 0u;
+#pragma unroll
+      for (int q = 0; q < 4; ++q) {
+        const uint4 w = p[q];
+        acc |= w.x | w.y | w.z | w.w;
+      }
+      any |= (acc & (0x01010101u * (unsigned)(KP1_DONE_TERMINATED | KP1_DONE_TRUNCATED))) != 0u;
+    } else {
+      for (int b = 0; b < 64 && first + b < n; ++b) any |= (dones[first + b] & (KP1_DONE_TERMINATED | KP1_DONE_TRUNCATED)) != 0;
+    }
+  }
+  if (__ballot(any) != 0ull) return false;
+  if (lane == 0) atomicAdd(reinterpret_cast<unsigned long long*>(&st->num_timesteps), (unsigned long long)(long long)steps_per_call);
+  return true;
+}
+
+__device__ __forceinline__ void tracker_observe_step(kp1_curriculum_state* __restrict__ st, int* __restrict__ ring, const TrackerScratch& ws,
+                                                     const uint8_t* __restrict__ dones, int n, int steps_per_call) {
+  if (tracker_idle_step(st, dones, n, steps_per_call)) return;
+  TrackerCtx c;
+  tracker_load(st, ring, c);
+  curriculum_scan(st, ring, c, ws, dones, n, steps_per_call);
+  tracker_store(st, ring, c);
+}
diff --git a/rl_brain_trainer_amd/csrc/kp1_mlp.hip b/rl_brain_trainer_amd/csrc/kp1_mlp.hip
--- a/rl_brain_trainer_amd/csrc/kp1_mlp.hip
+++ b/rl_brain_trainer_amd/csrc/kp1_mlp.hip
@@ -1273,6 +1273,12 @@
 __global__ void anchor_count_kernel(int* __restrict__ actor_extra) { *actor_extra += 1; }
 
 #include "kp1_env_step.inc"
+#define KP1_TRACKER_SYNC()                                    \
+  do {                                                        \
+    __builtin_amdgcn_fence(__ATOMIC_ACQ_REL, "workgroup");    \
+    __builtin_amdgcn_wave_barrier();                          \
+  } while (0)
+#include "kp1_curriculum.inc"
 #include "kp1_eval_step.inc"
 #include "kp1_mlp_tile.inc"
 #include "kp1_mlp_fused.inc"
@@ -1784,6 +1790,14 @@
 
 int kp1_mlp_forward_env_step(kp1_mlp* m, kp1_env* env, const float* obs, int32_t obs_stride, const float* noise, float* value, float* action,
                              float* log_prob, float* next_obs, float* reward, uint8_t* done, float* terminal_obs, void* stream) {
+  return kp1_mlp_forward_env_step_tracked(m, env, obs, obs_stride, noise, value, action, log_prob, next_obs, reward, done, terminal_obs, nullptr, nullptr,
+                                          0, stream);
+}
+
+int kp1_mlp_forward_env_step_tracked(kp1_mlp* m, kp1_env* env, const float* obs, int32_t obs_stride, const float* noise, float* value,
+                                     float* action, float* log_prob, float* next_obs, float* reward, uint8_t* done, float* terminal_obs,
+                                     kp1_curriculum_state* tracker, uint32_t* ticket, int32_t steps_per_call, void* stream) {
+  if ((tracker == nullptr) != (ticket == nullptr)) return fail(KP1_ERR_INVALID, "kp1_mlp_forward_env_step_tracked takes a tracker and its ticket word together");
   if (!m || !env || !obs || !action || !next_obs || !reward || !done) return fail(KP1_ERR_INVALID, "NULL argument to kp1_mlp_forward_env_step");
   if (m->K > 1) return fail(KP1_ERR_UNSUPPORTED, "kp1_mlp_forward_env_step is not available on population handles");
   if (!(m->fused && m->Hp == FU_HP) || m->L.INP != 64)
@@ -1801,6 +1815,7 @@
   fa.obs = obs; fa.obs_stride = obs_stride; fa.Kreal = obs_stride >= m->L.INP ? m->L.INP : m->L.IN; fa.inp = m->L.INP; fa.idx = nullptr; fa.n = (int)n_envs;
   fa.k = m->k;
   fa.noise = noise; fa.value = value; fa.action = action; fa.log_prob = log_prob;
+  fa.trk = tracker; fa.trk_ticket = ticket; fa.trk_steps = steps_per_call;
   rc = launch_fused_infer_env(fa, mode, (hipStream_t)stream);
   if (rc != KP1_OK) return rc;
   HIP_TRY(kp1::launch_status());
diff --git a/rl_brain_trainer_amd/csrc/kp1_mlp_tile.inc b/rl_brain_trainer_amd/csrc/kp1_mlp_tile.inc
--- a/rl_brain_trainer_amd/csrc/kp1_mlp_tile.inc
+++ b/rl_brain_trainer_amd/csrc/kp1_mlp_tile.inc
@@ -15,6 +15,7 @@
   int net_base;
   int stagger_ticks, n_cus;
   StepArgs<float> env;
+  kp1_curriculum_state* trk; unsigned int* trk_ticket; int trk_steps;
   unsigned short* sp_h1; unsigned short* sp_dz2; unsigned short* sp_dz1; unsigned short* sp_xf; int64_t sp_plane, sp_plane_x;
 };
 
@@ -55,6 +56,8 @@
 constexpr int FU_SCRATCH = 4 * FU_BM * 8 + FU_BM * 8 + FU_NW * 24 + 64;
 constexpr int FU_LDS_FLOATS = 2 * FU_BM * FU_AP + HEADS * FU_HP + FU_SCRATCH;
 static_assert(FU_LDS_FLOATS * 4 * 2 <= 160 * 1024, "the two training tiles of one CU must fit its LDS");
+static_assert(KP1_CURRICULUM_MAX_WINDOW * 4 + TRK_BLOCK + (TRK_BLOCK + KP1_CURRICULUM_MAX_WINDOW + 1) * 2 <= FU_BM * FU_AP * 4,
+              "the tracker's ring and whole-wave scratch must fit bufA (fused rollout tile)");
 
 template <bool TRAIN, int K1S, int ENV = 0, bool SPLIT = false>
 __global__ void __launch_bounds__(FU_NTH, ENV ? 1 : 2) mlp_tile_kernel(const FusedArgs a) {
@@ -349,6 +352,28 @@
           if (live) step_env_lane<float, ENV == 1 ? KP1_MODE_APPROACH : KP1_MODE_DOCK, false>(a.env, (int64_t)(m0 + lane), dout + lane * 8, o);
           store_obs_tile(a.env.obs, (int64_t)m0, min(BM, a.n - m0), o, live, a.env.obs_stride, bufA);
         }
+        if (a.trk_ticket) {
+          asm volatile("s_waitcnt vmcnt(0)" ::: "memory");
+          __syncthreads();
+          if (tid == 0) {
+            __builtin_amdgcn_fence(__ATOMIC_RELEASE, "agent");
+            asm volatile("s_waitcnt vmcnt(0)" ::: "memory");
+            const unsigned int drawn = __hip_atomic_fetch_add(a.trk_ticket, 1u, __ATOMIC_RELAXED, __HIP_MEMORY_SCOPE_AGENT);
+            reinterpret_cast<unsigned int*>(misc)[2] = drawn == gridDim.x - 1u ? 1u : 0u;
+            if (drawn == gridDim.x - 1u) {
+              __builtin_amdgcn_fence(__ATOMIC_ACQUIRE, "agent");
+              asm volatile("s_waitcnt vmcnt(0) lgkmcnt(0)" ::: "memory");
+            }
+          }
+          __syncthreads();
+          if (reinterpret_cast<const unsigned int*>(misc)[2] != 0u && wave == 0) {
+            __builtin_amdgcn_fence(__ATOMIC_ACQUIRE, "agent");
+            int* ring = reinterpret_cast<int*>(bufA);
+            uint8_t* sbit = reinterpret_cast<uint8_t*>(ring + KP1_CURRICULUM_MAX_WINDOW);
+            const TrackerScratch ws = {sbit, reinterpret_cast<uint16_t*>(sbit + TRK_BLOCK)};
+            tracker_observe_step(a.trk, ring, ws, a.env.done, a.n, a.trk_steps);
+          }
+        }
       }
     } else if (l_ok && l_out == 7 && a.value) {
       a.value[l_src] = v;
diff --git a/rl_brain_trainer_amd/csrc/kp1_ppo.hip b/rl_brain_trainer_amd/csrc/kp1_ppo.hip
--- a/rl_brain_trainer_amd/csrc/kp1_ppo.hip
+++ b/rl_brain_trainer_amd/csrc/kp1_ppo.hip
@@ -59,235 +59,8 @@
   if ((d & KP1_DONE_TRUNCATED) && !(d & KP1_DONE_TERMINATED)) rewards[k] += gamma * tv[k];
 }
 
-struct TrackerCtx {
-  int stage, count, len, head, window, min_episodes, max_stage, n_events, sum;
-  double threshold;
-  long long timesteps;
-  bool ring_dirty;
-};
-
-__device__ __forceinline__ void tracker_load(const kp1_curriculum_state* __restrict__ st, int* __restrict__ ring, TrackerCtx& c) {
-  const int lane = threadIdx.x;
-  c.stage = st->stage_index; c.count = st->stage_episode_count; c.len = st->ring_len; c.head = st->ring_head;
-  c.window = st->window_episodes; c.min_episodes = st->min_episodes_per_stage; c.max_stage = st->max_stage_index; c.n_events = st->n_events;
-  c.threshold = st->success_rate_threshold; c.timesteps = st->num_timesteps;
-  c.ring_dirty = false;
-  int part = 0;
-  for (int k = lane; k < c.window; k += 64) {
-    const int v = st->ring[k];
-    ring[k] = v;
-    const int age = k >= c.head ? k - c.head : k - c.head + c.window;
-    if (age < c.len) part += v;
-  }
-  for (int off = 32; off > 0; off >>= 1) part += __shfl_xor(part, off);
-  c.sum = part;
-  __syncthreads();
-}
-
-__device__ __forceinline__ void tracker_store(kp1_curriculum_state* __restrict__ st, const int* __restrict__ ring, const TrackerCtx& c) {
-  const int lane = threadIdx.x;
-  __syncthreads();
-  if (c.ring_dirty)
-    for (int k = lane; k < c.window; k += 64) st->ring[k] = ring[k];
-  if (lane == 0) {
-    st->stage_index = c.stage; st->stage_episode_count = c.count; st->ring_len = c.len; st->ring_head = c.head;
-    st->n_events = c.n_events; st->num_timesteps = c.timesteps;
-  }
-}
-
-constexpr int TRK_BLOCK = 64 * 64, TRK_PARALLEL_MIN = 192;
-struct TrackerScratch { uint8_t* sbit; uint16_t* pfx; };
-
-__device__ __forceinline__ void tracker_append_run(int* __restrict__ ring, TrackerCtx& c, const uint8_t* __restrict__ sbit, int pos, int R) {
-  const int lane = threadIdx.x, W = c.window;
-  const int j0 = R > W ? R - W : 0;
-  __syncthreads();
-  for (int j = j0 + lane; j < R; j += 64) ring[(c.head + c.len + j) % W] = sbit[pos + j];
-  __syncthreads();
-  const int over = c.len + R - W;
-  c.head = over > 0 ? (c.head + over) % W : c.head;
-  c.len = c.len + R < W ? c.len + R : W;
-  c.count += R;
-  int part = 0;
-  for (int k = lane; k < W; k += 64) {
-    const int age = k >= c.head ? k - c.head : k - c.head + W;
-    if (age < c.len) part += ring[k];
-  }
-  for (int off = 32; off > 0; off >>= 1) part += __shfl_xor(part, off);
-  c.sum = part;
-}
-
-__device__ __forceinline__ void tracker_block_parallel(kp1_curriculum_state* __restrict__ st, int* __restrict__ ring, TrackerCtx& c, const TrackerScratch& ws,
-                                                       unsigned long long dmask, unsigned long long smask, int E) {
-  const int lane = threadIdx.x, W = c.window;
-  int mine = __popcll(dmask), off = mine;
-  for (int d = 1; d < 64; d <<= 1) {
-    const int up = __shfl_up(off, d);
-    if (lane >= d) off += up;
-  }
-  off -= mine;
-  __syncthreads();
-  for (unsigned long long m = dmask; m; m &= m - 1) {
-    const int b = __ffsll((long long)m) - 1;
-    ws.sbit[off++] = (uint8_t)((smask >> b) & 1ull);
-  }
-  __syncthreads();
-  int pos = 0;
-  while (pos < E) {
-    const int R = E - pos;
-    if (c.stage >= c.max_stage) {
-      tracker_append_run(ring, c, ws.sbit, pos, R);
-      break;
-    }
-    const int L = c.len, T = L + R;
-    const int seg = (T + 63) / 64, j_lo = lane * seg < T ? lane * seg : T, j_hi = j_lo + seg < T ? j_lo + seg : T;
-    auto y = [&](int j) -> int { return j < L ? ring[(c.head + j) % W] : (int)ws.sbit[pos + (j - L)]; };
-    int tot = 0;
-    for (int j = j_lo; j < j_hi; ++j) tot += y(j);
-    int run = tot;
-    for (int d = 1; d < 64; d <<= 1) {
-      const int up = __shfl_up(run, d);
-      if (lane >= d) run += up;
-    }
-    run -= tot;
-    __syncthreads();
-    if (lane == 0) ws.pfx[0] = 0;
-    for (int j = j_lo; j < j_hi; ++j) {
-      run += y(j);
-      ws.pfx[j + 1] = (uint16_t)run;
-    }
-    __syncthreads();
-    int best = R;
-    for (int r = lane; r < R; r += 64) {
-      const int filled = L + r + 1;
-      if (filled < W || c.count + r + 1 < c.min_episodes) continue;
-      const int wsum = (int)ws.pfx[filled] - (int)ws.pfx[filled - W];
-      if ((double)wsum / (double)W >= c.threshold) {
-        best = r;
-        break;
-      }
-    }
-    for (int d = 32; d > 0; d >>= 1) {
-      const int o = __shfl_xor(best, d);
-      best = o < best ? o : best;
-    }
-    if (best >= R) {
-      tracker_append_run(ring, c, ws.sbit, pos, R);
-      break;
-    }
-    const int filled = L + best + 1;
-    const double rate = (double)((int)ws.pfx[filled] - (int)ws.pfx[filled - W]) / (double)W;
-    if (lane == 0 && c.n_events < KP1_CURRICULUM_MAX_HISTORY) {
-      kp1_curriculum_event& ev = st->events[c.n_events];
-      ev.total_timesteps = c.timesteps;
-      ev.from_stage = c.stage;
-      ev.to_stage = c.stage + 1;
-      ev.trigger_success_rate = rate;
-    }
-    c.n_events += 1;
-    c.stage += 1;
-    c.count = 0;
-    c.len = 0;
-    c.head = 0;
-    c.sum = 0;
-    pos += best + 1;
-  }
-}
-
-__device__ __forceinline__ void curriculum_scan(kp1_curriculum_state* __restrict__ st, int* __restrict__ ring, TrackerCtx& c, const TrackerScratch& ws,
-                                                const uint8_t* __restrict__ dones, int n, int steps_per_call) {
-  const int lane = threadIdx.x;
-  c.timesteps += steps_per_call;
-  for (int base = 0; base < n; base += 64 * 64) {
-    const int first = base + lane * 64;
-    unsigned long long dmask = 0ull, smask = 0ull;
-    if (first + 64 <= n && (reinterpret_cast<uintptr_t>(dones + first) & 15) == 0) {
-      const uint4* p = reinterpret_cast<const uint4*>(dones + first);
-      uint4 w[4];
-#pragma unroll
-      for (int q = 0; q < 4; ++q) w[q] = p[q];
-#pragma unroll
-      for (int q = 0; q < 4; ++q) {
-        const unsigned int words[4] = {w[q].x, w[q].y, w[q].z, w[q].w};
-#pragma unroll
-        for (int k = 0; k < 4; ++k)
-#pragma unroll
-          for (int b = 0; b < 4; ++b) {
-            const unsigned int d = (words[k] >> (8 * b)) & 0xffu;
-            const int bit = q * 16 + k * 4 + b;
-            if (d & (KP1_DONE_TERMINATED | KP1_DONE_TRUNCATED)) {
-              dmask |= 1ull << bit;
-              if (d & KP1_DONE_SUCCESS) smask |= 1ull << bit;
-            }
-          }
-      }
-    } else {
-      for (int b = 0; b < 64 && first + b < n; ++b) {
-        const uint8_t d = dones[first + b];
-        if (d & (KP1_DONE_TERMINATED | KP1_DONE_TRUNCATED)) {
-          dmask |= 1ull << b;
-          if (d & KP1_DONE_SUCCESS) smask |= 1ull << b;
-        }
-      }
-    }
-    unsigned long long busy = __ballot(dmask != 0ull);
-    if (busy == 0ull) continue;
-    c.ring_dirty = true;
-    {
-      int ended = __popcll(dmask);
-      for (int off = 32; off > 0; off >>= 1) ended += __shfl_xor(ended, off);
-      if (ended >= TRK_PARALLEL_MIN) {
-        tracker_block_parallel(st, ring, c, ws, dmask, smask, ended);
-        continue;
-      }
-    }
-    int stage = c.stage, count = c.count, len = c.len, head = c.head, sum = c.sum, n_events = c.n_events;
-    const int window = c.window;
-    while (busy) {
-      const int src = __ffsll((long long)busy) - 1;
-      busy &= busy - 1;
-      unsigned long long m = __shfl(dmask, src);
-      const unsigned long long sm = __shfl(smask, src);
-      if (lane != 0) continue;
-      while (m) {
-        const int b = __ffsll((long long)m) - 1;
-        m &= m - 1;
-        const int success = (int)((sm >> b) & 1ull);
-        count += 1;
-        if (len < window) {
-          ring[head + len < window ? head + len : head + len - window] = success;
-          len += 1;
-          sum += success;
-        } else {
-          sum += success - ring[head];
-          ring[head] = success;
-          head = head + 1 < window ? head + 1 : 0;
-        }
-        if (stage >= c.max_stage) continue;
-        if (count < c.min_episodes) continue;
-        if (len < window) continue;
-        const double rate = (double)sum / (double)len;
-        if (rate >= c.threshold) {
-          if (n_events < KP1_CURRICULUM_MAX_HISTORY) {
-            kp1_curriculum_event& ev = st->events[n_events];
-            ev.total_timesteps = c.timesteps;
-            ev.from_stage = stage;
-            ev.to_stage = stage + 1;
-            ev.trigger_success_rate = rate;
-          }
-          n_events += 1;
-          stage += 1;
-          count = 0;
-          len = 0;
-          head = 0;
-          sum = 0;
-        }
-      }
-    }
-    c.stage = __shfl(stage, 0); c.count = __shfl(count, 0); c.len = __shfl(len, 0); c.head = __shfl(head, 0);
-    c.sum = __shfl(sum, 0); c.n_events = __shfl(n_events, 0);
-  }
-}
+#define KP1_TRACKER_SYNC() __syncthreads()
+#include "kp1_curriculum.inc"
 
 __global__ void __launch_bounds__(64) curriculum_kernel(kp1_curriculum_state* __restrict__ st, const uint8_t* __restrict__ dones, int n,
                                                         int steps_per_call) {
@@ -295,33 +68,7 @@
   __shared__ uint8_t sbit[TRK_BLOCK];
   __shared__ uint16_t pfx[TRK_BLOCK + KP1_CURRICULUM_MAX_WINDOW + 1];
   const TrackerScratch ws = {sbit, pfx};
-  {
-    const int lane = threadIdx.x;
-    bool any = false;
-    for (int base = 0; base < n; base += 64 * 64) {
-      const int first = base + lane * 64;
-      if (first + 64 <= n && (reinterpret_cast<uintptr_t>(dones + first) & 15) == 0) {
-        const uint4* p = reinterpret_cast<const uint4*>(dones + first);
-        unsigned int acc = 0u;
-#pragma unroll
-        for (int q = 0; q < 4; ++q) {
-          const uint4 w = p[q];
-          acc |= w.x | w.y | w.z | w.w;
-        }
-        any |= (acc & (0x01010101u * (unsigned)(KP1_DONE_TERMINATED | KP1_DONE_TRUNCATED))) != 0u;
-      } else {
-        for (int b = 0; b < 64 && first + b < n; ++b) any |= (dones[first + b] & (KP1_DONE_TERMINATED | KP1_DONE_TRUNCATED)) != 0;
-      }
-    }
-    if (__ballot(any) == 0ull) {
-      if (lane == 0) atomicAdd(reinterpret_cast<unsigned long long*>(&st->num_timesteps), (unsigned long long)(long long)steps_per_call);
-      return;
-    }
-  }
-  TrackerCtx c;
-  tracker_load(st, ring, c);
-  curriculum_scan(st, ring, c, ws, dones, n, steps_per_call);
-  tracker_store(st, ring, c);
+  tracker_observe_step(st, ring, ws, dones, n, steps_per_call);
 }
 
 __global__ void __launch_bounds__(64) curriculum_chunk_kernel(kp1_curriculum_state* __restrict__ st, const uint8_t* __restrict__ dones, int n_local,
@@ -459,6 +206,17 @@
   out[i] = (int64_t)x;
 }
 
+__device__ __forceinline__ void minibatch_stats_row(const double* __restrict__ sums, int64_t b, float* __restrict__ out) {
+#pragma clang fp contract(off)
+  const double s0 = sums[3 * b], s1 = sums[3 * b + 1], cnt = sums[3 * b + 2];
+  const double mean = s0 / cnt;
+  const double dof = cnt - 1.0 < 1.0 ? 1.0 : cnt - 1.0;
+  double var = (s1 - cnt * mean * mean) / dof;
+  var = var < 0.0 ? 0.0 : var;
+  out[2 * b] = (float)mean;
+  out[2 * b + 1] = (float)(1.0 / (sqrt(var) + 1e-8));
+}
+
 __global__ void __launch_bounds__(64) adv_minibatch_stats_kernel(const double* __restrict__ sums, int64_t n_mb, float* __restrict__ out) {
 #pragma clang fp contract(off)
   const int64_t b = (int64_t)blockIdx.x * 64 + threadIdx.x;
@@ -471,9 +229,196 @@
   out[2 * b] = (float)mean;
   out[2 * b + 1] = (float)(1.0 / (sqrt(var) + 1e-8));
 }
+
+__device__ __forceinline__ unsigned int truncated_bytes(unsigned int w) { return (w >> 1) & ~w & 0x01010101u; }
+
+constexpr int TC_NTH = 1024;
+__global__ void __launch_bounds__(TC_NTH) truncated_compact_kernel(const uint8_t* __restrict__ dones, int64_t count, int64_t* __restrict__ idx, int cap,
+                                                                   int* __restrict__ n_out) {
+  __shared__ int wave_sum[TC_NTH / 64 + 1];
+  const int tid = threadIdx.x, lane = tid & 63, wave = tid >> 6;
+  const int64_t per = (((count + TC_NTH - 1) / TC_NTH) + 15) & ~(int64_t)15;
+  const int64_t b0 = tid * per < count ? tid * per : count, b1 = b0 + per < count ? b0 + per : count;
+  const bool vec = (reinterpret_cast<uintptr_t>(dones) & 15) == 0;
+  int mine = 0;
+  for (int64_t i = b0; i < b1; i += 16) {
+    if (vec && i + 16 <= b1) {
+      const uint4 w = *reinterpret_cast<const uint4*>(dones + i);
+      mine += __popc(truncated_bytes(w.x)) + __popc(truncated_bytes(w.y)) + __popc(truncated_bytes(w.z)) + __popc(truncated_bytes(w.w));
+    } else {
+      for (int64_t k = i; k < b1 && k < i + 16; ++k) mine += (dones[k] & 3) == 2;
+    }
+  }
+  int incl = mine;
+  for (int d = 1; d < 64; d <<= 1) {
+    const int up = __shfl_up(incl, d);
+    if (lane >= d) incl += up;
+  }
+  if (lane == 63) wave_sum[wave] = incl;
+  __syncthreads();
+  if (tid == 0) {
+    int run = 0;
+    for (int w = 0; w < TC_NTH / 64; ++w) {
+      const int s = wave_sum[w];
+      wave_sum[w] = run;
+      run += s;
+    }
+    wave_sum[TC_NTH / 64] = run;
+  }
+  __syncthreads();
+  const int total = wave_sum[TC_NTH / 64];
+  int pos = wave_sum[wave] + incl - mine;
+  for (int64_t i = b0; i < b1 && mine > 0; i += 16) {
+    if (vec && i + 16 <= b1) {
+      const uint4 w = *reinterpret_cast<const uint4*>(dones + i);
+      const unsigned int words[4] = {w.x, w.y, w.z, w.w};
+#pragma unroll
+      for (int q = 0; q < 4; ++q)
+        for (unsigned int m = truncated_bytes(words[q]); m; m &= m - 1) {
+          if (pos < cap) idx[pos] = i + 4 * q + ((__ffs((int)m) - 1) >> 3);
+          ++pos;
+        }
+    } else {
+      for (int64_t k = i; k < b1 && k < i + 16; ++k)
+        if ((dones[k] & 3) == 2) {
+          if (pos < cap) idx[pos] = k;
+          ++pos;
+        }
+    }
+  }
+  for (int j = total + tid; j < cap; j += TC_NTH) idx[j] = 0;
+  if (tid == 0) *n_out = total;
+}
+
+__global__ void __launch_bounds__(256) bootstrap_scatter_kernel(float* __restrict__ rewards, const int64_t* __restrict__ idx, const float* __restrict__ tv,
+                                                                const int* __restrict__ n, float gamma, int cap) {
+#pragma clang fp contract(off)
+  const int i = blockIdx.x * 256 + threadIdx.x;
+  if (i >= cap) return;
+  const int cnt = *n < cap ? *n : cap;
+  const bool zero_is_real = cnt > 0 && idx[0] == 0;
+  if (i < cnt) {
+    float r = rewards[idx[i]] + gamma * tv[i];
+    if (i == 0 && zero_is_real && cnt < cap) r += 0.0f;
+    rewards[idx[i]] = r;
+  } else if (i == cnt && !zero_is_real) {
+    rewards[0] += 0.0f;
+  }
+}
+
+constexpr int EP_U = 8;
+__global__ void __launch_bounds__(256) epoch_prepare_kernel(const float* __restrict__ adv, int64_t* __restrict__ perm, int64_t total, int64_t mb, int bits,
+                                                            const uint32_t* __restrict__ keys, double* __restrict__ sums, int n_mb,
+                                                            float* __restrict__ stats, unsigned int* __restrict__ ticket) {
+  __shared__ double s1[256], s2[256];
+  PermKeys k;
+#pragma unroll
+  for (int r = 0; r < 4; ++r) {
+    k.mul[r] = keys[r] | 1u;
+    k.add[r] = keys[4 + r];
+  }
+  const uint32_t mask = bits >= 32 ? 0xffffffffu : ((1u << bits) - 1u);
+  const int sh = bits > 1 ? bits / 2 : 1;
+  const int64_t begin = (int64_t)blockIdx.x * mb, end = begin + mb < total ? begin + mb : total;
+  double a = 0.0, b = 0.0;
+  for (int64_t i0 = begin + threadIdx.x; i0 < end; i0 += 256 * EP_U) {
+    float g[EP_U];
+#pragma unroll
+    for (int u = 0; u < EP_U; ++u) {
+      const int64_t i = i0 + 256 * u;
+      g[u] = 0.f;
+      if (i < end) {
+        uint32_t x = (uint32_t)i;
+        do {
+#pragma unroll
+          for (int r = 0; r < 4; ++r) {
+            x = (x * k.mul[r] + k.add[r]) & mask;
+            x ^= x >> sh;
+          }
+        } while ((int64_t)x >= total);
+        perm[i] = (int64_t)x;
+        g[u] = adv[x];
+      }
+    }
+#pragma unroll
+    for (int u = 0; u < EP_U; ++u)
+      if (i0 + 256 * u < end) {
+        const double v = (double)g[u];
+        a += v;
+        b += v * v;
+      }
+  }
+  s1[threadIdx.x] = a;
+  s2[threadIdx.x] = b;
+  __syncthreads();
+  for (int j = 128; j > 0; j >>= 1) {
+    if (threadIdx.x < j) {
+      s1[threadIdx.x] += s1[threadIdx.x + j];
+      s2[threadIdx.x] += s2[threadIdx.x + j];
+    }
+    __syncthreads();
+  }
+  if (threadIdx.x == 0) {
+    sums[3 * blockIdx.x] = s1[0];
+    sums[3 * blockIdx.x + 1] = s2[0];
+    sums[3 * blockIdx.x + 2] = (double)(end - begin);
+  }
+  asm volatile("s_waitcnt vmcnt(0)" ::: "memory");
+  __syncthreads();
+  if (threadIdx.x == 0) {
+    __builtin_amdgcn_fence(__ATOMIC_RELEASE, "agent");
+    asm volatile("s_waitcnt vmcnt(0)" ::: "memory");
+    const unsigned int drawn = __hip_atomic_fetch_add(ticket, 1u, __ATOMIC_RELAXED, __HIP_MEMORY_SCOPE_AGENT);
+    s1[1] = drawn == gridDim.x - 1u ? 1.0 : 0.0;
+    if (drawn == gridDim.x - 1u) {
+      __builtin_amdgcn_fence(__ATOMIC_ACQUIRE, "agent");
+      asm volatile("s_waitcnt vmcnt(0) lgkmcnt(0)" ::: "memory");
+    }
+  }
+  __syncthreads();
+  if (s1[1] == 0.0) return;
+  __builtin_amdgcn_fence(__ATOMIC_ACQUIRE, "agent");
+  for (int m = threadIdx.x; m < n_mb; m += 256) minibatch_stats_row(sums, m, stats);
+}
 }
 
 extern "C" {
+
+int kp1_epoch_prepare(int32_t device, const float* advantages, int64_t total, int64_t minibatch, const uint32_t* keys_dev, int32_t epoch,
+                      int64_t* out_perm, double* out_sums, float* out_stats, uint32_t* ticket, void* stream) {
+  if (!advantages || !keys_dev || !out_perm || !out_sums || !out_stats || !ticket || total <= 0 || total > ((int64_t)1 << 31) || minibatch <= 0 || epoch < 0)
+    return fail(KP1_ERR_INVALID, "bad argument to kp1_epoch_prepare");
+  int rc = check_device(device);
+  if (rc != KP1_OK) return rc;
+  const int64_t n_mb = (total + minibatch - 1) / minibatch;
+  if (n_mb > 65535) return fail(KP1_ERR_INVALID, "kp1_epoch_prepare: too many minibatches");
+  int bits = 1;
+  while (((int64_t)1 << bits) < total) ++bits;
+  hipLaunchKernelGGL(epoch_prepare_kernel, dim3((unsigned)n_mb), dim3(256), 0, (hipStream_t)stream, advantages, out_perm, total, minibatch, bits,
+                     keys_dev + 8 * (int64_t)epoch, out_sums, (int)n_mb, out_stats, ticket + epoch);
+  HIP_TRY(kp1::launch_status());
+  return KP1_OK;
+}
+
+int kp1_truncated_compact(int32_t device, const uint8_t* dones, int64_t count, int64_t* out_idx, int32_t cap, int32_t* out_count, void* stream) {
+  if (!dones || !out_idx || !out_count || count <= 0 || cap <= 0) return fail(KP1_ERR_INVALID, "bad argument to kp1_truncated_compact");
+  int rc = check_device(device);
+  if (rc != KP1_OK) return rc;
+  hipLaunchKernelGGL(truncated_compact_kernel, dim3(1), dim3(TC_NTH), 0, (hipStream_t)stream, dones, count, out_idx, (int)cap, out_count);
+  HIP_TRY(kp1::launch_status());
+  return KP1_OK;
+}
+
+int kp1_bootstrap_scatter(int32_t device, float* rewards, const int64_t* idx, const float* values, const int32_t* count_dev, float gamma, int32_t cap,
+                          void* stream) {
+  if (!rewards || !idx || !values || !count_dev || cap <= 0) return fail(KP1_ERR_INVALID, "bad argument to kp1_bootstrap_scatter");
+  int rc = check_device(device);
+  if (rc != KP1_OK) return rc;
+  hipLaunchKernelGGL(bootstrap_scatter_kernel, dim3((unsigned)((cap + 255) / 256)), dim3(256), 0, (hipStream_t)stream, rewards, idx, values, count_dev, gamma,
+                     (int)cap);
+  HIP_TRY(kp1::launch_status());
+  return KP1_OK;
+}
 
 int kp1_random_permutation(int32_t device, int64_t n, const uint32_t* keys, int64_t* out, void* stream) {
   if (!keys || !out || n <= 0 || n > ((int64_t)1 << 31)) return fail(KP1_ERR_INVALID, "bad argument to kp1_random_permutation");
@@ -567,6 +512,13 @@
   HIP_TRY(kp1::launch_status());
   return KP1_OK;
 }
+int kp1_ticket_clear(int32_t device, uint32_t* tickets, int64_t count, void* stream) {
+  if (!tickets || count <= 0) return fail(KP1_ERR_INVALID, "bad argument to kp1_ticket_clear");
+  int rc = check_device(device);
+  if (rc != KP1_OK) return rc;
+  HIP_TRY(hipMemsetAsync(tickets, 0, sizeof(uint32_t) * (size_t)count, (hipStream_t)stream));
+  return KP1_OK;
+}
 int kp1_curriculum_observe_chunk(int32_t device, kp1_curriculum_state* st_dev, const uint8_t* dones, int32_t n_local, int32_t chunk_steps,
                                  int32_t world, void* stream) {
   if (!st_dev || !dones || n_local <= 0 || chunk_steps <= 0 || world <= 0) return fail(KP1_ERR_INVALID, "bad argument to kp1_curriculum_observe_chunk");
diff --git a/rl_brain_trainer_amd/mlp.py b/rl_brain_trainer_amd/mlp.py
--- a/rl_brain_trainer_amd/mlp.py
+++ b/rl_brain_trainer_amd/mlp.py
@@ -28,6 +28,7 @@
         L.kp1_mlp_pack_weights.argtypes = [vp, vp, vp]
         L.kp1_mlp_forward.argtypes = [vp, vp, i32, i32, vp, vp, vp, vp, vp, vp, vp]
         L.kp1_mlp_forward_env_step.argtypes = [vp, vp, vp, i32, vp, vp, vp, vp, vp, vp, vp, vp, vp]
+        L.kp1_mlp_forward_env_step_tracked.argtypes = [vp, vp, vp, i32, vp, vp, vp, vp, vp, vp, vp, vp, vp, vp, i32, vp]
         L.kp1_mlp_loss_grad.argtypes = [vp, vp, i32, vp, i32, vp, vp, vp, vp, f32, f32, vp, f32, f32, f32, f32, vp, vp, i32, vp]
         L.kp1_mlp_adam_step.argtypes = [vp, vp, vp, vp, vp, f32, f32, f32, i32, i32, vp]
         L.kp1_mlp_time_kernels.argtypes = [vp, vp, i32, i32, i32, vp, vp, vp]
@@ -107,8 +108,15 @@
         assert obs.is_contiguous() and obs.dtype == torch.float32
         native.check(self.L.kp1_mlp_forward(self._h, _p(obs), stride, n, _p(noise), _p(mean), _p(value), _p(action), _p(clipped), _p(log_prob), self._stream()))
 
-    def forward_env_step(self, env, obs: torch.Tensor, *, noise, value, action, log_prob, next_obs, reward, done, terminal_obs) -> None:
+    def forward_env_step(self, env, obs: torch.Tensor, *, noise, value, action, log_prob, next_obs, reward, done, terminal_obs,
+                         tracker=None, ticket: torch.Tensor | None = None, steps_per_call: int = 0) -> None:
         assert obs.is_contiguous() and obs.dtype == torch.float32 and obs.shape[0] == env.n_envs
+        if tracker is not None:
+            assert ticket is not None and ticket.numel() == 1 and ticket.dtype in (torch.int32, torch.uint32) and ticket.device == obs.device
+            native.check(self.L.kp1_mlp_forward_env_step_tracked(self._h, env._handle, _p(obs), obs.shape[1], _p(noise), _p(value), _p(action),
+                                                                 _p(log_prob), _p(next_obs), _p(reward), _p(done), _p(terminal_obs), tracker._st,
+                                                                 _p(ticket), int(steps_per_call), self._stream()))
+            return
         native.check(self.L.kp1_mlp_forward_env_step(self._h, env._handle, _p(obs), obs.shape[1], _p(noise), _p(value), _p(action), _p(log_prob),
                                                      _p(next_obs), _p(reward), _p(done), _p(terminal_obs), self._stream()))
 
diff --git a/rl_brain_trainer_amd/native.py b/rl_brain_trainer_amd/native.py
--- a/rl_brain_trainer_amd/native.py
+++ b/rl_brain_trainer_amd/native.py
@@ -93,9 +93,13 @@
     L.kp1_gae_scan.argtypes = [i32, vp, vp, vp, vp, f32, f32, vp, vp, i32, i32, vp]
     L.kp1_gae_scan_replicas.argtypes = [i32, vp, vp, vp, vp, vp, i32, vp, vp, i32, i32, vp]
     L.kp1_bootstrap_truncated.argtypes = [i32, vp, vp, vp, f32, i64, vp]
+    L.kp1_truncated_compact.argtypes = [i32, vp, i64, vp, i32, vp, vp]
+    L.kp1_bootstrap_scatter.argtypes = [i32, vp, vp, vp, vp, f32, i32, vp]
     L.kp1_adv_minibatch_sums.argtypes = [i32, vp, vp, i64, i64, vp, vp]
     L.kp1_adv_minibatch_stats.argtypes = [i32, vp, i64, vp, vp]
     L.kp1_random_permutation.argtypes = [i32, i64, vp, vp, vp]
+    L.kp1_epoch_prepare.argtypes = [i32, vp, i64, i64, vp, i32, vp, vp, vp, vp, vp]
+    L.kp1_ticket_clear.argtypes = [i32, vp, i64, vp]
     L.kp1_curriculum_create.argtypes = [i32, C.c_double, i32, i32, i32, i32, C.POINTER(vp)]
     L.kp1_curriculum_destroy.argtypes = [i32, vp]
     L.kp1_curriculum_observe.argtypes = [i32, vp, vp, i32, i32, vp]
diff --git a/rl_brain_trainer_amd/ppo.py b/rl_brain_trainer_amd/ppo.py
--- a/rl_brain_trainer_amd/ppo.py
+++ b/rl_brain_trainer_amd/ppo.py
@@ -460,6 +460,13 @@
         self.perm = torch.zeros((K, T * N), dtype=torch.int64, device=dev)
         self.gens = [torch.Generator(device=dev).manual_seed(int(s) + 7919 * self.dist.rank) for s in seeds]
         self._perm_rngs = [np.random.Generator(np.random.PCG64(np.random.SeedSequence([int(s), self.dist.rank, 0x6B7031]))) for s in seeds]
+        self._stacked = bool(stacked)
+        self._step_tickets = torch.zeros(T, dtype=torch.int32, device=dev)
+        self._epoch_tickets = torch.zeros(cfg.n_epochs, dtype=torch.int32, device=dev)
+        self._perm_keys_dev = torch.zeros((cfg.n_epochs, 8), dtype=torch.int32, device=dev)
+        self._tracked_step = False
+        self._update_graph = None
+        self._update_graph_key = None
         self._needs_reset = True
         self._last_stats_dev: tuple[torch.Tensor, int] | None = None
         self._last_stats_host: list[dict[str, float]] = [{} for _ in range(K)]
@@ -497,9 +504,12 @@
         if total < self.PERM_CIPHER_MIN:
             torch.randperm(total, device=self.device, generator=self.gens[k], out=out)
             return
-        keys = self._perm_rngs[k].integers(0, 1 << 32, size=8, dtype=np.uint64).astype(np.uint32)
+        keys = self._draw_perm_keys(k)
         native.check(self.L.kp1_random_permutation(self.device.index or 0, total, keys.ctypes.data_as(C.c_void_p), C.c_void_p(out.data_ptr()),
                                                    C.c_void_p(torch.cuda.current_stream(self.device).cuda_stream)))
+
+    def _draw_perm_keys(self, k: int) -> np.ndarray:
+        return self._perm_rngs[k].integers(0, 1 << 32, size=8, dtype=np.uint64).astype(np.uint32)
 
     def _draw_noise(self) -> None:
         self.noise_all.normal_(generator=self.gens[0])
@@ -507,6 +517,7 @@
     def invalidate_graphs(self) -> None:
         self._rollout_graph = None
         self._epoch_graph = None
+        self._update_graph = None
 
     def _epoch_key(self) -> tuple:
         c = self.cfg
@@ -549,7 +560,7 @@
                 if isinstance(data.get("_n_updates"), int) and isinstance(saved_epochs, int) and saved_epochs > 0:
                     self.n_train_calls = int(data["_n_updates"]) // saved_epochs
             if restore_hyperparameters:
-                if self._epoch_graph is not None or self.adam_t != restored.get("adam_steps", self.adam_t):
+                if self._epoch_graph is not None or self._update_graph is not None or self.adam_t != restored.get("adam_steps", self.adam_t):
                     raise RuntimeError("restore_hyperparameters must happen before the first update")
                 restored["hyperparameters"] = restore_saved_hyperparameters(self.cfg, data)
         return restored
@@ -576,15 +587,17 @@
         if not dense:
             max_steps = max(int(env.config.c.termination.max_episode_steps), 1)
             cap = min(N * (T // max_steps + 1), T * N)
-            trunc = (self.done_buf.view(-1) & 3) == 2
-            idx = torch.nonzero_static(trunc, size=cap, fill_value=0).view(-1)
-            valid = torch.arange(cap, device=self.device) < trunc.sum()
+            idx = torch.empty(cap, dtype=torch.int64, device=self.device)
+            count = torch.empty(1, dtype=torch.int32, device=self.device)
+            native.check(self.L.kp1_truncated_compact(dev, C.c_void_p(self.done_buf.data_ptr()), T * N, C.c_void_p(idx.data_ptr()), cap,
+                                                      C.c_void_p(count.data_ptr()), C.c_void_p(stream)))
             sel = self.term_obs_buf.view(T * N, self.obs_w).index_select(0, idx)
             tv = torch.empty(cap, dtype=torch.float32, device=self.device)
             for s0 in range(0, cap, self._mlp.max_batch):
                 e0 = min(s0 + self._mlp.max_batch, cap)
                 self._mlp.forward(sel[s0:e0], value=tv[s0:e0])
-            self.rew_buf.view(-1).index_add_(0, idx, torch.where(valid, cfg.gamma * tv, torch.zeros_like(tv)))
+            native.check(self.L.kp1_bootstrap_scatter(dev, C.c_void_p(self.rew_buf.data_ptr()), C.c_void_p(idx.data_ptr()), C.c_void_p(tv.data_ptr()),
+                                                      C.c_void_p(count.data_ptr()), cfg.gamma, cap, C.c_void_p(stream)))
         else:
             _, tv = self._forward(self.term_obs_buf.view(T * N, self.obs_w))
             tv = tv.contiguous()
@@ -603,9 +616,12 @@
         world = self.dist.world_size
         graph_rollout = self.use_graphs and self.step_callback is None
         self._draw_noise()
+        self._tracked_step = self._tracked_step_ok()
+        if self._tracked_step and not graph_rollout:
+            self._clear_tickets(self._step_tickets)
         if graph_rollout:
             key = (tuple(getattr(env, "launch_args_version", 0) for env in self.envs), tuple(cur is not None for cur in self.curricula),
-                   cfg.gamma, cfg.gae_lambda)
+                   cfg.gamma, cfg.gae_lambda, self._tracked_step)
             if self._rollout_graph is None or self._rollout_graph_key != key:
                 self._capture_rollout()
                 self._rollout_graph_key = key
@@ -632,15 +648,28 @@
                                          C.c_void_p(self.done_buf.data_ptr()), C.c_void_p(last_v.data_ptr()), cfg.gamma, cfg.gae_lambda,
                                          C.c_void_p(self.adv_buf.data_ptr()), C.c_void_p(self.ret_buf.data_ptr()), T, KN, C.c_void_p(stream)))
 
+    def _tracked_step_ok(self) -> bool:
+        return bool(getattr(self, "_fused_env_step", False) and not self._stacked and self.K == 1 and not self.dist.enabled
+                    and type(self.curricula[0]) is PointCurriculum and not getattr(self.envs[0], "_reward_components_on", False)
+                    and os.environ.get("KP1_TICKET_TRACKER", "1") != "0")
+
+    def _clear_tickets(self, tickets: torch.Tensor) -> None:
+        native.check(self.L.kp1_ticket_clear(self.device.index or 0, C.c_void_p(tickets.data_ptr()), tickets.numel(),
+                                             C.c_void_p(torch.cuda.current_stream(self.device).cuda_stream)))
+
     def _rollout_step_hip(self, t: int) -> None:
+        if self._tracked_step:
+            self._policy_env_step(t, tracked=True)
+            return
         self._policy_env_step(t)
         self._curriculum_observe(t)
 
-    def _policy_env_step(self, t: int) -> None:
+    def _policy_env_step(self, t: int, tracked: bool = False) -> None:
         if self._fused_env_step:
+            trk = dict(tracker=self.curriculum, ticket=self._step_tickets[t:t + 1], steps_per_call=self.n_envs) if tracked else {}
             self._mlp.forward_env_step(self.env, self.obs_buf[t], noise=self.noise_all[t], value=self.val_buf[t], action=self.act_buf[t],
                                        log_prob=self.logp_buf[t], next_obs=self.obs_buf[t + 1], reward=self.rew_buf[t], done=self.done_buf[t],
-                                       terminal_obs=self.term_obs_buf[t])
+                                       terminal_obs=self.term_obs_buf[t], **trk)
         else:
             self._mlp.forward(self.obs_buf[t], noise=self.noise_all[t], value=self.val_buf[t], action=self.act_buf[t],
                               clipped=self.clip_act, log_prob=self.logp_buf[t])
@@ -673,6 +702,8 @@
         torch.cuda.synchronize(self.device)
 
         def body() -> None:
+            if self._tracked_step:
+                self._clear_tickets(self._step_tickets)
             for t in range(T):
                 self._rollout_step_hip(t)
             self._post_rollout()
@@ -734,6 +765,10 @@
         n_mb = (total + local_bs - 1) // local_bs
         self.n_train_calls += 1
         self.stats_dev.zero_()
+        if self._one_graph_update(total):
+            self._train_one_graph(n_mb)
+            self._last_stats_dev = (self.stats_dev.clone(), n_mb * cfg.n_epochs)
+            return
         for _epoch in range(cfg.n_epochs):
             for k in range(self.K):
                 self._draw_perm(k)
@@ -759,6 +794,60 @@
             self.adam_t += n_mb
         self._last_stats_dev = (self.stats_dev.clone(), n_mb * cfg.n_epochs)
 
+    def _one_graph_update(self, total: int) -> bool:
+        return bool(self.use_graphs and not self.dist.enabled and not self._stacked and self.K == 1 and self.cfg.normalize_advantage
+                    and total >= self.PERM_CIPHER_MIN and os.environ.get("KP1_EPOCH_PREP", "1") != "0")
+
+    def _train_one_graph(self, n_mb: int) -> None:
+        cfg = self.cfg
+        if self._perm_keys_dev.shape[0] != cfg.n_epochs:
+            self._perm_keys_dev = torch.zeros((cfg.n_epochs, 8), dtype=torch.int32, device=self.device)
+            self._epoch_tickets = torch.zeros(cfg.n_epochs, dtype=torch.int32, device=self.device)
+            self._update_graph = None
+        keys = np.stack([self._draw_perm_keys(0) for _ in range(cfg.n_epochs)])
+        self._perm_keys_dev.copy_(torch.from_numpy(keys.view(np.int32)).pin_memory(), non_blocking=True)
+        if self._update_graph is not None and self._update_graph_key != (self._epoch_key(), cfg.n_epochs):
+            self._update_graph = None
+        if not self._epoch_warm:
+            self._epoch_warm = True
+            native.check(self.L.kp1_random_permutation(self.device.index or 0, self.perm[0].numel(), keys[0].ctypes.data_as(C.c_void_p),
+                                                       C.c_void_p(self.perm[0].data_ptr()), C.c_void_p(torch.cuda.current_stream(self.device).cuda_stream)))
+            self._epoch_body()
+            self._update_body(1)
+        else:
+            if self._update_graph is None:
+                torch.cuda.synchronize(self.device)
+                self._update_graph = self._capture(self._update_body)
+                self._update_graph_key = (self._epoch_key(), cfg.n_epochs)
+            self._replay_checked("epoch", self._update_graph)
+        self.adam_t += n_mb * cfg.n_epochs
+
+    def _update_body(self, first_epoch: int = 0) -> None:
+        cfg = self.cfg
+        T = cfg.n_steps
+        total = T * self.n_envs
+        local_bs = max(cfg.batch_size, 1)
+        n_mb = (total + local_bs - 1) // local_bs
+        obs = self.obs_buf[:T].view(total, self.obs_w)
+        act, old_logp = self.act_buf.view(total, ACT_DIM), self.logp_buf.view(total)
+        adv, ret = self.adv_buf.view(total), self.ret_buf.view(total)
+        perm = self.perm[0]
+        self._clear_tickets(self._epoch_tickets)
+        for e in range(first_epoch, cfg.n_epochs):
+            mb_stats = self._epoch_prepare(e, adv, perm, total, local_bs)
+            for i, start in enumerate(range(0, total, local_bs)):
+                self._hip_minibatch_step(obs, perm[start:start + local_bs], act, old_logp, adv, ret, device_step=True, adv_stats=mb_stats[i])
+
+    def _epoch_prepare(self, epoch: int, adv, perm, total: int, local_bs: int):
+        n_mb = (total + local_bs - 1) // local_bs
+        sums = torch.empty((n_mb, 3), dtype=torch.float64, device=self.device)
+        out = torch.empty((n_mb, 2), dtype=torch.float32, device=self.device)
+        native.check(self.L.kp1_epoch_prepare(self.device.index or 0, C.c_void_p(adv.data_ptr()), total, local_bs,
+                                              C.c_void_p(self._perm_keys_dev.data_ptr()), int(epoch), C.c_void_p(perm.data_ptr()),
+                                              C.c_void_p(sums.data_ptr()), C.c_void_p(out.data_ptr()), C.c_void_p(self._epoch_tickets.data_ptr()),
+                                              C.c_void_p(torch.cuda.current_stream(self.device).cuda_stream)))
+        return out
+
     def _epoch_body(self) -> None:
         cfg = self.cfg
         T = cfg.n_steps
```
